# kakaobrain/hqtransformer

Measured on AMD Instinct MI355X. Metric: images/sec (256x256 class-cond sampling), higher is better.
Workload: dtype bf16

## Files before the change

hqtransformer_amd/_lib.py:

```python
from __future__ import annotations

import ctypes as C
import os
import subprocess
from typing import List, Optional

HERE = os.path.dirname(os.path.abspath(__file__))
LIB_PATH = os.path.join(HERE, 'libhqt.so')
CSRC = os.path.join(HERE, 'csrc')
SOURCES = ['engine.hip', 'kernels.hip', 'attention.hip', 'fast_kernels.hip', 'persist.hip', 'tile_gemm.hip', 'exact_gemm.hip', 'mfma_gemm.hip', 'split_conv.hip', 'split_stream_conv.hip']
ABI_VERSION = 9

PRECISION_EXACT, PRECISION_FAST, PRECISION_SPLIT = 0, 1, 2
PRECISIONS = {'exact': PRECISION_EXACT, 'fast': PRECISION_FAST, 'split': PRECISION_SPLIT}
POLICY_LATENCY, POLICY_THROUGHPUT = 0, 1
SWITCH_PERSIST, SWITCH_SINGLE_KEY, SWITCH_PERSIST_FAULT, SWITCH_SPLIT_KSLICES = 0, 1, 2, 3
LAYOUT_FAST, LAYOUT_EXACT, LAYOUT_SPLIT, LAYOUT_ALL = 1, 2, 4, 7
RESAMPLE_PIXELSHUFFLE, RESAMPLE_NEAREST, RESAMPLE_CONV2 = 0, 1, 2


class HqtLibraryError(RuntimeError):
    pass


class HqtError(RuntimeError):
    def __init__(self, code: int, msg: str):
        super().__init__(f'libhqt error {code}: {msg}')
        self.code = code


class hqt_config(C.Structure):
    _fields_ = [
        ('abi_version', C.c_int32),
        ('has_stage2', C.c_int32),
        ('embed_dim', C.c_int32), ('n_layers', C.c_int32), ('n_heads', C.c_int32), ('n_layers_depth', C.c_int32),
        ('vocab_top', C.c_int32), ('vocab_bot', C.c_int32), ('vocab_txt', C.c_int32),
        ('ctx_len_img', C.c_int32), ('ctx_len_txt', C.c_int32), ('n_classes', C.c_int32),
        ('cond_type', C.c_int32), ('embedding_type', C.c_int32), ('gelu_approx', C.c_int32),
        ('has_stage1', C.c_int32),
        ('s1_ch', C.c_int32), ('s1_n_mult', C.c_int32), ('s1_ch_mult', C.c_int32 * 8),
        ('s1_num_res_blocks', C.c_int32),
        ('s1_n_attn_res', C.c_int32), ('s1_attn_res', C.c_int32 * 4),
        ('s1_resolution', C.c_int32), ('s1_z_channels', C.c_int32), ('s1_embed_dim', C.c_int32),
        ('s1_n_embed', C.c_int32), ('s1_out_ch', C.c_int32),
        ('s1_use_init_downsample', C.c_int32), ('s1_use_mid_block', C.c_int32), ('s1_use_attn', C.c_int32),
        ('max_batch', C.c_int32), ('max_steps', C.c_int32),
        ('code_levels', C.c_int32),
        ('depth_decoding', C.c_int32),
        ('ar_layouts', C.c_int32),
        ('s1_resample', C.c_int32),
    ]


class hqt_sample_opts(C.Structure):
    _fields_ = [
        ('precision', C.c_int32), ('n_steps', C.c_int32),
        ('top_k_top', C.c_int32), ('top_k_bot', C.c_int32),
        ('top_p_top', C.c_float), ('top_p_bot', C.c_float),
        ('temperature_top', C.c_float), ('temperature_bot', C.c_float),
        ('seed', C.c_uint64), ('sample_offset', C.c_int64),
        ('use_graph', C.c_int32),
        ('row_seeds', C.c_void_p), ('row_offsets', C.c_void_p),
    ]


class hqt_sample_opts_l3(C.Structure):
    _fields_ = [
        ('precision', C.c_int32), ('n_steps', C.c_int32),
        ('top_k', C.c_int32 * 3), ('top_p', C.c_float * 3), ('temperature', C.c_float * 3),
        ('seed', C.c_uint64), ('sample_offset', C.c_int64),
        ('use_graph', C.c_int32),
        ('row_seeds', C.c_void_p), ('row_offsets', C.c_void_p),
    ]


class hqt_row_sampler(C.Structure):
    _fields_ = [('temperature', C.c_float * 3), ('top_k', C.c_int32 * 3), ('top_p', C.c_float * 3)]


class hqt_guide_pair(C.Structure):
    _fields_ = [('pos_row', C.c_int32), ('neg_row', C.c_int32), ('scale', C.c_float * 3)]


class hqt_encode_out(C.Structure):
    _fields_ = [
        ('codes', C.c_void_p * 3), ('quant', C.c_void_p * 3), ('resid', C.c_void_p * 3),
        ('recon', C.c_void_p), ('diff', C.c_void_p),
    ]


_VP, _I64P, _F32P = C.c_void_p, C.c_void_p, C.c_void_p
SYMBOLS = {
    'hqt_abi_version': (C.c_int, []),
    'hqt_last_error': (C.c_char_p, []),
    'hqt_create': (C.c_int, [C.POINTER(hqt_config), C.c_int, C.POINTER(_VP)]),
    'hqt_set_weight': (C.c_int, [_VP, C.c_char_p, _VP, C.c_int, C.POINTER(C.c_int64), C.c_int]),
    'hqt_finalize_weights': (C.c_int, [_VP]),
    'hqt_clone': (C.c_int, [_VP, C.POINTER(_VP)]),
    'hqt_set_policy': (C.c_int, [_VP, C.c_int]),
    'hqt_set_switch': (C.c_int, [_VP, C.c_int, C.c_int]),
    'hqt_set_row_samplers': (C.c_int, [_VP, C.c_int, C.POINTER(hqt_row_sampler)]),
    'hqt_set_logprob_out': (C.c_int, [_VP, _F32P]),
    'hqt_set_guidance': (C.c_int, [_VP, C.c_int, C.POINTER(hqt_guide_pair)]),
    'hqt_set_keep_mask': (C.c_int, [_VP, C.c_int, C.c_int, _VP, C.POINTER(C.c_void_p)]),
    'hqt_set_prompt_groups': (C.c_int, [_VP, C.c_int, C.c_int, _VP]),
    'hqt_sample': (C.c_int, [_VP, C.c_int, _I64P, C.POINTER(hqt_sample_opts), _F32P, _I64P, _I64P, _F32P, _I64P, _I64P, _VP]),
    'hqt_set_max_prefix': (C.c_int, [_VP, C.c_int]),
    'hqt_sample_prefix': (C.c_int, [_VP, C.c_int, _I64P, C.POINTER(hqt_sample_opts), _F32P, C.c_int, _I64P, _I64P, _I64P, _I64P, _F32P, _I64P, _I64P, _VP]),
    'hqt_set_score_chunk': (C.c_int, [_VP, C.c_int]),
    'hqt_score': (C.c_int, [_VP, C.c_int, _I64P, C.POINTER(C.c_void_p), C.c_int, C.c_int, _F32P, C.POINTER(C.c_void_p), _VP]),
    'hqt_decode': (C.c_int, [_VP, C.c_int, _I64P, _I64P, _F32P, C.c_int, C.c_int, _VP]),
    'hqt_decode_seq': (C.c_int, [_VP, C.c_int, _I64P, _I64P, _F32P, C.c_int, C.c_int, _VP]),
    'hqt_sample_l3': (C.c_int, [_VP, C.c_int, _I64P, C.POINTER(hqt_sample_opts_l3), _F32P, _I64P, _I64P, _I64P, _F32P, _I64P, _I64P, _I64P, _VP]),
    'hqt_sample_prefix_l3': (C.c_int, [_VP, C.c_int, _I64P, C.POINTER(hqt_sample_opts_l3), _F32P, C.c_int, _I64P, _I64P, _I64P, _I64P, _I64P, _I64P, _F32P, _I64P, _I64P, _I64P, _VP]),
    'hqt_decode_l3': (C.c_int, [_VP, C.c_int, _I64P, _I64P, _I64P, _F32P, C.c_int, C.c_int, _VP]),
    'hqt_decode_seq_l3': (C.c_int, [_VP, C.c_int, _I64P, _I64P, _I64P, _F32P, C.c_int, C.c_int, _VP]),
    'hqt_encode': (C.c_int, [_VP, C.c_int, _F32P, C.c_int, C.POINTER(hqt_encode_out), _VP]),
    'hqt_has_encoder': (C.c_int, [_VP]),
    'hqt_range_check': (C.c_int, [_VP, _VP]),
    'hqt_param_count': (C.c_int64, [_VP, C.c_int]),
    'hqt_workspace_bytes': (C.c_int64, [_VP]),
    'hqt_timing_enable': (C.c_int, [_VP, C.c_int]),
    'hqt_timing_reset': (C.c_int, [_VP]),
    'hqt_timing_get': (C.c_int, [_VP, C.c_int, C.c_char_p, C.c_int, C.POINTER(C.c_int64), C.POINTER(C.c_double)]),
    'hqt_timing_slots': (C.c_int, [_VP]),
    'hqt_destroy': (C.c_int, [_VP]),
}

_lib: Optional[C.CDLL] = None


def build(force: bool = False, verbose: bool = False) -> str:
    import hashlib
    from concurrent.futures import ThreadPoolExecutor
    hdrs = sorted([os.path.join(CSRC, f) for f in os.listdir(CSRC) if f.endswith('.h')] + [os.path.join(os.path.dirname(HERE), 'include', 'hqt.h')])
    hipcc = os.environ.get('HIPCC', '/opt/rocm/bin/hipcc')
    flags = ['-O3', '--offload-arch=gfx950', '-std=c++17', '-fPIC', '-Wno-unused-value', '-Wno-unused-result']
    objdir = os.path.join(CSRC, 'build')
    os.makedirs(objdir, exist_ok=True)
    ver = subprocess.run([hipcc, '--version'], stdout=subprocess.PIPE, stderr=subprocess.STDOUT, text=True).stdout
    common = hashlib.sha256()
    for f in hdrs:
        with open(f, 'rb') as fp:
            common.update(os.path.basename(f).encode() + b'\0' + fp.read())
    common.update(' '.join(flags).encode() + ver.encode())

    def read(path):
        try:
            with open(path) as fp:
                return fp.read().strip()
        except OSError:
            return ''

    def stamp_of(name):
        hh = common.copy()
        with open(os.path.join(CSRC, name), 'rb') as fp:
            hh.update(name.encode() + b'\0' + fp.read())
        return hh.hexdigest()

    def compile_one(name):
        src, obj = os.path.join(CSRC, name), os.path.join(objdir, name.replace('.hip', '.o'))
        stamp, want = obj[:-2] + '.stamp', stamp_of(name)
        if not force and os.path.exists(obj) and read(stamp) == want:
            return obj, want
        if os.path.exists(stamp):
            os.remove(stamp)
        cmd = [hipcc] + flags + ['-c', src, '-o', obj]
        if verbose:
            print(' '.join(cmd), flush=True)
# ... 106 lines not shown
```

hqtransformer_amd/csrc/engine.hip:

```cpp
#include "../../include/hqt.h"
#include "kernels.h"
#include "fast_kernels.h"
#include "split_kernels.h"
#include "persist.h"

#include <algorithm>
#include <cmath>
#include <cstdarg>
#include <cstdio>
#include <cstring>
#include <map>
#include <memory>
#include <mutex>
#include <string>
#include <vector>

static thread_local std::string g_err;
static int fail(int code, const char* fmt, ...) {
    char buf[1024];
    va_list ap;
    va_start(ap, fmt);
    vsnprintf(buf, sizeof(buf), fmt, ap);
    va_end(ap);
    g_err = buf;
// ... 21 lines not shown
    }
    ~DeviceGuard() { if (prev >= 0) hipSetDevice(prev); }
};
#define ON_DEVICE(h_)                                                                          \
    DeviceGuard dg_((h_)->device);                                                             \
    if (!dg_.ok) return fail(HQT_ERR_HIP, "hipSetDevice(%d) failed", (h_)->device)

struct Tensor {
    float* d = nullptr;
    std::vector<int64_t> shape;
    size_t n = 0;
};

struct Lin {
    const float* w32 = nullptr;
    const float* b32 = nullptr;
    bf16_t* w16 = nullptr;
    half_t* w16h = nullptr;
    half_t* w16l = nullptr;
    float* w32t = nullptr;
    half_t* wfrag16 = nullptr;
    half_t* wup16 = nullptr;
    bf16_t* wpk = nullptr;
    bf16_t* wpk_ln = nullptr;
    float* colsum = nullptr;
    float* bias_ln = nullptr;
    int N = 0, K = 0;
};

struct BlockW {
    bool body = false;
    const float *ln1_g, *ln1_b, *ln2_g, *ln2_b;
    Lin qkv, proj, fc1, fc2;
};

struct DecLayer {
    int kind;
    std::string name;
    int cin, cout, res;
    Lin conv1, conv2, nin, q, k, v, proj;
    const float *n1_g = nullptr, *n1_b = nullptr, *n2_g = nullptr, *n2_b = nullptr;
};

struct PersistProg {
    std::vector<PersistPhase> phases;
    char* stream = nullptr;
    unsigned long long* d_cu_off = nullptr;
    PersistPhase* d_phases = nullptr;
    bool ok = false;
};

struct TimingSlot {
    std::string name;
    std::vector<std::pair<hipEvent_t, hipEvent_t>> ev;
    size_t used = 0;
    int64_t launches = 0;
    double total_ms = 0.0;
};

struct hqt_handle {
    hqt_config cfg;
    int device = 0;
    bool finalized = false;
    std::map<std::string, Tensor> w;
    std::vector<void*> owned;
    size_t workspace_bytes = 0;
    int64_t params[3] = {0, 0, 0};
    std::vector<BlockW> body, depth;
    Lin head_top, head_bot;
    int Tmax = 0;
    int max_prefix = 0;
    static constexpr int BODY_BUFS = 10;
    size_t body_bytes[BODY_BUFS] = {};
    int depth_rows = 0;
    int score_chunk = 0;
    int depth_cap() const { return std::max(cfg.max_batch, score_chunk); }
    static constexpr int DEPTH_BUFS = 4;
    size_t depth_bytes[DEPTH_BUFS] = {};
    float *x = nullptr, *xd = nullptr, *logits = nullptr;
    void *hbuf = nullptr, *qbuf = nullptr, *abuf = nullptr, *mbuf = nullptr;
    void *kcache = nullptr, *vcache = nullptr, *dk = nullptr, *dv = nullptr;
    bf16_t *xpk = nullptr, *xdpk = nullptr;
    float *parts = nullptr, *partsd = nullptr;
    int nparts = 0, npartsd = 0;
    float* fold_tmp = nullptr;
    bool tile_gemm = true;
    float* splitk = nullptr;
    size_t splitk_elems = 0;
    struct { const float* slabs; int S; int rows; const float* bias; } pend = {nullptr, 0, 0, nullptr};
    StepState* state = nullptr;
    RowKey* rows = nullptr;
    static constexpr int ROWS_RING = 4;
    RowKey* rows_pinned[ROWS_RING] = {nullptr, nullptr, nullptr, nullptr};
    hipEvent_t rows_ev[ROWS_RING] = {nullptr, nullptr, nullptr, nullptr};
    bool rows_busy[ROWS_RING] = {false, false, false, false};
    int rows_next = 0;
    RowSampler* row_set = nullptr;
    std::vector<hqt_row_sampler> row_set_staged;
    float* logprob_staged = nullptr;
    GuidePair* guide = nullptr;
    std::vector<hqt_guide_pair> guide_staged;
    size_t guide_room() const { return (size_t)std::max(1, cfg.max_batch / 2); }
    std::vector<uint8_t> keep_staged;
    int keep_B = 0, keep_n = 0;
    const int64_t* keep_codes[3] = {nullptr, nullptr, nullptr};
    unsigned char* keep_mask = nullptr;
    std::vector<int32_t> groups_staged;
    int groups_G = 0;
    int* group_of_row = nullptr;
    void *pg_k = nullptr, *pg_v = nullptr;
    float* pg_x = nullptr;
    int pg_cap = 0;
    size_t pg_bytes = 0;
    void clear_staged() { row_set_staged.clear(); logprob_staged = nullptr; guide_staged.clear(); keep_staged.clear(); groups_staged.clear(); }
    int64_t *cond_buf = nullptr, *codes_top = nullptr, *codes_bot = nullptr;
    int64_t* codes_l2 = nullptr;
    Lin head_l2;
    std::vector<DecLayer> dec;
    std::vector<DecLayer> enc;
    bool has_encoder = false;
    Lin post_quant, quant_conv;
    float* cb_norm[3] = {nullptr, nullptr, nullptr};
    float *vq_h = nullptr, *vq_recon = nullptr, *vq_zz = nullptr, *vq_err = nullptr;
    void* vq_z = nullptr;
    unsigned long long* vq_best = nullptr;
    float* up_table = nullptr;
    Lin up_lin, down_lin;
    float *vq_t = nullptr, *vq_q = nullptr;
    void* act[4] = {nullptr, nullptr, nullptr, nullptr};
    double* gn_partial = nullptr;
    float* gn_tiles = nullptr;
    void* zero_page = nullptr;
    int* range_flag = nullptr;
    size_t act_elems = 0;
    int dec_chunk = 0;
    void *aq = nullptr, *ak = nullptr, *av = nullptr, *ao = nullptr, *as = nullptr, *quant = nullptr;
    float* gn = nullptr;
    hipGraphExec_t graph_exec = nullptr;
    std::vector<uint64_t> graph_key;
    hqt_handle* parent = nullptr;
    int n_clones = 0;
    int policy = 0;
    PersistProg pbody, pfull;
    float* lnf_shift = nullptr;
    int ncu = 0;
    unsigned* persist_counters = nullptr;
    unsigned* persist_err = nullptr;
    float* persist_slabs = nullptr;
    bool persist_used = false;
    bool persist_enabled = true;
    bool persist_tripped = false;
    bool single_key = true;
    bool split_kslices = true;
    bool capture_persist = false;
    bool graph_has_persist = false;
    int layouts = 0;
    bool timing = false;
    std::vector<TimingSlot> slots;
    hipEvent_t chain_ev = nullptr;
    bool chain_valid = false;
    std::vector<hipEvent_t> all_events;
};

static int dev_alloc(hqt_handle* h, void** p, size_t bytes, bool workspace) {
    HIPCHK(hipMalloc(p, bytes ? bytes : 16));
    const bool poison = getenv("HQT_POISON_WORKSPACE") != nullptr;
    if (poison && workspace && bytes) HIPCHK(hipMemset(*p, 0xFF, bytes));
    h->owned.push_back(*p);
    if (workspace) h->workspace_bytes += bytes;
    return HQT_OK;
}

static int slot_id(hqt_handle* h, const char* name) {
    for (size_t i = 0; i < h->slots.size(); ++i)
        if (h->slots[i].name == name) return (int)i;
    h->slots.push_back(TimingSlot());
    h->slots.back().name = name;
    return (int)h->slots.size() - 1;
}
struct Timed {
    hqt_handle* h; int slot; hipStream_t st; bool on;
    Timed(hqt_handle* h_, const char* name, hipStream_t st_) : h(h_), slot(-1), st(st_), on(h_->timing) {
        if (!on) return;
        slot = slot_id(h, name);
        if (!h->chain_valid) {
            hipEventCreate(&h->chain_ev);
            hipEventRecord(h->chain_ev, st);
            h->chain_valid = true;
        }
    }
    void next(const char* name) {
        if (!on) return;
        hipEvent_t e;
        hipEventCreate(&e);
        hipEventRecord(e, st);
        h->slots[slot].ev.push_back({h->chain_ev, e});
        h->slots[slot].used++;
        h->all_events.push_back(h->chain_ev);
        h->chain_ev = e;
        slot = slot_id(h, name);
    }
    ~Timed() {
        if (!on) return;
        hipEvent_t e;
        hipEventCreate(&e);
        hipEventRecord(e, st);
        h->slots[slot].ev.push_back({h->chain_ev, e});
        h->slots[slot].used++;
        h->all_events.push_back(h->chain_ev);
        h->chain_ev = e;
    }
};
static void count_variant(hqt_handle* h, const char* fmt, ...) {
    if (!h->timing) return;
    char buf[96];
    va_list ap;
    va_start(ap, fmt);
    vsnprintf(buf, sizeof buf, fmt, ap);
    va_end(ap);
    h->slots[slot_id(h, buf)].launches++;
}
static void timing_collect(hqt_handle* h) {
    if (h->chain_valid) hipEventSynchronize(h->chain_ev);
    for (auto& s : h->slots) {
        for (auto& pr : s.ev) {
            float ms = 0.f;
            if (hipEventElapsedTime(&ms, pr.first, pr.second) == hipSuccess) { s.total_ms += ms; s.launches++; }
        }
        s.ev.clear();
        s.used = 0;
    }
    for (hipEvent_t e : h->all_events) hipEventDestroy(e);
    h->all_events.clear();
    if (h->chain_valid) { hipEventDestroy(h->chain_ev); h->chain_valid = false; }
}

static void build_decoder_plan(hqt_handle* h) {
    const hqt_config& c = h->cfg;
    const int n = c.s1_n_mult;
    int block_in = c.s1_ch * c.s1_ch_mult[n - 1];
    int res = c.s1_resolution >> (c.s1_use_init_downsample ? n : n - 1);
    auto is_attn_res = [&](int r) {
        for (int i = 0; i < c.s1_n_attn_res; ++i) if (c.s1_attn_res[i] == r) return true;
        return false;
    };
    auto add = [&](int kind, const std::string& name, int cin, int cout, int r) {
        DecLayer l; l.kind = kind; l.name = name; l.cin = cin; l.cout = cout; l.res = r;
        h->dec.push_back(l);
    };
    add(0, "decoder.conv_in", c.s1_z_channels, block_in, res);
    if (c.s1_use_mid_block) {
        add(1, "decoder.mid.block_1", block_in, block_in, res);
        if (c.s1_use_attn) add(2, "decoder.mid.attn_1", block_in, block_in, res);
        add(1, "decoder.mid.block_2", block_in, block_in, res);
    }
    for (int lvl = n - 1; lvl >= 0; --lvl) {
        const int block_out = c.s1_ch * c.s1_ch_mult[lvl];
        for (int b = 0; b <= c.s1_num_res_blocks; ++b) {
            add(1, "decoder.up." + std::to_string(lvl) + ".block." + std::to_string(b), block_in, block_out, res);
            block_in = block_out;
            if (is_attn_res(res) && c.s1_use_attn)
                add(2, "decoder.up." + std::to_string(lvl) + ".attn." + std::to_string(b), block_in, block_in, res);
        }
        if (lvl != 0 || c.s1_use_init_downsample) {
            add(3, "decoder.up." + std::to_string(lvl) + ".upsample.conv", block_in, block_in, res);
            res *= 2;
        }
    }
    add(4, "decoder", block_in, c.s1_out_ch, res);
}

static void build_encoder_plan(hqt_handle* h) {
    const hqt_config& c = h->cfg;
    const int n = c.s1_n_mult;
    auto is_attn_res = [&](int r) {
        for (int i = 0; i < c.s1_n_attn_res; ++i) if (c.s1_attn_res[i] == r) return true;
        return false;
    };
    auto add = [&](int kind, const std::string& name, int cin, int cout, int r) {
        DecLayer l; l.kind = kind; l.name = name; l.cin = cin; l.cout = cout; l.res = r;
        h->enc.push_back(l);
    };
    add(6, "encoder.conv_in", 3, c.s1_ch, c.s1_resolution);
    int label = c.s1_resolution;
    int res = c.s1_use_init_downsample ? c.s1_resolution / 2 : c.s1_resolution;
    int block_in = c.s1_ch;
    for (int lvl = 0; lvl < n; ++lvl) {
        const int block_out = c.s1_ch * c.s1_ch_mult[lvl];
        for (int b = 0; b < c.s1_num_res_blocks; ++b) {
            add(1, "encoder.down." + std::to_string(lvl) + ".block." + std::to_string(b), block_in, block_out, res);
            block_in = block_out;
            if (is_attn_res(label) && c.s1_use_attn)
                add(2, "encoder.down." + std::to_string(lvl) + ".attn." + std::to_string(b), block_in, block_in, res);
        }
        if (lvl != n - 1) {
            add(5, "encoder.down." + std::to_string(lvl) + ".downsample.conv", block_in, block_in, res);
            res /= 2; label /= 2;
        }
    }
    if (c.s1_use_mid_block) {
        add(1, "encoder.mid.block_1", block_in, block_in, res);
        if (c.s1_use_attn) add(2, "encoder.mid.attn_1", block_in, block_in, res);
        add(1, "encoder.mid.block_2", block_in, block_in, res);
    }
    add(7, "encoder", block_in, c.s1_z_channels, res);
}

extern "C" int hqt_abi_version(void) { return HQT_ABI_VERSION; }
extern "C" const char* hqt_last_error(void) { return g_err.c_str(); }

static int alloc_workspace(hqt_handle* hp);

extern "C" int hqt_create(const hqt_config* cfg, int device, hqt_handle** out) {
    if (!cfg || !out) return fail(HQT_ERR_INVALID, "null argument");
    if (cfg->abi_version != HQT_ABI_VERSION) return fail(HQT_ERR_INVALID, "abi_version %d != %d", cfg->abi_version, HQT_ABI_VERSION);
    if (cfg->max_batch < 1) return fail(HQT_ERR_INVALID, "max_batch must be >= 1");
    DeviceGuard dg(device);
    if (!dg.ok) return fail(HQT_ERR_HIP, "hipSetDevice(%d) failed", device);
    std::unique_ptr<hqt_handle> h(new hqt_handle());
    h->tile_gemm = getenv("HQT_NO_TILE_GEMM") == nullptr;
    { const char* e = getenv("HQT_PERSIST"); h->persist_enabled = !(e && atoi(e) == 0); }
    h->single_key = getenv("HQT_NO_SINGLE_KEY") == nullptr;
    h->split_kslices = getenv("HQT_SPLIT_KSLICES_OFF") == nullptr;
    h->cfg = *cfg;
    h->layouts = (cfg->ar_layouts & HQT_LAYOUT_ALL) ? (cfg->ar_layouts & HQT_LAYOUT_ALL) : HQT_LAYOUT_ALL;
    h->device = device;
    const hqt_config& c = h->cfg;
    if (c.has_stage2) {
        if (c.embed_dim % c.n_heads || c.embed_dim % 16) return fail(HQT_ERR_INVALID, "embed_dim must be a multiple of n_heads and 16");
        const int hs = c.embed_dim / c.n_heads;
        if (hs % 8 || hs > 256 || (hs & (hs - 1))) return fail(HQT_ERR_INVALID, "head_dim %d unsupported (power of two in [8, 256])", hs);
        if (c.vocab_top != c.vocab_bot) return fail(HQT_ERR_INVALID, "vocab_top != vocab_bot");
        const bool bidir = c.depth_decoding == HQT_DEPTH_BIDIRECTIONAL;
        if (c.depth_decoding < 0 || c.depth_decoding > HQT_DEPTH_BIDIRECTIONAL || (c.depth_decoding && !bidir && c.code_levels != 3) || (bidir && c.code_levels == 3))
            return fail(HQT_ERR_INVALID, "depth_decoding %d: 0 'parallel-add', 1 'parallel', 2 'parallel-reduce', 3 'top2mid2bot' (three code levels only), "
                        "4 'bidirectional' (two code levels only)", c.depth_decoding);
        if (bidir && c.cond_type == HQT_COND_TEXT)
            return fail(HQT_ERR_INVALID, "depth_decoding 4 'bidirectional' with text conditioning is not built");
        if (c.vocab_top > HQT_MAX_V || c.vocab_top % 4) return fail(HQT_ERR_INVALID, "vocab size %d unsupported", c.vocab_top);
        if (c.cond_type == HQT_COND_CLASS && c.n_classes < 1) return fail(HQT_ERR_INVALID, "n_classes");
        if (c.max_steps < 1 || c.max_steps > c.ctx_len_img) return fail(HQT_ERR_INVALID, "max_steps must be in [1, ctx_len_img]");
    }
    if (c.has_stage1) {
        if (c.s1_n_mult < 1 || c.s1_n_mult > 8) return fail(HQT_ERR_INVALID, "s1_n_mult");
        if (c.s1_ch % 32) return fail(HQT_ERR_INVALID, "GroupNorm(32) needs ch %% 32 == 0");
        if (c.s1_z_channels % 16 || (2 * c.s1_embed_dim) % 16) return fail(HQT_ERR_INVALID, "z_channels and 2*embed_dim must be multiples of 16");
        if (c.s1_resample < 0 || c.s1_resample > HQT_RESAMPLE_CONV2) return fail(HQT_ERR_INVALID, "s1_resample %d: 0 pixelshuffle, 1 nearest, 2 conv2", c.s1_resample);
        if (c.s1_resample && c.code_levels == 3) return fail(HQT_ERR_INVALID, "s1_resample %d with three code levels: the three-level HQ-VAE is built with pixelshuffle only", c.s1_resample);
        if (c.s1_resample == HQT_RESAMPLE_CONV2 && c.s1_embed_dim % 16) return fail(HQT_ERR_INVALID, "s1_resample 2 (conv2) needs embed_dim %% 16 == 0");
        build_decoder_plan(h.get());
        build_encoder_plan(h.get());
    }
    CHK(alloc_workspace(h.get()));
    *out = h.release();
    return HQT_OK;
}

static int alloc_encode_workspace(hqt_handle* h) {
    const hqt_config& c = h->cfg;
    const int r = h->dec.front().res;
    const size_t rows = (size_t)c.max_batch * r * r, elems = rows * c.s1_embed_dim;
    CHK(dev_alloc(h, (void**)&h->vq_h, elems * 4, true));
    CHK(dev_alloc(h, (void**)&h->vq_recon, elems * 4, true));
    CHK(dev_alloc(h, &h->vq_z, elems * 4, true));
    CHK(dev_alloc(h, (void**)&h->vq_zz, rows * 4, true));
    CHK(dev_alloc(h, (void**)&h->vq_best, rows * 8, true));
    CHK(dev_alloc(h, (void**)&h->vq_err, rows * 4 * 3, true));
    if (c.s1_resample) {
        CHK(dev_alloc(h, (void**)&h->vq_t, elems / 4 * 4, true));
        CHK(dev_alloc(h, (void**)&h->vq_q, elems / 4 * 4, true));
    }
    return HQT_OK;
}

static int alloc_body_rows(hqt_handle* h, bool release_old) {
    const hqt_config& c = h->cfg;
    const size_t B = (size_t)c.max_batch, D = c.embed_dim;
    const int Tp = c.cond_type == HQT_COND_TEXT ? c.ctx_len_txt + h->max_prefix : (h->max_prefix > 0 ? h->max_prefix + 1 : 1);
    const int Tdepth = c.code_levels == 3 ? 16 : (c.depth_decoding == HQT_DEPTH_BIDIRECTIONAL ? 5 : 4);
    const size_t rows = (std::max(B * (size_t)std::max(Tp, Tdepth), (size_t)h->depth_cap() * Tdepth) + 31) / 32 * 32;
    size_t rows_pk = 256;
    while (rows_pk < rows && rows_pk < (size_t)PACKED_MAX_ROWS) rows_pk *= 2;
    rows_pk = std::max(rows_pk, rows);
    h->splitk_elems = (size_t)16 * rows * (size_t)std::max<size_t>(4 * D, (size_t)c.vocab_top);
    void** const bufs[hqt_handle::BODY_BUFS] = {(void**)&h->x, &h->hbuf, &h->qbuf, &h->abuf, &h->mbuf, (void**)&h->splitk,
                                                (void**)&h->xpk, (void**)&h->xdpk, (void**)&h->parts, (void**)&h->partsd};
    const size_t bytes[hqt_handle::BODY_BUFS] = {rows * D * 4, rows * D * 4, rows * D * 4, rows * D * 4, rows * 4 * D * 4, h->splitk_elems * 4,
                                                 rows_pk * D * 2, rows_pk * D * 2, (D / 32 + 1) * rows_pk * 2 * 4, (D / 32 + 1) * rows_pk * 2 * 4};
    for (int i = 0; i < hqt_handle::BODY_BUFS; ++i) {
        if (release_old && *bufs[i]) {
            HIPCHK(hipFree(*bufs[i]));
            h->owned.erase(std::remove(h->owned.begin(), h->owned.end(), *bufs[i]), h->owned.end());
            h->workspace_bytes -= h->body_bytes[i];
            *bufs[i] = nullptr;
        }
        CHK(dev_alloc(h, bufs[i], bytes[i], true));
        h->body_bytes[i] = bytes[i];
    }
    return HQT_OK;
}

static int alloc_depth_ws(hqt_handle* h, bool release_old) {
    const hqt_config& c = h->cfg;
    const size_t cap = (size_t)h->depth_cap(), D = c.embed_dim;
    const int Tdepth = c.code_levels == 3 ? 16 : (c.depth_decoding == HQT_DEPTH_BIDIRECTIONAL ? 5 : 4);
    const size_t dkv = (size_t)c.n_layers_depth * cap * h->depth_rows * D * 4;
    void** const bufs[hqt_handle::DEPTH_BUFS] = {(void**)&h->xd, (void**)&h->logits, &h->dk, &h->dv};
    const size_t bytes[hqt_handle::DEPTH_BUFS] = {cap * Tdepth * D * 4, cap * Tdepth * (size_t)c.vocab_top * 4, dkv, dkv};
    for (int i = 0; i < hqt_handle::DEPTH_BUFS; ++i) {
        if (release_old && *bufs[i]) {
            HIPCHK(hipFree(*bufs[i]));
            h->owned.erase(std::remove(h->owned.begin(), h->owned.end(), *bufs[i]), h->owned.end());
            h->workspace_bytes -= h->depth_bytes[i];
            *bufs[i] = nullptr;
        }
        CHK(dev_alloc(h, bufs[i], bytes[i], true));
        h->depth_bytes[i] = bytes[i];
    }
    return HQT_OK;
}

extern "C" int hqt_set_score_chunk(hqt_handle* h, int pairs) {
    if (!h) return fail(HQT_ERR_INVALID, "null handle");
    const hqt_config& c = h->cfg;
    if (!c.has_stage2) return fail(HQT_ERR_INVALID, "hqt_set_score_chunk: the handle was created without stage 2");
    if (h->finalized || h->parent) return fail(HQT_ERR_STATE, "hqt_set_score_chunk comes between hqt_create and hqt_finalize_weights (lanes inherit the value)");
    const int Tdepth = c.code_levels == 3 ? 16 : (c.depth_decoding == HQT_DEPTH_BIDIRECTIONAL ? 5 : 4);
    if (pairs < 0) return fail(HQT_ERR_INVALID, "hqt_set_score_chunk: pairs=%d is negative (0 restores the default, max_batch pairs)", pairs);
    if ((long long)pairs * Tdepth > PACKED_MAX_ROWS)
        return fail(HQT_ERR_INVALID, "hqt_set_score_chunk: pairs * Tdepth = %d * %d exceeds the %d rows of one pass (at most %d pairs for this depth head)", pairs, Tdepth, PACKED_MAX_ROWS, PACKED_MAX_ROWS / Tdepth);
    if (pairs == h->score_chunk) return HQT_OK;
    ON_DEVICE(h);
    const int cap_before = h->depth_cap();
    h->score_chunk = pairs;
    if (h->depth_cap() == cap_before) return HQT_OK;
    CHK(alloc_depth_ws(h, true));
    return alloc_body_rows(h, true);
}

extern "C" int hqt_set_max_prefix(hqt_handle* h, int max_prefix) {
    if (!h) return fail(HQT_ERR_INVALID, "null handle");
    const hqt_config& c = h->cfg;
    if (!c.has_stage2) return fail(HQT_ERR_INVALID, "hqt_set_max_prefix: the handle was created without stage 2");
    if (h->finalized || h->parent) return fail(HQT_ERR_STATE, "hqt_set_max_prefix comes between hqt_create and hqt_finalize_weights (lanes inherit the value)");
    if (max_prefix < 0 || max_prefix > c.max_steps - 1) return fail(HQT_ERR_INVALID, "max_prefix=%d outside [0, max_steps - 1 = %d]", max_prefix, c.max_steps - 1);
    if (max_prefix && c.cond_type == HQT_COND_TEXT) {
        if (c.code_levels == 3) return fail(HQT_ERR_INVALID, "max_prefix with text conditioning and three code levels is not built (two code levels are)");
        if ((long long)c.max_batch * (c.ctx_len_txt + max_prefix) > PACKED_MAX_ROWS)
            return fail(HQT_ERR_INVALID, "max_batch * (ctx_len_txt + max_prefix) = %d * (%d + %d) exceeds the %d rows of one pass", c.max_batch, c.ctx_len_txt, max_prefix, PACKED_MAX_ROWS);
    }
    if (max_prefix == h->max_prefix) return HQT_OK;
    ON_DEVICE(h);
    h->max_prefix = max_prefix;
    return alloc_body_rows(h, true);
}

static int alloc_workspace(hqt_handle* hp) {
    struct { hqt_handle* p; hqt_handle* get() const { return p; } hqt_handle* operator->() const { return p; } } h{hp};
    const hqt_config& c = h->cfg;
    const size_t B = (size_t)c.max_batch;
    CHK(dev_alloc(h.get(), &h->zero_page, 256, true));
    HIPCHK(hipMemset(h->zero_page, 0, 256));
    CHK(dev_alloc(h.get(), (void**)&h->range_flag, 256, true));
    HIPCHK(hipMemset(h->range_flag, 0, 256));
    if (c.has_stage2) {
        const size_t D = c.embed_dim;
        h->Tmax = (c.cond_type == HQT_COND_TEXT ? c.ctx_len_txt : 0) + c.max_steps;
        h->depth_rows = c.code_levels == 3 ? 21 : 5;
        CHK(alloc_body_rows(h.get(), false));
        h->xd = h->logits = nullptr; h->dk = h->dv = nullptr;
        CHK(alloc_depth_ws(h.get(), false));
        const size_t kv = (size_t)c.n_layers * B * h->Tmax * D * 4;
        CHK(dev_alloc(h.get(), &h->kcache, kv, true));
        CHK(dev_alloc(h.get(), &h->vcache, kv, true));
        CHK(dev_alloc(h.get(), (void**)&h->state, sizeof(StepState), true));
        CHK(dev_alloc(h.get(), (void**)&h->rows, B * sizeof(RowKey), true));
// ... 338 lines not shown
        const int64_t D = c.embed_dim;
        const bool l3 = c.code_levels == 3;
        CHK(get_w(h, key2(h, "head_top.weight"), {c.vocab_top, D}, &w));
        CHK(make_lin(h, h->head_top, w, nullptr, c.vocab_top, D, true, true));
        CHK(get_w(h, key2(h, "head_bot.weight"), {c.vocab_bot, D}, &w));
        CHK(make_lin(h, h->head_bot, w, nullptr, c.vocab_bot, D, true, true));
        if (l3) {
            CHK(get_w(h, "stage2.head_levels.2.weight", {c.vocab_top, D}, &w));
            CHK(make_lin(h, h->head_l2, w, nullptr, c.vocab_top, D, true, true));
        }
        const float* t;
        CHK(get_w(h, "stage2.ln_f.weight", {D}, &t)); CHK(get_w(h, "stage2.ln_f.bias", {D}, &t));
        CHK(get_w(h, key2(h, "ln_top.weight"), {D}, &t)); CHK(get_w(h, key2(h, "ln_top.bias"), {D}, &t));
        CHK(get_w(h, key2(h, "ln_bot.weight"), {D}, &t)); CHK(get_w(h, key2(h, "ln_bot.bias"), {D}, &t));
        CHK(get_w(h, "stage2.sos_depth", {1, 1, D}, &t));
        CHK(get_w(h, key2(h, "tok_emb_top.weight"), {c.vocab_top, D}, &t));
        CHK(get_w(h, key2(h, "tok_emb_bot.weight"), {c.vocab_bot, c.embedding_type == HQT_EMB_REDUCE ? D / 4 : D}, &t));
        if (c.embedding_type == HQT_EMB_TRANSFORMER1) CHK(get_w(h, "stage2.pos_emb_emb.weight", {l3 ? 21 : 5, D}, &t));
        CHK(get_w(h, "stage2.pos_emb_top.weight", {c.ctx_len_img, D}, &t));
        const int dmul = (l3 && c.depth_decoding == HQT_DEPTH_PARALLEL_REDUCE) ? 4 : 1;
        const bool causal_head = l3 && c.depth_decoding == HQT_DEPTH_TOP2MID2BOT;
        if (!causal_head) CHK(get_w(h, key2(h, "tok_emb_top_depth.weight"), {c.vocab_top, dmul * D}, &t));
        CHK(get_w(h, key2(h, "pos_emb_depth.weight"), {causal_head ? 21 : (l3 ? 4 : 5), D}, &t));
        if (l3) {
            CHK(get_w(h, "stage2.tok_emb_levels.2.weight", {c.vocab_top, D}, &t));
            if (!causal_head) {
                CHK(get_w(h, "stage2.tok_emb_depth_levels.1.weight", {c.vocab_top, dmul * D}, &t));
                CHK(get_w(h, "stage2.pos_emb_depths.1.weight", {16, D}, &t));
            }
            CHK(get_w(h, "stage2.ln_levels.2.weight", {D}, &t)); CHK(get_w(h, "stage2.ln_levels.2.bias", {D}, &t));
        }
        {
            const float *g1, *b1;
            CHK(get_w(h, key2(h, "ln_top.weight"), {D}, &g1)); CHK(get_w(h, key2(h, "ln_top.bias"), {D}, &b1));
            CHK(fold_ln(h, h->head_top, g1, b1));
            CHK(get_w(h, key2(h, "ln_bot.weight"), {D}, &g1)); CHK(get_w(h, key2(h, "ln_bot.bias"), {D}, &b1));
            CHK(fold_ln(h, h->head_bot, g1, b1));
            if (l3) {
                CHK(get_w(h, "stage2.ln_levels.2.weight", {D}, &g1)); CHK(get_w(h, "stage2.ln_levels.2.bias", {D}, &b1));
                CHK(fold_ln(h, h->head_l2, g1, b1));
            }
            HIPCHK(hipDeviceSynchronize());
        }
        CHK(persist_build(h));
        if (c.cond_type == HQT_COND_CLASS) CHK(get_w(h, "stage2.sos.weight", {c.n_classes, D}, &t));
        else if (c.cond_type == HQT_COND_TEXT) {
            CHK(get_w(h, "stage2.tok_emb_txt.weight", {c.vocab_txt, D}, &t));
            CHK(get_w(h, "stage2.pos_emb_txt.weight", {c.ctx_len_txt, D}, &t));
        } else CHK(get_w(h, "stage2.sos", {1, 1, D}, &t));
    }
    if (c.has_stage1) {
        const int E = c.s1_embed_dim;
        const float* t;
        if (c.code_levels == 3) {
            CHK(get_w(h, "stage1.quantizers.0.embedding", {c.s1_n_embed, 16 * E}, &t));
            CHK(get_w(h, "stage1.quantizers.1.embedding", {c.s1_n_embed, 4 * E}, &t));
            CHK(get_w(h, "stage1.quantizers.2.embedding", {c.s1_n_embed, E}, &t));
            CHK(load_conv(h, "post_quant_conv_b", c.s1_z_channels, E, 1, h->post_quant));
        } else {
            CHK(get_w(h, "stage1.quantize_t.embedding", {c.s1_n_embed, c.s1_resample ? E : 4 * E}, &t));
            if (c.s1_resample == HQT_RESAMPLE_CONV2) {
                const float *uw, *ub;
                CHK(get_w(h, "stage1.upsample_t.weight", {E, E, 2, 2}, &uw));
                CHK(get_w(h, "stage1.upsample_t.bias", {E}, &ub));
                CHK(dev_alloc(h, (void**)&h->up_table, (size_t)c.s1_n_embed * 4 * E * 4, false));
                HIPCHK(launch_fold_upsample_t(t, uw, ub, h->up_table, c.s1_n_embed, E, 0));
                float *wt, *b4;
                CHK(dev_alloc(h, (void**)&wt, (size_t)4 * E * E * 4, false));
                CHK(dev_alloc(h, (void**)&b4, (size_t)4 * E * 4, false));
                HIPCHK(launch_repack_upsample_t(uw, ub, wt, b4, E, 0));
                h->up_lin = Lin();
                h->up_lin.w32 = wt; h->up_lin.b32 = b4; h->up_lin.N = 4 * E; h->up_lin.K = E;
            }
            CHK(get_w(h, "stage1.quantize_b.embedding", {c.s1_n_embed, E}, &t));
            CHK(load_conv(h, "post_quant_conv_b", c.s1_z_channels, 2 * E, 1, h->post_quant));
        }
        for (auto& l : h->dec) {
            if (l.kind == 0 || l.kind == 3) CHK(load_conv(h, l.name, l.cout, l.cin, 3, l.conv1, l.kind == 3));
            else if (l.kind == 1) {
                CHK(get_w(h, "stage1." + l.name + ".norm1.weight", {l.cin}, &l.n1_g));
                CHK(get_w(h, "stage1." + l.name + ".norm1.bias", {l.cin}, &l.n1_b));
                CHK(get_w(h, "stage1." + l.name + ".norm2.weight", {l.cout}, &l.n2_g));
                CHK(get_w(h, "stage1." + l.name + ".norm2.bias", {l.cout}, &l.n2_b));
                CHK(load_conv(h, l.name + ".conv1", l.cout, l.cin, 3, l.conv1));
                CHK(load_conv(h, l.name + ".conv2", l.cout, l.cout, 3, l.conv2));
                if (l.cin != l.cout) CHK(load_conv(h, l.name + ".nin_shortcut", l.cout, l.cin, 1, l.nin));
            } else if (l.kind == 2) {
                CHK(get_w(h, "stage1." + l.name + ".norm.weight", {l.cin}, &l.n1_g));
                CHK(get_w(h, "stage1." + l.name + ".norm.bias", {l.cin}, &l.n1_b));
                CHK(load_conv(h, l.name + ".q", l.cin, l.cin, 1, l.q));
                CHK(load_conv(h, l.name + ".k", l.cin, l.cin, 1, l.k));
                CHK(load_conv(h, l.name + ".v", l.cin, l.cin, 1, l.v));
                CHK(load_conv(h, l.name + ".proj_out", l.cin, l.cin, 1, l.proj));
            } else {
                CHK(get_w(h, "stage1.decoder.norm_out.weight", {l.cin}, &l.n1_g));
                CHK(get_w(h, "stage1.decoder.norm_out.bias", {l.cin}, &l.n1_b));
                CHK(load_conv(h, "decoder.conv_out", l.cout, l.cin, 3, l.conv1));
            }
        }
    }
    if (c.has_stage1 && h->w.count("stage1.encoder.conv_in.weight") && (c.s1_resample != HQT_RESAMPLE_CONV2 || h->w.count("stage1.down_t.weight")))
        CHK(load_encoder(h));
    HIPCHK(stream_gemm_configure());
    HIPCHK(tile_gemm_configure());
    HIPCHK(mfma_gemm_configure());
    HIPCHK(split_kernels_configure());
    HIPCHK(hipDeviceSynchronize());
    h->finalized = true;
    return HQT_OK;
}

struct Mode {
    bool fast = false;
    bool split = false;
    bool split_ar = false;
    int act_dt() const { return fast ? DT_BF16 : DT_F32; }
    size_t act_sz() const { return fast ? 2 : 4; }
};
static int mode_of(int precision, bool stage1, Mode* md) {
    if (precision == HQT_PRECISION_FAST) md->fast = true;
    else if (precision == HQT_PRECISION_SPLIT && stage1) md->split = true;
    else if (precision == HQT_PRECISION_SPLIT) md->split_ar = true;
    else if (precision != HQT_PRECISION_EXACT) return fail(HQT_ERR_INVALID, "unknown precision %d", precision);
    return HQT_OK;
}

static void lin_args(const hqt_handle* h, GemmArgs& g, const Lin& l, bool split_planes) {
    g.N = l.N; g.K = l.K; g.ldb = l.K;
    g.bias = l.b32;
    g.zero_page = h->zero_page;
    g.tune = h->policy;
    if (g.alpha == 0.0f) g.alpha = 1.0f;
    if (g.lda == 0) g.lda = l.K;
    if (split_planes) { g.Bw = l.w16h; g.Bw_lo = l.w16l; g.Bw_frag16 = l.wfrag16; g.Bw_up16 = l.wup16; }
}

struct SlotName {
    char s[64];
    SlotName(const char* tag, int rows) {
        static const bool by_rows = getenv("HQT_TIMING_BY_ROWS") != nullptr;
        snprintf(s, sizeof s, by_rows ? "%s@%d" : "%s", tag, rows);
    }
};

static int ar_linear(hqt_handle* h, const Mode& md, GemmArgs g, const Lin& l, int a_dt, int c_dt, hipStream_t st,
                     const char* tag, bool defer_residual = false, int* resid_nparts = nullptr) {
    lin_args(h, g, l, false);
    g.k_quarters = 1;
    const SlotName slot(tag, g.M);
    Timed t(h, slot.s, st);
    if (md.fast) {
        if (resid_nparts) *resid_nparts = g.N / 32;
        if ((g.ln_parts ? l.wpk_ln : l.wpk) && h->tile_gemm && tile_gemm_ok(g, a_dt, c_dt)) {
            const TilePlan tp = tile_gemm_plan(g);
            if (tp.geom >= 0 && (size_t)tp.S * 32 * g.a_packed_mb * g.N <= h->splitk_elems) {
                if (g.ln_parts) g.bias = l.bias_ln;
                HIPCHK(launch_tile_gemm(g, g.ln_parts ? l.wpk_ln : l.wpk, a_dt, c_dt, tp, h->splitk, st));
                if (tp.S > 1) {
                    count_variant(h, "variant:tile_gemm_%dx%d_splitk%d:%s", tp.bm, tp.bn, tp.S, slot.s);
                    t.next(SlotName("gemm_combine", g.M).s);
                    HIPCHK(launch_resid_combine(g, h->splitk, tp.S, st));
                } else count_variant(h, "variant:tile_gemm_%dx%d%s:%s", tp.bm, tp.bn, g.ln_parts ? "_dln" : "", slot.s);
                if (resid_nparts) *resid_nparts = tp.S > 1 ? 1 : g.N / tp.bn;
                return HQT_OK;
            }
        }
        if (g.ln_parts) {
            if (!l.wpk_ln || !stream_gemm_ok(g, a_dt, c_dt)) return fail(HQT_ERR_STATE, "deferred-LayerNorm GEMM without folded weights (%s)", tag);
            g.bias = l.bias_ln;
            HIPCHK(launch_stream_gemm(g, l.wpk_ln, a_dt, c_dt, 1, nullptr, st));
            count_variant(h, "variant:stream_gemm_dln:%s", tag);
            return HQT_OK;
        }
        if (l.wpk && stream_gemm_ok(g, a_dt, c_dt)) {
            int S = (defer_residual && g.store != STORE_RESID) ? stream_gemm_splitk(g) : 1;
            if ((size_t)S * 32 * g.a_packed_mb * g.N > h->splitk_elems) S = 1;
            HIPCHK(launch_stream_gemm(g, l.wpk, a_dt, c_dt, S, h->splitk, st));
            count_variant(h, "variant:stream_gemm:%s", tag);
            if (S > 1) h->pend = {h->splitk, S, 32 * g.a_packed_mb, l.b32};
            return HQT_OK;
        }
        g.Bw = l.w16;
        if (mfma_gemm_ok(g, a_dt, DT_BF16, c_dt)) {
            HIPCHK(launch_mfma_gemm(g, a_dt, DT_BF16, c_dt, st));
            count_variant(h, "variant:mfma_gemm:%s", tag);
        } else {
            HIPCHK(launch_gemm_generic(g, a_dt, DT_BF16, c_dt, st));
            count_variant(h, "variant:gemm_generic_bf16:%s", tag);
        }
        return HQT_OK;
    }
    if (md.split_ar && l.w16h && l.w16l && !g.a_packed_mb && g.M > 256) {
        GemmArgs sg = g;
        lin_args(h, sg, l, true);
        sg.a_f32 = 1; sg.range_flag = h->range_flag;
        if (split_gemm_ok(sg)) {
            const int S = h->split_kslices ? split_gemm_slices(sg) : 1;
            if (S > 1 && (size_t)S * sg.M * sg.N <= h->splitk_elems) { sg.k_slices = S; sg.k_slabs = h->splitk; }
            HIPCHK(launch_split_gemm(sg, st));
            if (sg.k_slices > 1) count_variant(h, "variant:split_gemm_kslices%d:%s", sg.k_slices, tag);
            else count_variant(h, "variant:split_gemm:%s", tag);
            return HQT_OK;
        }
    }
    g.Bw = l.w32;
    if (exact_mfma_ok(g)) {
        if (l.w32t && g.N % 16 == 0) { g.Bw = l.w32t; g.b_tile16 = 1; }
        HIPCHK(launch_exact_mfma_gemm(g, st));
        count_variant(h, "variant:exact_mfma:%s", tag);
        return HQT_OK;
    }
    HIPCHK(launch_gemm_generic(g, DT_F32, DT_F32, DT_F32, st));
    count_variant(h, "variant:gemm_generic_f32:%s", tag);
    return HQT_OK;
}

struct SamplerSet { float temperature = 1.f; int top_k = 0; float top_p = 0.f; };
struct SampleCtx {
    int B;
    const int64_t* cond;
    int levels;
    int precision, n_steps, use_graph;
    uint64_t seed;
    int64_t sample_offset;
    const uint64_t* row_seeds;
    const int64_t* row_offsets;
    SamplerSet lv[3];
    const hqt_row_sampler* row_set = nullptr;
    bool row_top_p = false;
    const float* noise;
    const int64_t* feed[3] = {nullptr, nullptr, nullptr};
    int64_t* out[3] = {nullptr, nullptr, nullptr};
    int prefix_len = 0;
    const int64_t* prefix[3] = {nullptr, nullptr, nullptr};
    bool with_prefix = false;
    float* logits_out;
    float* logprob_out = nullptr;
    const hqt_guide_pair* guide = nullptr;
    int n_guide = 0;
    const uint8_t* keep = nullptr;
    const int64_t* keep_codes[3] = {nullptr, nullptr, nullptr};
    const int32_t* groups = nullptr;
    int n_groups = 0;
    hipStream_t st;
    Mode md;
};

static std::string key2(const hqt_handle* h, const char* name) {
    std::string n(name);
    if (h->cfg.code_levels == 3) {
        static const char* const tr[][2] = {
            {"tok_emb_top.weight", "tok_emb_levels.0.weight"}, {"tok_emb_bot.weight", "tok_emb_levels.1.weight"},
            {"tok_emb_top_depth.weight", "tok_emb_depth_levels.0.weight"}, {"pos_emb_depth.weight", "pos_emb_depths.0.weight"},
            {"ln_top.weight", "ln_levels.0.weight"}, {"ln_top.bias", "ln_levels.0.bias"},
            {"ln_bot.weight", "ln_levels.1.weight"}, {"ln_bot.bias", "ln_levels.1.bias"},
            {"head_top.weight", "head_levels.0.weight"}, {"head_bot.weight", "head_levels.1.weight"}};
        for (auto& t : tr) if (n == t[0]) { n = t[1]; break; }
    }
    return "stage2." + n;
}
static const float* W(hqt_handle* h, const char* name) { return h->w[key2(h, name)].d; }


struct PackSrc { const float* w; const float* gamma; };

static void persist_block_shapes(hqt_handle* h, const BlockW& bw, bool single_key, int cache_T, int* k4, std::vector<PersistPhase>& out, std::vector<PackSrc>& src) {
    const int D = h->cfg.embed_dim;
    PersistPhase ph{};
    if (single_key) {
        ph.type = PP_KV1; ph.N = 2 * D; ph.K = D; ph.dln = 1; ph.cache_T = cache_T; ph.kv_row = 0;
        out.push_back(ph); src.push_back({bw.qkv.w32 + (size_t)D * D, bw.ln1_g});
    } else {
        ph.type = PP_QKV; ph.N = 3 * D; ph.K = D; ph.dln = 1; ph.cache_T = cache_T;
        out.push_back(ph); src.push_back({bw.qkv.w32, bw.ln1_g});
        ph = PersistPhase{}; ph.type = PP_ATTN; ph.cache_T = cache_T;
        out.push_back(ph); src.push_back({nullptr, nullptr});
    }
    ph = PersistPhase{}; ph.type = PP_RESID; ph.map = PP_MAP_QUAD; ph.N = D; ph.K = D;
    out.push_back(ph); src.push_back({bw.proj.w32, nullptr});
    ph = PersistPhase{}; ph.type = PP_GELU; ph.N = 4 * D; ph.K = D; ph.dln = 1; ph.act = h->cfg.gelu_approx ? ACT_GELU_SIGMOID : ACT_GELU_ERF;
    out.push_back(ph); src.push_back({bw.fc1.w32, bw.ln2_g});
    ph = PersistPhase{}; ph.type = PP_RESID_K4; ph.map = PP_MAP_K4; ph.N = D; ph.K = 4 * D; ph.k4_epoch = ++*k4;
    out.push_back(ph); src.push_back({bw.fc2.w32, nullptr});
}

static int persist_build_one(hqt_handle* h, PersistProg& pr, const std::vector<PackSrc>& src) {
    const hqt_config& c = h->cfg;
    pr.ok = false;
    if (!persist_program_ok(pr.phases, c.embed_dim, 64, c.n_heads, h->ncu)) return HQT_OK;
    std::vector<unsigned long long> cu_off, tile_off;
    const size_t bytes = persist_layout(pr.phases, h->ncu, cu_off, tile_off);
    CHK(dev_alloc(h, (void**)&pr.stream, bytes + 1024, false));
    CHK(dev_alloc(h, (void**)&pr.d_cu_off, cu_off.size() * 8, false));
    HIPCHK(hipMemcpy(pr.d_cu_off, cu_off.data(), cu_off.size() * 8, hipMemcpyHostToDevice));
    unsigned long long* d_tile = nullptr;
    HIPCHK(hipMalloc((void**)&d_tile, tile_off.size() * 8));
    hipError_t e = hipMemcpy(d_tile, tile_off.data(), tile_off.size() * 8, hipMemcpyHostToDevice);
    for (size_t p = 0; p < pr.phases.size() && e == hipSuccess; ++p)
        if (src[p].w) e = launch_persist_pack(src[p].w, src[p].gamma, pr.phases[p], h->ncu, pr.stream, d_tile + p * h->ncu, 0);
    if (e == hipSuccess) e = hipDeviceSynchronize();
    hipFree(d_tile);
    HIPCHK(e);
    pr.ok = true;
    return HQT_OK;
}

static int persist_build(hqt_handle* h) {
// ... 767 lines not shown
                    HIPCHK(launch_score_depth_embed(feed[0], p0, np, W(h, "tok_emb_top_depth.weight"), W(h, "pos_emb_depth.weight"), h->xd, D, xpk, pk, h->partsd,
                                                    c.st, V, dmul * D));
                } else {
                    Timed t(h, "embed", c.st);
                    HIPCHK(launch_score_depth_embed_l2(feed[0], feed[1], p0, np, cf.depth_decoding == HQT_DEPTH_PARALLEL_ADD ? W(h, "tok_emb_top_depth.weight") : nullptr,
                                                       W(h, "tok_emb_depth_levels.1.weight"), W(h, "pos_emb_depths.1.weight"), h->xd, D, xpk, pk, h->partsd,
                                                       c.st, V, dmul * D));
                }
                h->npartsd = 1;
                CHK(run_depth(h, cc, dln, s.Tq, s.tbase));
            }
            float* lg = (logits_out && logits_out[s.lv]) ? logits_out[s.lv] + (size_t)p0 * s.Tq * V : h->logits;
            CHK(run_head(h, cc, *heads[s.lv], s.lv, M, dln, normed[s.lv], lg));
            {
                Timed t(h, "score_logprob", c.st);
                HIPCHK(launch_score_logprob(lg, feed[s.lv] + (size_t)p0 * s.Tq, logprobs + (size_t)p0 * draws, np, V, s.Tq, s.tbase, draws, c.st));
            }
        }
    }
    return HQT_OK;
}

struct PersistOrder {
    static std::mutex& mu() { static std::mutex m; return m; }
    static hipEvent_t& ev(int device) { static std::map<int, hipEvent_t> evs; return evs[device]; }
    std::unique_lock<std::mutex> lock;
    hipStream_t st;
    int device;
    bool active;
    PersistOrder(int device_, hipStream_t st_, bool active_) : st(st_), device(device_), active(active_) {
        if (!active) return;
        lock = std::unique_lock<std::mutex>(mu());
        hipEvent_t& e = ev(device);
        if (!e) { if (hipEventCreateWithFlags(&e, hipEventDisableTiming) != hipSuccess) { e = nullptr; return; } }
        else hipStreamWaitEvent(st, e, 0);
    }
    ~PersistOrder() {
        if (!active) return;
        hipEvent_t e = ev(device);
        if (e) hipEventRecord(e, st);
    }
};

static int sample_run(hqt_handle* h, const SampleCtx& c) {
    const hqt_config& cf = h->cfg;
    const int B = c.B;
    bool top_p = false;
    for (int i = 0; i < c.levels; ++i) top_p = top_p || c.lv[i].top_p > 0.f;
    HIPCHK(sampler_configure(cf.vocab_top, top_p || c.row_top_p));
    CHK(persist_bind(h));
    HIPCHK(launch_set_step(h->state, 0, 0, c.st));
    if ((c.row_seeds || c.row_offsets) && (!c.row_seeds || !c.row_offsets)) return fail(HQT_ERR_INVALID, "row_seeds and row_offsets come together");
    if (c.row_seeds || c.row_set || c.guide || c.keep || c.groups) {
        const int slot = h->rows_next;
        h->rows_next = (slot + 1) % hqt_handle::ROWS_RING;
        if (!h->rows_pinned[slot]) {
            HIPCHK(hipHostMalloc((void**)&h->rows_pinned[slot], (size_t)h->cfg.max_batch * (sizeof(RowKey) + sizeof(RowSampler)) + h->guide_room() * sizeof(GuidePair) + (size_t)h->cfg.max_batch * sizeof(int32_t) + (size_t)h->cfg.max_batch * h->cfg.max_steps, hipHostMallocDefault));
            HIPCHK(hipEventCreateWithFlags(&h->rows_ev[slot], hipEventDisableTiming));
        }
        if (h->rows_busy[slot]) HIPCHK(hipEventSynchronize(h->rows_ev[slot]));
        RowKey* rk = h->rows_pinned[slot];
        if (c.row_seeds || c.guide) {
            for (int b = 0; b < B; ++b) {
                rk[b].seed = c.row_seeds ? c.row_seeds[b] : c.seed;
                rk[b].global_row = c.row_offsets ? c.row_offsets[b] : c.sample_offset + b;
            }
            for (int i = 0; i < c.n_guide; ++i) rk[c.guide[i].neg_row] = rk[c.guide[i].pos_row];
            HIPCHK(hipMemcpyAsync(h->rows, rk, (size_t)B * sizeof(RowKey), hipMemcpyHostToDevice, c.st));
        }
        if (c.row_set) {
            RowSampler* rs = reinterpret_cast<RowSampler*>(rk + h->cfg.max_batch);
            memcpy(rs, c.row_set, (size_t)B * sizeof(RowSampler));
            HIPCHK(hipMemcpyAsync(h->row_set, rs, (size_t)B * sizeof(RowSampler), hipMemcpyHostToDevice, c.st));
        }
        if (c.guide) {
            GuidePair* gp = reinterpret_cast<GuidePair*>(reinterpret_cast<RowSampler*>(rk + h->cfg.max_batch) + h->cfg.max_batch);
            memcpy(gp, c.guide, (size_t)c.n_guide * sizeof(GuidePair));
            HIPCHK(hipMemcpyAsync(h->guide, gp, (size_t)c.n_guide * sizeof(GuidePair), hipMemcpyHostToDevice, c.st));
        }
        if (c.keep) {
            unsigned char* km = reinterpret_cast<unsigned char*>(reinterpret_cast<int32_t*>(reinterpret_cast<GuidePair*>(reinterpret_cast<RowSampler*>(rk + h->cfg.max_batch) + h->cfg.max_batch) + h->guide_room()) + h->cfg.max_batch);
            memcpy(km, c.keep, (size_t)B * c.n_steps);
            HIPCHK(hipMemcpyAsync(h->keep_mask, km, (size_t)B * c.n_steps, hipMemcpyHostToDevice, c.st));
        }
        if (c.groups) {
            int32_t* gr = reinterpret_cast<int32_t*>(reinterpret_cast<GuidePair*>(reinterpret_cast<RowSampler*>(rk + h->cfg.max_batch) + h->cfg.max_batch) + h->guide_room());
            memcpy(gr, c.groups, (size_t)B * sizeof(int32_t));
            HIPCHK(hipMemcpyAsync(h->group_of_row, gr, (size_t)B * sizeof(int32_t), hipMemcpyHostToDevice, c.st));
        }
        HIPCHK(hipEventRecord(h->rows_ev[slot], c.st));
        h->rows_busy[slot] = true;
    }
    if (c.keep) {
        static const int width[3] = {1, 4, 16};
        for (int i = 0; i < c.levels; ++i)
            HIPCHK(launch_copy_kept(c.keep_codes[i], c.out[i], h->keep_mask, B, c.n_steps, width[i], cf.vocab_top, c.st));
    }
    if (!c.row_seeds && !c.guide) HIPCHK(launch_set_rows(h->rows, B, c.seed, c.sample_offset, c.st));
    int first = 0;
    const int64_t* const own[3] = {h->codes_top, h->codes_bot, h->codes_l2};
    if (cf.cond_type == HQT_COND_TEXT && c.groups) {
        const int T = cf.ctx_len_txt;
        const int G = c.n_groups, D = cf.embed_dim;
        SampleCtx cg = c;
        cg.B = G;
        HIPCHK(launch_embed_text(c.cond, W(h, "tok_emb_txt.weight"), W(h, "pos_emb_txt.weight"), h->x, G, T, D, c.st, cf.vocab_txt, T));
        const KvStage stage{h->pg_k, h->pg_v};
        bool pfull = false;
        CHK(run_body(h, cg, T, 0, false, false, &pfull, &stage));
        if (h->pend.slabs) CHK(run_ln(h, c.st, h->x, W(h, "ln_f.weight"), W(h, "ln_f.bias"), nullptr, h->hbuf, G * T, D, 1, 0, DT_F32, 0));
        {
            Timed t(h, "prompt_fanout", c.st);
            const FanoutArgs fa{h->pg_k, h->pg_v, h->kcache, h->vcache, h->x, h->pg_x, h->group_of_row, cf.n_layers, B, G, T, D,
                                D * (int)c.md.act_sz(), cf.max_batch, h->Tmax};
            HIPCHK(launch_prompt_fanout(fa, c.st));
        }
        float* const x_body = h->x;
        h->x = h->pg_x;
        const int rc = run_depth_head(h, c, 1, false);
        h->x = x_body;
        CHK(rc);
        HIPCHK(launch_advance_step(h->state, T, c.st));
        first = 1;
    } else if (cf.cond_type == HQT_COND_TEXT) {
        const int T = cf.ctx_len_txt, P = c.prefix_len;
        if (P) HIPCHK(launch_set_step(h->state, P, 0, c.st));
        HIPCHK(launch_embed_text(c.cond, W(h, "tok_emb_txt.weight"), W(h, "pos_emb_txt.weight"), h->x, B, T, cf.embed_dim, c.st, cf.vocab_txt, T + P));
        if (P) {
            Timed t(h, "embed_prefix", c.st);
            HIPCHK(launch_embed_prefix(embed_args(h, c, own), P, T + P, T, 1, c.st));
        }
        CHK(run_position(h, c, T + P, 0, false));
        HIPCHK(launch_advance_step(h->state, T + P, c.st));
        first = P + 1;
    } else if (c.prefix_len) {
        const int P = c.prefix_len;
        HIPCHK(launch_set_step(h->state, P, 0, c.st));
        {
            Timed t(h, "embed_prefix", c.st);
            HIPCHK(launch_embed_prefix(embed_args(h, c, own), P + 1, P + 1, 0, 0, c.st));
        }
        CHK(run_position(h, c, P + 1, 0, false));
        HIPCHK(launch_advance_step(h->state, P + 1, c.st));
        first = P + 1;
    }
    const int remaining = c.n_steps - first;
    if (remaining <= 0) return HQT_OK;
    if (c.use_graph && !h->timing) {
        static const int gmax = getenv("HQT_GRAPH_POSITIONS") ? std::max(1, atoi(getenv("HQT_GRAPH_POSITIONS"))) : 16;
        int G = 1;
        for (int d = std::min(gmax, remaining); d >= 1; --d) if (remaining % d == 0) { G = d; break; }
        std::vector<uint64_t> key = {(uint64_t)G, (uint64_t)B, (uint64_t)(c.cond != nullptr), (uint64_t)c.noise, (uint64_t)c.logits_out, (uint64_t)c.logprob_out,
                                     (uint64_t)c.precision, (uint64_t)c.n_steps, (uint64_t)c.levels, (uint64_t)h->policy,
                                     (uint64_t)((h->persist_enabled && !h->persist_tripped ? 1 : 0) + (h->single_key ? 0 : 4) + (h->split_kslices ? 0 : 8))};
        for (const int64_t* f : c.feed) key.push_back((uint64_t)f);
        for (const SamplerSet& l : c.lv) {
            uint32_t f[2];
            memcpy(f, &l.top_p, 4); memcpy(f + 1, &l.temperature, 4);
            key.push_back((uint64_t)l.top_k); key.push_back(f[0]); key.push_back(f[1]);
        }
        key.push_back((uint64_t)((c.row_set ? 1 : 0) + (c.row_top_p ? 2 : 0)));
        key.push_back((uint64_t)c.n_guide);
        key.push_back(c.keep ? (uint64_t)c.prefix_len + 1 : 0);
        if (!h->graph_exec || key != h->graph_key) {
            if (h->graph_exec) {
                HIPCHK(hipStreamSynchronize(c.st));
                hipGraphExecDestroy(h->graph_exec);
                h->graph_exec = nullptr;
            }
            hipStream_t cs;
            HIPCHK(hipStreamCreateWithFlags(&cs, hipStreamNonBlocking));
            SampleCtx cc = c;
            cc.st = cs;
            h->capture_persist = false;
            HIPCHK(hipStreamBeginCapture(cs, hipStreamCaptureModeThreadLocal));
            int rc = HQT_OK;
            for (int gi = 0; gi < G && rc == HQT_OK; ++gi) rc = run_decode_step(h, cc);
            hipGraph_t graph = nullptr;
            hipError_t e = hipStreamEndCapture(cs, &graph);
            hipStreamDestroy(cs);
            if (rc != HQT_OK) { if (graph) hipGraphDestroy(graph); return rc; }
            HIPCHK(e);
            HIPCHK(hipGraphInstantiate(&h->graph_exec, graph, nullptr, nullptr, 0));
            hipGraphDestroy(graph);
            h->graph_key = key;
            h->graph_has_persist = h->capture_persist;
            h->persist_used = false;
        }
        PersistOrder order(h->device, c.st, h->graph_has_persist);
        if (h->graph_has_persist) h->persist_used = true;
        for (int s = 0; s < remaining / G; ++s) HIPCHK(hipGraphLaunch(h->graph_exec, c.st));
        return HQT_OK;
    }
    const bool may_persist = c.md.fast && c.B <= 64 && (persist_on(h, c, h->pfull) || persist_on(h, c, h->pbody));
    PersistOrder order(h->device, c.st, may_persist);
    for (int s = 0; s < remaining; ++s) CHK(run_decode_step(h, c));
    return HQT_OK;
}

static const float* W1(hqt_handle* h, const std::string& name) { return h->w["stage1." + name].d; }

static GemmArgs conv_args(const void* in, int nimg, int res_out, int cin, int taps, int upsample, void* out, int cout) {
    GemmArgs g{};
    g.A = in; g.conv_taps = taps; g.H = res_out; g.W = res_out; g.Cin = cin; g.upsample = upsample;
    g.M = nimg * res_out * res_out; g.batch = 1;
    g.C = out; g.ldc = cout; g.store = STORE_ROWS;
    return g;
}
static void with_gn(GemmArgs& g, const float* stats, const float* gamma, const float* beta, int swish) {
    g.gn_stats = stats; g.gn_gamma = gamma; g.gn_beta = beta; g.gn_groups = 32; g.gn_swish = swish;
}

struct S1Ctx {
    hqt_handle* h;
    int n;
    Mode md;
    hipStream_t st;
    int adt;
    void *cur, *t1, *t2, *tn;
    float *gn1, *gn2;
    bool cur_planes = false;
    struct { const void* tensor; int tiles; bool dbl; } gn_ready = {nullptr, 0, false};
};

enum S1Operand { S1_TENSOR, S1_PLANES, S1_SPLIT_IN_KERNEL };

static bool split_shape_ok(const hqt_handle* h, const GemmArgs& g, const Lin& l) {
    if (!l.w16h) return false;
    GemmArgs t = g;
    lin_args(h, t, l, true);
    return t.conv_taps == 9 ? split_conv3_ok(t) : split_gemm_ok(t);
}
static int s1_split_pack(S1Ctx& c, GemmArgs* g, const float* stats, const float* gamma, const float* beta, int swish) {
    hqt_handle* h = c.h;
    const int hw_in = g->conv_taps ? ((g->H << g->conv_stride2) >> g->upsample) * ((g->W << g->conv_stride2) >> g->upsample) : 0;
    const int C = g->conv_taps ? g->Cin : g->lda;
    const int rows = g->conv_taps ? c.n : 1, per = g->conv_taps ? hw_in : g->M;
    Timed t(h, "split_pack", c.st);
    HIPCHK(launch_split_pack(reinterpret_cast<const float*>(g->A), reinterpret_cast<half_t*>(c.tn), stats, gamma, beta, rows, per, C, 32, swish, h->range_flag, c.st));
    g->A = c.tn;
    if (!g->conv_taps) g->lda = 2 * C;
    return HQT_OK;
}

static int s1_split_stats(S1Ctx& c, const void* src, int C, int hw, float* stats) {
    Timed t(c.h, "gn_stats", c.st);
    if (c.gn_ready.tensor == src && c.gn_ready.dbl) {
        count_variant(c.h, "variant:gn_stats_tiles:gn");
        HIPCHK(launch_gn_finalize_tiles_d(reinterpret_cast<const double*>(c.h->gn_tiles), stats, c.n, c.gn_ready.tiles, hw, C, 32, 1e-6f, c.st));
    } else {
        count_variant(c.h, "variant:gn_stats_pass:gn");
        HIPCHK(launch_gn_stats_fast(src, stats, c.h->gn_partial, c.n, hw, C, 32, 1e-6f, c.st, DT_F32));
    }
    return HQT_OK;
}

static int s1_norm(S1Ctx& c, const void* src, int C, int hw, float* stats, const float* gamma, const float* beta, int swish, GemmArgs* g,
                   const Lin& l, S1Operand* a) {
    hqt_handle* h = c.h;
    hipStream_t st = c.st;
    *a = S1_TENSOR;
    if (c.md.fast) {
        {
            Timed t(h, "gn_stats", st);
            if (c.gn_ready.tensor == src && !c.gn_ready.dbl) {
                count_variant(h, "variant:gn_stats_tiles:gn");
                HIPCHK(launch_gn_finalize_tiles(h->gn_tiles, stats, c.n, c.gn_ready.tiles, hw, C, 32, 1e-6f, st));
            } else {
                count_variant(h, "variant:gn_stats_pass:gn");
                HIPCHK(launch_gn_stats_fast(src, stats, h->gn_partial, c.n, hw, C, 32, 1e-6f, st));
            }
        }
        { Timed t(h, "gn_apply", st); HIPCHK(launch_gn_apply(src, c.tn, stats, gamma, beta, c.n, hw, C, 32, swish, st)); }
        g->A = c.tn;
    } else if (c.md.split && split_shape_ok(h, *g, l)) {
        CHK(s1_split_stats(c, src, C, hw, stats));
        CHK(s1_split_pack(c, g, stats, gamma, beta, swish));
        *a = S1_PLANES;
    } else {
        { Timed t(h, "gn_stats", st); HIPCHK(launch_gn_stats(src, c.adt, stats, c.n, hw, C, 32, 1e-6f, st)); }
        count_variant(h, "variant:gn_stats_two_pass:gn");
        with_gn(*g, stats, gamma, beta, swish);
    }
    return HQT_OK;
}
static int s1_plain(S1Ctx& c, GemmArgs* g, const Lin& l, S1Operand* a) {
    *a = S1_TENSOR;
    if (!c.md.split) return HQT_OK;
    if (g->conv_taps == 1) {
        GemmArgs t = *g;
        t.a_f32 = 1;
        if (split_shape_ok(c.h, t, l)) {
            g->a_f32 = 1; g->range_flag = c.h->range_flag; *a = S1_SPLIT_IN_KERNEL;
            return HQT_OK;
        }
    }
    if (!split_shape_ok(c.h, *g, l)) return HQT_OK;
    *a = S1_PLANES;
    return s1_split_pack(c, g, nullptr, nullptr, nullptr, 0);
}

static int s1_conv(S1Ctx& c, GemmArgs g, S1Operand a, const Lin& l, int c_dt, const char* tag) {
    hqt_handle* h = c.h;
    lin_args(h, g, l, a != S1_TENSOR);
    Timed t(h, SlotName(tag, g.M).s, c.st);
    if (c.gn_ready.tensor == g.C) c.gn_ready.tensor = nullptr;
    if (a != S1_TENSOR) {
// ... 212 lines not shown
                          int precision, void* stream) {
    return decode_impl(h, B, code_t, nullptr, code_b, 0, out, clamp01, precision, stream, 2);
}
extern "C" int hqt_decode_seq(hqt_handle* h, int B, const int64_t* codes_top, const int64_t* codes_bot, float* out,
                              int clamp01, int precision, void* stream) {
    return decode_impl(h, B, codes_top, nullptr, codes_bot, 1, out, clamp01, precision, stream, 2);
}
extern "C" int hqt_decode_l3(hqt_handle* h, int B, const int64_t* code_t, const int64_t* code_m, const int64_t* code_b, float* out,
                             int clamp01, int precision, void* stream) {
    return decode_impl(h, B, code_t, code_m, code_b, 0, out, clamp01, precision, stream, 3);
}
extern "C" int hqt_decode_seq_l3(hqt_handle* h, int B, const int64_t* codes0, const int64_t* codes1, const int64_t* codes2, float* out,
                                 int clamp01, int precision, void* stream) {
    return decode_impl(h, B, codes0, codes1, codes2, 1, out, clamp01, precision, stream, 3);
}

static int encode_chunk(hqt_handle* h, int n, const float* pixels, float* h_rows, const Mode& md, hipStream_t st) {
    const hqt_config& cf = h->cfg;
    const int adt = md.act_dt();
    S1Ctx c{h, n, md, st, adt, h->act[0], h->act[1], h->act[2], h->act[3], h->gn, h->gn + (size_t)h->dec_chunk * 64};
    for (auto& l : h->enc) {
        if (l.kind == 6) {
            const int cp = conv_in_cpad(cf), down = cf.s1_use_init_downsample ? 1 : 0;
            { Timed t(h, "image_layout", st); HIPCHK(launch_image_to_nhwc(pixels, c.t2, adt, n, l.res, cp, st)); }
            GemmArgs g = conv_args(c.t2, n, l.res >> down, cp, down ? 16 : 9, 0, c.t1, l.cout);
            g.conv_stride2 = down;
            CHK(s1_conv(c, g, S1_TENSOR, l.conv1, adt, "conv_in"));
            std::swap(c.cur, c.t1);
        } else if (l.kind == 7) {
            const int hw = l.res * l.res;
            GemmArgs g = conv_args(c.cur, n, l.res, l.cin, 9, 0, c.t1, l.cout);
            S1Operand a;
            CHK(s1_norm(c, c.cur, l.cin, hw, c.gn1, l.n1_g, l.n1_b, 1, &g, l.conv1, &a));
            CHK(s1_conv(c, g, a, l.conv1, adt, "conv3x3"));
            GemmArgs q = conv_args(c.t1, n, l.res, l.cout, 1, 0, h_rows, cf.s1_embed_dim);
            CHK(s1_plain(c, &q, h->quant_conv, &a));
            CHK(s1_conv(c, q, a, h->quant_conv, DT_F32, "conv1x1"));
        } else {
            CHK(s1_layer(c, l));
        }
    }
    return HQT_OK;
}

static int encode_top_resampled(hqt_handle* h, int B, const hqt_encode_out* out, hipStream_t st) {
    const hqt_config& cf = h->cfg;
    const int r = h->dec.front().res, E = cf.s1_embed_dim, rq = r / 2, M = B * rq * rq;
    const bool conv2 = cf.s1_resample == HQT_RESAMPLE_CONV2;
    auto linear = [&](const float* A, const Lin& l, float* C, const char* slot) -> int {
        Timed t(h, slot, st);
        GemmArgs g{};
        g.A = A; g.lda = l.K; g.M = M; g.N = l.N; g.K = l.K; g.batch = 1; g.Bw = l.w32; g.ldb = l.K; g.bias = l.b32; g.alpha = 1.0f;
        g.C = C; g.ldc = l.N; g.store = STORE_ROWS; g.zero_page = h->zero_page;
        HIPCHK(launch_gemm_generic(g, DT_F32, DT_F32, DT_F32, st));
        return HQT_OK;
    };
    if (conv2) {
        VqArgs u{};
        u.h = h->vq_h; u.recon = nullptr; u.B = B; u.r = r; u.E = E; u.k = 1; u.z = h->vq_z; u.z_dtype = DT_F32; u.zz = h->vq_zz;
        { Timed t(h, "vq_rows", st); HIPCHK(launch_vq_rows(u, st)); }
        CHK(linear((const float*)h->vq_z, h->down_lin, h->vq_t, "vq_down_t"));
    } else {
        Timed t(h, "vq_rows", st);
        HIPCHK(launch_vq_avgpool_rows(h->vq_h, h->vq_t, B, r, E, st));
    }
    HIPCHK(launch_row_sumsq(h->vq_t, DT_F32, h->vq_zz, M, E, st));
    if (out->resid[0]) HIPCHK(launch_nhwc_to_nchw_f32(h->vq_t, out->resid[0], B, rq * rq, E, st));
    HIPCHK(hipMemsetAsync(h->vq_best, 0xff, (size_t)M * 8, st));
    const float* emb = W1(h, "quantize_t.embedding");
    {
        Timed t(h, "vq_distance", st);
        GemmArgs g{};
        g.A = h->vq_t; g.lda = E; g.M = M; g.N = cf.s1_n_embed; g.K = E; g.batch = 1; g.ldb = E; g.alpha = 1.0f;
        g.store = STORE_ARGMIN; g.am_rownorm = h->vq_zz; g.am_best = h->vq_best; g.zero_page = h->zero_page;
        g.Bw = emb; g.am_colnorm = h->cb_norm[0];
        HIPCHK(launch_gemm_generic(g, DT_F32, DT_F32, DT_F32, st));
    }
    VqTopArgs a{h->vq_t, h->vq_best, emb, B, r, E, out->codes[0], out->quant[0], conv2 ? h->vq_q : nullptr, conv2 ? nullptr : h->vq_recon, h->vq_err};
    { Timed t(h, "vq_finish", st); HIPCHK(launch_vq_finish_top(a, st)); }
    if (conv2) {
        CHK(linear(h->vq_q, h->up_lin, (float*)h->vq_z, "vq_upsample_t"));
        Timed t(h, "vq_finish", st);
        HIPCHK(launch_vq_scatter_up((const float*)h->vq_z, h->vq_recon, B, r, E, st));
    }
    if (out->diff) HIPCHK(launch_vq_diff(h->vq_err, M, 0.25f / ((float)M * (float)E), out->diff, st));
    return HQT_OK;
}

extern "C" int hqt_has_encoder(const hqt_handle* h) { return h ? (h->has_encoder ? 1 : 0) : -1; }

extern "C" int hqt_encode(hqt_handle* h, int B, const float* pixels, int precision, const hqt_encode_out* out, void* stream) {
    if (!h || !pixels || !out) return fail(HQT_ERR_INVALID, "null argument");
    if (!h->finalized) return fail(HQT_ERR_STATE, "hqt_finalize_weights has not run");
    if (!h->cfg.has_stage1) return fail(HQT_ERR_STATE, "handle was created without stage 1");
    if (!h->has_encoder) return fail(HQT_ERR_STATE, "the encoder tensors (stage1.encoder.*, stage1.quant_conv_b.*%s) were not set before hqt_finalize_weights",
                                     h->cfg.s1_resample == HQT_RESAMPLE_CONV2 ? ", stage1.down_t.*" : "");
    if (B < 1 || B > h->cfg.max_batch) return fail(HQT_ERR_INVALID, "B must be in [1, max_batch = %d]", h->cfg.max_batch);
    const hqt_config& cf = h->cfg;
    const int L = cf.code_levels == 3 ? 3 : 2;
    for (int l = 0; l < L; ++l) if (!out->codes[l]) return fail(HQT_ERR_INVALID, "codes[%d] is NULL", l);
    ON_DEVICE(h);
    hipStream_t st = (hipStream_t)stream;
    Mode md;
    CHK(mode_of(precision, true, &md));
    const int r = h->dec.front().res, E = cf.s1_embed_dim, R = cf.s1_resolution;
    for (int b0 = 0; b0 < B; b0 += h->dec_chunk) {
        const int n = std::min(h->dec_chunk, B - b0);
        CHK(encode_chunk(h, n, pixels + (size_t)b0 * 3 * R * R, h->vq_h + (size_t)b0 * r * r * E, md, st));
    }
    const size_t elems = (size_t)B * r * r * E;
    for (int l = 0; l < L; ++l) {
        if (l == 0 && cf.s1_resample) { CHK(encode_top_resampled(h, B, out, st)); continue; }
        const int k = L - 1 - l, rq = r >> k, dim = E << (2 * k), M = B * rq * rq;
        const std::string name = L == 3 ? "quantizers." + std::to_string(l) + ".embedding" : (l == 0 ? "quantize_t.embedding" : "quantize_b.embedding");
        VqArgs a{};
        a.h = h->vq_h; a.recon = l == 0 ? nullptr : h->vq_recon;
        a.B = B; a.r = r; a.E = E; a.k = k;
        a.z = h->vq_z; a.z_dtype = DT_F32; a.zz = h->vq_zz; a.resid_nchw = out->resid[l];
        a.best = h->vq_best; a.emb = W1(h, name); a.codes = out->codes[l]; a.quant_nchw = out->quant[l];
        a.err_rows = h->vq_err + (size_t)l * cf.max_batch * r * r;
        { Timed t(h, "vq_rows", st); HIPCHK(launch_vq_rows(a, st)); }
        HIPCHK(hipMemsetAsync(h->vq_best, 0xff, (size_t)M * 8, st));
        {
            Timed t(h, "vq_distance", st);
            GemmArgs g{};
            g.A = h->vq_z; g.lda = dim; g.M = M; g.N = cf.s1_n_embed; g.K = dim; g.batch = 1; g.ldb = dim; g.alpha = 1.0f;
            g.store = STORE_ARGMIN; g.am_rownorm = h->vq_zz; g.am_best = h->vq_best; g.zero_page = h->zero_page;
            g.Bw = a.emb; g.am_colnorm = h->cb_norm[l];
            HIPCHK(launch_gemm_generic(g, DT_F32, DT_F32, DT_F32, st));
        }
        if (l == 0) {
            HIPCHK(hipMemsetAsync(h->vq_recon, 0, elems * 4, st));
            a.recon = h->vq_recon;
        }
        { Timed t(h, "vq_finish", st); HIPCHK(launch_vq_finish(a, st)); }
        if (out->diff) HIPCHK(launch_vq_diff(a.err_rows, M, 0.25f / ((float)M * (float)dim), out->diff + l, st));
    }
    if (out->recon) HIPCHK(launch_nhwc_to_nchw_f32(h->vq_recon, out->recon, B, r * r, E, st));
    return HQT_OK;
}

extern "C" int hqt_set_policy(hqt_handle* h, int policy) {
    if (!h) return fail(HQT_ERR_INVALID, "null handle");
    if (policy != HQT_POLICY_LATENCY && policy != HQT_POLICY_THROUGHPUT) return fail(HQT_ERR_INVALID, "unknown policy %d", policy);
    h->policy = policy;
    return HQT_OK;
}

extern "C" int hqt_set_switch(hqt_handle* h, int which, int on) {
    if (!h) return fail(HQT_ERR_INVALID, "null handle");
    if (which == HQT_SWITCH_PERSIST) { h->persist_enabled = on != 0; if (on) h->persist_tripped = false; }
    else if (which == HQT_SWITCH_SINGLE_KEY) h->single_key = on != 0;
    else if (which == HQT_SWITCH_SPLIT_KSLICES) h->split_kslices = on != 0;
    else if (which == HQT_SWITCH_PERSIST_FAULT) {
        if (!h->persist_err) return fail(HQT_ERR_STATE, "no persistent chain on this handle (a lane, or a handle without stage 2)");
        ON_DEVICE(h);
        const unsigned v = (unsigned)on;
        HIPCHK(hipDeviceSynchronize());
        HIPCHK(hipMemcpy(h->persist_err + 1, &v, sizeof v, hipMemcpyHostToDevice));
    }
    else return fail(HQT_ERR_INVALID, "unknown switch %d", which);
    return HQT_OK;
}

extern "C" int hqt_range_check(hqt_handle* h, void* stream) {
    if (!h) return fail(HQT_ERR_INVALID, "null");
    ON_DEVICE(h);
    int flag = 0;
    HIPCHK(hipStreamSynchronize((hipStream_t)stream));
    if (h->persist_used && h->persist_err) {
        unsigned pe = 0;
        HIPCHK(hipMemcpy(&pe, h->persist_err, sizeof pe, hipMemcpyDeviceToHost));
        h->persist_used = false;
        if (pe) {
            HIPCHK(hipMemset(h->persist_err, 0, sizeof pe));
            h->persist_tripped = true;
            return fail(HQT_ERR_STATE, "a persistent AR launch on this handle gave up at the grid barrier in front of phase %u (its workgroups were not all resident within 1 s: the GPU is shared with a process that keeps compute units busy): "
                                       "the codes of that call are invalid; repeat it -- this handle now takes the launch chain (hqt_set_switch(h, HQT_SWITCH_PERSIST, 1) re-arms the persistent launch)", pe - 1);
        }
    }
    HIPCHK(hipMemcpy(&flag, h->range_flag, sizeof flag, hipMemcpyDeviceToHost));
    if (!flag) return HQT_OK;
    HIPCHK(hipMemset(h->range_flag, 0, sizeof flag));
    return fail(HQT_ERR_RANGE, "a SPLIT-precision call on this handle met an activation outside the fp16 range (NaN or |x| >= 65504): its output is "
                               "invalid; repeat the call with HQT_PRECISION_EXACT");
}

extern "C" int64_t hqt_param_count(const hqt_handle* h, int stage) { return (h && (stage == 1 || stage == 2)) ? h->params[stage] : -1; }
extern "C" int64_t hqt_workspace_bytes(const hqt_handle* h) { return h ? (int64_t)h->workspace_bytes : -1; }
extern "C" int hqt_timing_enable(hqt_handle* h, int on) { if (!h) return fail(HQT_ERR_INVALID, "null"); timing_collect(h); h->timing = on != 0; return HQT_OK; }
extern "C" int hqt_timing_reset(hqt_handle* h) {
    if (!h) return fail(HQT_ERR_INVALID, "null");
    timing_collect(h);
    for (auto& s : h->slots) { s.launches = 0; s.total_ms = 0.0; }
    return HQT_OK;
}
extern "C" int hqt_timing_slots(const hqt_handle* h) { return h ? (int)h->slots.size() : -1; }
extern "C" int hqt_timing_get(hqt_handle* h, int slot, char* name, int name_len, int64_t* launches, double* total_ms) {
    if (!h || slot < 0 || slot >= (int)h->slots.size()) return fail(HQT_ERR_INVALID, "bad slot");
    timing_collect(h);
    const TimingSlot& s = h->slots[slot];
    if (name && name_len > 0) { strncpy(name, s.name.c_str(), name_len - 1); name[name_len - 1] = 0; }
    if (launches) *launches = s.launches;
    if (total_ms) *total_ms = s.total_ms;
    return HQT_OK;
}
```

hqtransformer_amd/csrc/fast_kernels.h:

```cpp
#pragma once
#include "common.h"
#include "kernels.h"

hipError_t launch_f32_to_bf16(const float* src, bf16_t* dst, size_t n, hipStream_t st);
hipError_t launch_repack_conv(const float* src, float* dst, int O, int I, int taps, hipStream_t st, int Ipad = 0);

bool stream_gemm_supported(int N, int K);
hipError_t launch_pack_stream_weights(const float* w32, bf16_t* packed, int N, int K, hipStream_t st);
hipError_t launch_fold_layernorm(const float* w32, const float* gamma, const float* beta, const float* bias, float* wfold_tmp,
                                 bf16_t* packed, float* colsum, float* bias_out, int N, int K, hipStream_t st);
bool stream_gemm_ok(const GemmArgs& g, int a_dt, int c_dt);
hipError_t stream_gemm_configure();
int stream_gemm_splitk(const GemmArgs& g);
hipError_t launch_stream_gemm(const GemmArgs& g, const bf16_t* wpk, int a_dt, int c_dt, int S, float* slabs, hipStream_t st);

struct TilePlan { int geom; int bm, bn; int S; };
constexpr int TILE_CTR_MAX = 4096;
bool tile_gemm_ok(const GemmArgs& g, int a_dt, int c_dt);
TilePlan tile_gemm_plan(const GemmArgs& g);
hipError_t launch_tile_gemm(const GemmArgs& g, const bf16_t* wpk, int a_dt, int c_dt, const TilePlan& p, float* slabs, hipStream_t st);
hipError_t launch_resid_combine(const GemmArgs& g, const float* slabs, int S, hipStream_t st);
hipError_t tile_gemm_configure();

bool mfma_gemm_ok(const GemmArgs& g, int a_dt, int b_dt, int c_dt);
hipError_t launch_mfma_gemm(const GemmArgs& g, int a_dt, int b_dt, int c_dt, hipStream_t st);
bool conv_halo_ok(const GemmArgs& g, int c_dt);
bool conv_halo_stats_ok(int N, int groups);
int conv_halo_tiles_per_image(const GemmArgs& g);
hipError_t mfma_gemm_configure();
```

hqtransformer_amd/csrc/tile_gemm.hip:

```cpp
#include "fast_kernels.h"
#include "gemm_generic.h"
#include <algorithm>
#include <type_traits>

typedef __attribute__((ext_vector_type(8))) __bf16 bf16x8;
typedef __attribute__((ext_vector_type(16))) float f32x16;
typedef __attribute__((ext_vector_type(4))) float f32x4;

enum { TS_QKV = 0, TS_PACKED = 1, TS_RESID = 2, TS_ROWS = 3, TS_SLAB = 4,
       TS_FUSED = 5 };
typedef __attribute__((ext_vector_type(4))) unsigned u32x4;
#ifndef HQT_TILE_STAGGER
#define HQT_TILE_STAGGER 1
#endif

template <int WGM_, int WGN_, int MBW_, int NT_, int KU_, int NSTAGE_, int NLOAD_ = 0>
struct TileGeom {
    static constexpr int WGM = WGM_, WGN = WGN_, MBW = MBW_, NT = NT_, KU = KU_, NSTAGE = NSTAGE_, NLOAD = NLOAD_;
    static constexpr int NC = WGM * WGN;
    static constexpr int NW = NC + NLOAD;
    static constexpr int NDMA = NLOAD ? NLOAD : NC;
    static constexpr int BM = 32 * MBW * WGM, BN = 32 * NT * WGN;
    static constexpr int ACH = BM / 32, WCH = BN / 32;
    static constexpr int CPS = ACH + WCH;
    static constexpr int CH_STAGE = KU * CPS;
    static constexpr int CPW = CH_STAGE / NDMA;
    static constexpr int STAGE_BYTES = CH_STAGE * 1024;
    static constexpr int RING_BYTES = NSTAGE * STAGE_BYTES;
    static constexpr int GR = NC * 64 / BM;
    static constexpr int AUX_BYTES = BM * 8 + BN * 8 + GR * BM * 8;
    static constexpr int LDS_BYTES = RING_BYTES + AUX_BYTES;
    static constexpr int WG_PER_CU = NW == 4 ? (160 * 1024 / LDS_BYTES < 4 ? 160 * 1024 / LDS_BYTES : 4) : (LDS_BYTES <= 80 * 1024 ? 2 : 1);
    static_assert(CH_STAGE % NDMA == 0, "every issuing wave issues the same number of DMA pieces per stage");
    static_assert(NC * 64 % BM == 0 && GR >= 1, "statistics prologue: whole thread groups per row");
    static_assert(WGN * BM * 8 <= RING_BYTES, "residual epilogue: per-wave partial statistics fit the dead ring");
};

__device__ __forceinline__ float gelu_erf_fast(float v) {
    const float x = fabsf(v) * 0.70710678118654752440f;
    const float t = __builtin_amdgcn_rcpf(fmaf(0.3275911f, x, 1.0f));
    const float poly = t * fmaf(t, fmaf(t, fmaf(t, fmaf(t, 1.061405429f, -1.453152027f), 1.421413741f), -0.284496736f), 0.254829592f);
    const float e = 1.0f - poly * __expf(-x * x);
    return 0.5f * v + 0.5f * fabsf(v) * e;
}
template <int ACT> __device__ __forceinline__ float tile_act(float v) {
    if (ACT == ACT_GELU_ERF) return gelu_erf_fast(v);
    if (ACT == ACT_GELU_SIGMOID) return v / (1.0f + __expf(-1.702f * v));
    return v;
}

template <int N> __device__ __forceinline__ void wait_vmcnt() {
    static_assert(N >= 0 && N < 64, "vmcnt immediate");
    asm volatile("s_waitcnt vmcnt(%0)" ::"n"(N) : "memory");
}

__device__ __forceinline__ void tile_of(int b, int total, int S, int TM, int TN, int& z, int& tm, int& tn) {
    int t;
    if (S > 1 && (8 % S) == 0) {
        const int xcd = b & 7, G = 8 / S, xg = xcd / S;
        z = xcd - xg * S;
        const int q = total / G, r = total - q * G;
        t = (xg < r ? xg * (q + 1) : r * (q + 1) + (xg - r) * q) + (b >> 3);
    } else {
        z = b / total;
        const int id = b - z * total;
        const int q = total >> 3, r = total & 7, xcd = id & 7;
        t = (xcd < r ? xcd * (q + 1) : r * (q + 1) + (xcd - r) * q) + (id >> 3);
    }
    const int nb = TM <= 12 ? 1 : (TM + 7) >> 3;
    const int GM = (TM + nb - 1) / nb;
    const int per_group = GM * TN;
    const int group = t / per_group, in_group = t - group * per_group;
    const int first = group * GM, rows = min(TM - first, GM);
    tn = in_group / rows;
    tm = first + in_group - tn * rows;
}

template <class G, int STORE, bool DLN, typename TC, int ACT = ACT_NONE>
__global__ __launch_bounds__(G::NW * 64, (G::NW / 4) * G::WG_PER_CU) void tile_gemm_kernel(GemmArgs g, const char* __restrict__ wpk,
                                                                                              float* __restrict__ slabs, int TM, int TN) {
#if defined(__HIP_DEVICE_COMPILE__)
    constexpr int WGM = G::WGM, MBW = G::MBW, NT = G::NT, KU = G::KU, NSTAGE = G::NSTAGE, NW = G::NW, NC = G::NC, NLOAD = G::NLOAD, NDMA = G::NDMA;
    constexpr int BM = G::BM, BN = G::BN, ACH = G::ACH, CPS = G::CPS, CPW = G::CPW, STAGE = G::STAGE_BYTES;
    extern __shared__ __attribute__((aligned(1024))) char lds[];
    float* const meanrstd = reinterpret_cast<float*>(lds + G::RING_BYTES);
    float* const colb = meanrstd + 2 * BM;
    float* const scratch = colb + 2 * BN;
#ifdef HQT_TILE_STAMPS
    long long stamp[8];
    stamp[5] = stamp[6] = stamp[7] = 0;
    stamp[0] = wall_clock64(); stamp[1] = clock64();
#endif
    const int wave = __builtin_amdgcn_readfirstlane(threadIdx.x >> 6), lane = threadIdx.x & 63;
    const int wm = wave % WGM, wn = wave / WGM;
    const bool loader = NLOAD > 0 && wave >= NC;
    const int dw = NLOAD > 0 ? max(wave - NC, 0) : wave;
    const int total = TM * TN;
    const int S = gridDim.x / total;
    int z, tile_m, tile_n;
    tile_of(blockIdx.x, total, S, TM, TN, z, tile_m, tile_n);
    const int m0 = tile_m * BM, n0 = tile_n * BN;
    const int MB = g.a_packed_mb, KS = g.K >> 4, NTILES = g.N >> 5;
    const int ks_lo = (int)(((long long)KS * z) / S), ks_hi = (int)(((long long)KS * (z + 1)) / S);
    const int KT = (ks_hi - ks_lo) / KU;

    const auto rsA = __builtin_amdgcn_make_buffer_rsrc(const_cast<void*>(g.A), 0, 0xFFFFFFFF, 0x00020000);
    const auto rsW = __builtin_amdgcn_make_buffer_rsrc(const_cast<char*>(wpk), 0, 0xFFFFFFFF, 0x00020000);
    constexpr int NA = KU * ACH;
    static_assert(NA % NDMA == 0, "pieces 0 .. NA / NDMA - 1 of every issuing wave are A fragments, the rest W fragments");
    unsigned off[CPW], dstoff[CPW];
#pragma unroll
    for (int i = 0; i < CPW; ++i) {
        const int f = i * NDMA + dw;
        if (i < NA / NDMA) {
            const int ku = f / ACH, r = f - ku * ACH;
            off[i] = (unsigned)(((size_t)(ks_lo + ku) * MB + min(tile_m * ACH + r, MB - 1)) * 1024);
            dstoff[i] = (ku * CPS + r) * 1024;
        } else {
            const int fw = f - NA, ku = fw / G::WCH, r = fw - ku * G::WCH;
            off[i] = (unsigned)(((size_t)min(tile_n * G::WCH + r, NTILES - 1) * KS + ks_lo + ku) * 1024);
            dstoff[i] = (ku * CPS + ACH + r) * 1024;
        }
    }
    const unsigned stepA = (unsigned)KU * MB * 1024, stepW = KU * 1024;
    const int lane16 = lane * 16;
    auto issue = [&](int slot) {
#pragma unroll
        for (int i = 0; i < CPW; ++i) {
            char* dst = lds + slot * STAGE + dstoff[i];
            if (i < NA / NDMA) {
                __builtin_amdgcn_raw_ptr_buffer_load_lds(rsA, (__attribute__((address_space(3))) void*)dst, 16, lane16, off[i], 0, 0);
                off[i] += stepA;
            } else {
                __builtin_amdgcn_raw_ptr_buffer_load_lds(rsW, (__attribute__((address_space(3))) void*)dst, 16, lane16, off[i], 0, 0);
                off[i] += stepW;
            }
        }
    };

    f32x16 acc[NT][MBW];
#pragma unroll
    for (int j = 0; j < NT; ++j)
#pragma unroll
        for (int i = 0; i < MBW; ++i)
#pragma unroll
            for (int r = 0; r < 16; ++r) acc[j][i][r] = 0.0f;

    float bias_r = 0.0f, cs_r = 0.0f;
    const int pc = min((int)threadIdx.x, BN - 1);
    if (STORE != TS_SLAB) {
        const float* zsrc = reinterpret_cast<const float*>(g.A);
        const int n = min(n0 + pc, g.N - 1);
        bias_r = *(g.bias ? g.bias + n : zsrc);
        cs_r = *(DLN ? g.ln_colsum + n : zsrc);
    }
    constexpr int NPL = 6;
    float2 pv[NPL];
    const int pr = threadIdx.x % BM, pgi = threadIdx.x / BM;
    if (DLN && !loader) {
        const float2* base = reinterpret_cast<const float2*>(g.ln_parts) + min(m0 + pr, MB * 32 - 1);
#pragma unroll
        for (int i = 0; i < NPL; ++i) pv[i] = base[(size_t)min(pgi + i * G::GR, g.ln_nparts - 1) * (MB * 32)];
    }
    __builtin_amdgcn_sched_barrier(0);
    if (NLOAD == 0 || loader) {
#pragma unroll
        for (int s = 0; s < NSTAGE; ++s) issue(s);
    }
    __builtin_amdgcn_sched_barrier(0);
    if (STORE != TS_SLAB && (int)threadIdx.x < BN) {
        colb[pc] = g.bias ? bias_r : 0.0f;
        colb[BN + pc] = cs_r;
    }
    if (DLN) {
        float sm = 0.0f, sq = 0.0f;
#pragma unroll
        for (int i = 0; i < NPL; ++i)
            if (pgi + i * G::GR < g.ln_nparts) { sm += pv[i].x; sq += pv[i].y; }
        if (g.ln_nparts > NPL * G::GR) {
            const float2* base = reinterpret_cast<const float2*>(g.ln_parts) + min(m0 + pr, MB * 32 - 1);
            for (int p0 = pgi + NPL * G::GR; p0 < g.ln_nparts; p0 += G::GR) { const float2 v = base[(size_t)p0 * (MB * 32)]; sm += v.x; sq += v.y; }
        }
        if (!loader) {
            scratch[2 * threadIdx.x] = sm;
            scratch[2 * threadIdx.x + 1] = sq;
        }
        asm volatile("s_waitcnt lgkmcnt(0)" ::: "memory");
        __builtin_amdgcn_s_barrier();
        __builtin_amdgcn_sched_barrier(0);
        if (threadIdx.x < BM) {
            float a = 0.0f, b = 0.0f;
#pragma unroll
            for (int k = 0; k < G::GR; ++k) { a += scratch[2 * (k * BM + threadIdx.x)]; b += scratch[2 * (k * BM + threadIdx.x) + 1]; }
            const float mean = a / (float)g.K;
            const float var = fmaxf(b / (float)g.K - mean * mean, 0.0f);
            meanrstd[2 * threadIdx.x] = mean;
            meanrstd[2 * threadIdx.x + 1] = 1.0f / sqrtf(var + g.ln_eps);
        }
    }
    const int qkv_row_dev = (STORE == TS_QKV && g.row_offset_dev) ? *g.row_offset_dev : 0;

    bf16x8 af[2][MBW], wf[2][NT];
    auto read_frags = [&](auto set_tag, int slot, int ku) {
        constexpr int SET = decltype(set_tag)::value;
        const char* st = lds + slot * STAGE + ku * (CPS * 1024) + lane * 16;
#pragma unroll
        for (int j = 0; j < NT; ++j) wf[SET][j] = *reinterpret_cast<const bf16x8*>(st + (ACH + wn * NT + j) * 1024);
#pragma unroll
        for (int i = 0; i < MBW; ++i) af[SET][i] = *reinterpret_cast<const bf16x8*>(st + (wm * MBW + i) * 1024);
    };
    auto multiply = [&](auto set_tag) {
        constexpr int SET = decltype(set_tag)::value;
#pragma unroll
        for (int j = 0; j < NT; ++j)
#pragma unroll
            for (int i = 0; i < MBW; ++i) acc[j][i] = __builtin_amdgcn_mfma_f32_32x32x16_bf16(wf[SET][j], af[SET][i], acc[j][i], 0, 0, 0);
    };
    auto wait_stage = [&](int younger) {
        constexpr int MAXY = (63 / CPW) < (NSTAGE - 1) ? (63 / CPW) : (NSTAGE - 1);
        if (MAXY >= 5 && younger >= 5) wait_vmcnt<MAXY >= 5 ? CPW * 5 : 0>();
        else if (MAXY >= 4 && younger >= 4) wait_vmcnt<MAXY >= 4 ? CPW * 4 : 0>();
        else if (MAXY >= 3 && younger >= 3) wait_vmcnt<MAXY >= 3 ? CPW * 3 : 0>();
        else if (MAXY >= 2 && younger >= 2) wait_vmcnt<MAXY >= 2 ? CPW * 2 : 0>();
        else if (MAXY >= 1 && younger >= 1) wait_vmcnt<CPW>();
        else wait_vmcnt<0>();
    };
    const bool early = NW < 8 || wave < NW / 2 || HQT_TILE_STAGGER == 0;
    if (NLOAD > 0 && loader) {
        wait_stage(NSTAGE - 1);
        __builtin_amdgcn_s_barrier();
        int slot = 0;
        for (int kt = 0; kt < KT - 1; ++kt) {
            wait_stage(min(NSTAGE - 2, KT - 2 - kt));
            __builtin_amdgcn_s_barrier();
            if (kt + NSTAGE < KT) issue(slot);
            slot = slot + 1 == NSTAGE ? 0 : slot + 1;
        }
        return;
    }
    if (NLOAD == 0) wait_stage(NSTAGE - 1);
    __builtin_amdgcn_s_barrier();
    __builtin_amdgcn_sched_barrier(0);
#ifdef HQT_TILE_STAMPS
    stamp[2] = clock64();
#endif
    __builtin_amdgcn_s_waitcnt(0xC07F);
    read_frags(std::integral_constant<int, 0>{}, 0, 0);
    int rd = 0;
    auto stage = [&](auto par_tag, auto last_tag, int kt) {
        constexpr int P = decltype(par_tag)::value;
        constexpr bool LAST = decltype(last_tag)::value;
#pragma unroll
        for (int ku = 0; ku < KU; ++ku) {
            const bool cur1 = ((P + ku) & 1) != 0;
            if (ku < KU - 1) {
                if (cur1) { read_frags(std::integral_constant<int, 0>{}, rd, ku + 1); __builtin_amdgcn_sched_barrier(0); multiply(std::integral_constant<int, 1>{}); }
                else { read_frags(std::integral_constant<int, 1>{}, rd, ku + 1); __builtin_amdgcn_sched_barrier(0); multiply(std::integral_constant<int, 0>{}); }
                __builtin_amdgcn_sched_barrier(0);
            } else {
                const int nxt = rd + 1 == NSTAGE ? 0 : rd + 1;
                if (!LAST) {
                    if (NLOAD == 0) wait_stage(min(NSTAGE - 2, KT - 2 - kt));
                    asm volatile("s_waitcnt lgkmcnt(0)" ::: "memory");
                    __builtin_amdgcn_s_barrier();
                    __builtin_amdgcn_sched_barrier(0);
                    if (NLOAD == 0 && early && kt + NSTAGE < KT) issue(rd);
                    if (cur1) read_frags(std::integral_constant<int, 0>{}, nxt, 0);
                    else read_frags(std::integral_constant<int, 1>{}, nxt, 0);
                    __builtin_amdgcn_sched_barrier(0);
                }
                if (cur1) multiply(std::integral_constant<int, 1>{});
                else multiply(std::integral_constant<int, 0>{});
                __builtin_amdgcn_sched_barrier(0);
                if (NLOAD == 0 && !LAST && !early && kt + NSTAGE < KT) issue(rd);
                __builtin_amdgcn_sched_barrier(0);
                rd = nxt;
            }
        }
    };
    constexpr std::integral_constant<int, 0> P0{};
    constexpr std::integral_constant<int, 1> P1{};
    constexpr std::false_type MORE{};
    constexpr std::true_type FINAL{};
    if (KU % 2 == 0) {
        for (int kt = 0; kt < KT - 1; ++kt) stage(P0, MORE, kt);
        stage(P0, FINAL, KT - 1);
    } else {
        int kt = 0;
        for (; kt + 2 < KT; kt += 2) { stage(P0, MORE, kt); stage(P1, MORE, kt + 1); }
        if (kt + 2 == KT) { stage(P0, MORE, kt); stage(P1, FINAL, kt + 1); }
        else stage(P0, FINAL, kt);
    }

#ifdef HQT_TILE_STAMPS
    __builtin_amdgcn_sched_barrier(0);
    asm volatile("s_nop 15\n\ts_nop 15" ::: "memory");
    stamp[3] = clock64();
    __builtin_amdgcn_sched_barrier(0);
#endif
    const int c = lane & 31, h = lane >> 5;
    const int Mc = g.c_packed_mb * 32;
    constexpr int WCOLS = 32 * NT, PITCH = WCOLS + 4;
    float* const stg = reinterpret_cast<float*>(lds) + wave * (32 * PITCH);
    static_assert(NC * 32 * PITCH * 4 <= G::RING_BYTES, "staging patches fit the ring");
    float mean[MBW], rstd[MBW];
#pragma unroll
    for (int i = 0; i < MBW; ++i) {
        mean[i] = DLN ? meanrstd[2 * ((wm * MBW + i) * 32 + c)] : 0.0f;
        rstd[i] = DLN ? meanrstd[2 * ((wm * MBW + i) * 32 + c) + 1] : 1.0f;
    }
    const int qkv_part_local = STORE == TS_QKV ? n0 / max(g.qkv_D, 1) : 0;
    const int qkv_part = qkv_part_local + g.qkv_first;
    bf16_t* const qkv_base = reinterpret_cast<bf16_t*>(qkv_part == 0 ? g.C : (qkv_part == 1 ? g.C2 : g.C3));
    bf16_t* const qkv_vcopy = (STORE == TS_QKV && qkv_part == 2) ? g.qkv_v_pk : nullptr;
    const auto rs_qkv = __builtin_amdgcn_make_buffer_rsrc(qkv_base, 0, 0xFFFFFFFF, 0x00020000);
    float* const slab_out = STORE == TS_SLAB ? slabs + (size_t)z * (MB * 32) * g.N : nullptr;
    const auto rs_slab = __builtin_amdgcn_make_buffer_rsrc(STORE == TS_FUSED ? slabs : nullptr, 0, 0xFFFFFFFF, 0x00020000);
    const unsigned slab_stride = (unsigned)((size_t)(MB * 32) * g.N * 4);
    float rs[MBW], rq[MBW];
#pragma unroll
    for (int i = 0; i < MBW; ++i) rs[i] = rq[i] = 0.0f;
    const int wcol0 = n0 + wn * WCOLS;
    if (STORE != TS_PACKED) __syncthreads();
    static_assert(STORE != TS_FUSED || (!DLN && G::NLOAD >= 0), "TS_FUSED: plain residual producers");
#ifdef HQT_TILE_STAMPS
    __builtin_amdgcn_sched_barrier(0);
    stamp[5] = clock64();
    __builtin_amdgcn_sched_barrier(0);
#endif
    auto run_epilogue = [&](auto mode_c, auto from_slabs_c) {
    constexpr int MODE = decltype(mode_c)::value;
    constexpr bool FROM_SLABS = decltype(from_slabs_c)::value;
#pragma unroll
    for (int i = 0; i < MBW; ++i) {
        const int mrow0 = m0 + (wm * MBW + i) * 32;
#pragma unroll
        for (int j = 0; j < NT; ++j)
#pragma unroll
            for (int q4 = 0; q4 < 4; ++q4) {
                if (FROM_SLABS) continue;
                const int cl = j * 32 + 8 * q4 + 4 * h;
                float v[4];
                if (MODE == TS_SLAB) {
#pragma unroll
                    for (int e = 0; e < 4; ++e) v[e] = acc[j][i][4 * q4 + e];
                } else {
                    const f32x4 b4 = *reinterpret_cast<const f32x4*>(colb + wn * WCOLS + cl);
                    const f32x4 cs4 = *reinterpret_cast<const f32x4*>(colb + BN + wn * WCOLS + cl);
#pragma unroll
                    for (int e = 0; e < 4; ++e) {
                        float t = acc[j][i][4 * q4 + e];
                        if (DLN) t = rstd[i] * (t - mean[i] * cs4[e]);
                        v[e] = t * g.alpha + b4[e];
                    }
                }
                if (MODE == TS_PACKED) {
#pragma unroll
                    for (int e = 0; e < 4; ++e) v[e] = tile_act<ACT>(v[e]);
                    if (mrow0 + c < g.M) st4<bf16_t>(reinterpret_cast<bf16_t*>(g.C) + packed_off(mrow0 + c, wcol0 + cl, g.c_packed_mb), v);
                    continue;
                }
                if (MODE == TS_ROWS) {
#pragma unroll
                    for (int e = 0; e < 4; ++e) v[e] = tile_act<ACT>(v[e]);
                }
                if (qkv_vcopy && mrow0 + c < g.M) st4<bf16_t>(qkv_vcopy + packed_off(mrow0 + c, wcol0 + cl - qkv_part_local * g.qkv_D, g.c_packed_mb), v);
                *reinterpret_cast<f32x4*>(stg + c * PITCH + cl) = f32x4{v[0], v[1], v[2], v[3]};
            }
        if (MODE == TS_PACKED) continue;
        __builtin_amdgcn_fence(__ATOMIC_ACQ_REL, "wavefront");
        __builtin_amdgcn_wave_barrier();
        if (MODE == TS_SLAB || MODE == TS_RESID || (MODE == TS_ROWS && sizeof(TC) == 4)) {
            constexpr int LPR = WCOLS / 4, RPP = 64 / LPR, NP = 32 / RPP;
            const int cg = (lane % LPR) * 4, r0 = lane / LPR;
            float* const out = MODE == TS_SLAB ? slab_out : reinterpret_cast<float*>(g.C);
            const int ldo = MODE == TS_SLAB ? g.N : g.ldc;
            f32x4 x0[NP];
            if (MODE == TS_RESID) {
#pragma unroll
                for (int p = 0; p < NP; ++p) {
                    const int m = min(mrow0 + p * RPP + r0, g.M - 1);
                    x0[p] = *reinterpret_cast<const f32x4*>(out + (size_t)m * ldo + wcol0 + cg);
                }
            }
            if (FROM_SLABS) {
                const f32x4 b4 = *reinterpret_cast<const f32x4*>(colb + wn * WCOLS + cg);
                constexpr int HP = NP / 2;
#pragma unroll
                for (int hp = 0; hp < 2; ++hp) {
                    u32x4 pz[8][HP];
#pragma unroll
                    for (int p = 0; p < HP; ++p) {
                        const int m = min(mrow0 + (hp * HP + p) * RPP + r0, g.M - 1);
                        const unsigned boff = (unsigned)(((size_t)m * g.N + wcol0 + cg) * 4);
#pragma unroll
                        for (int zz = 0; zz < 8; ++zz)
                            if (zz < S) pz[zz][p] = __builtin_amdgcn_raw_buffer_load_b128(rs_slab, boff + (unsigned)zz * slab_stride, 0, 16);
                    }
#pragma unroll
                    for (int p = 0; p < HP; ++p) {
                        const int r = (hp * HP + p) * RPP + r0, m = mrow0 + r;
                        f32x4 sum = __builtin_bit_cast(f32x4, pz[0][p]);
#pragma unroll
                        for (int zz = 1; zz < 8; ++zz)
                            if (zz < S) sum += __builtin_bit_cast(f32x4, pz[zz][p]);
                        f32x4 v = x0[hp * HP + p];
                        v += sum + b4;
                        *reinterpret_cast<f32x4*>(stg + r * PITCH + cg) = v;
                        if (m < g.M) *reinterpret_cast<f32x4*>(out + (size_t)m * ldo + wcol0 + cg) = v;
                    }
                }
            } else {
#pragma unroll
            for (int p = 0; p < NP; ++p) {
                const int r = p * RPP + r0, m = mrow0 + r;
                f32x4 v = *reinterpret_cast<const f32x4*>(stg + r * PITCH + cg);
                if (MODE == TS_RESID) {
                    v += x0[p];
                    *reinterpret_cast<f32x4*>(stg + r * PITCH + cg) = v;
                }
                if (MODE == TS_SLAB && STORE == TS_FUSED) {
                    if (m < g.M) __builtin_amdgcn_raw_buffer_store_b128(__builtin_bit_cast(u32x4, v), rs_slab, (unsigned)(((size_t)m * g.N + wcol0 + cg) * 4) + (unsigned)z * slab_stride, 0, 16);
                } else if (m < g.M) *reinterpret_cast<f32x4*>(out + (size_t)m * ldo + wcol0 + cg) = v;
            }
            }
        } else {
            constexpr int LPR = WCOLS / 8, RPP = 64 / LPR, NP = 32 / RPP;
            const int cg = (lane % LPR) * 8, r0 = lane / LPR;
#pragma unroll
            for (int p = 0; p < NP; ++p) {
                const int r = p * RPP + r0, m = mrow0 + r;
                const f32x4 a = *reinterpret_cast<const f32x4*>(stg + r * PITCH + cg), b = *reinterpret_cast<const f32x4*>(stg + r * PITCH + cg + 4);
                uint4 pk;
                pk.x = (unsigned)f32_to_bf16(a[0]) | ((unsigned)f32_to_bf16(a[1]) << 16);
                pk.y = (unsigned)f32_to_bf16(a[2]) | ((unsigned)f32_to_bf16(a[3]) << 16);
                pk.z = (unsigned)f32_to_bf16(b[0]) | ((unsigned)f32_to_bf16(b[1]) << 16);
                pk.w = (unsigned)f32_to_bf16(b[2]) | ((unsigned)f32_to_bf16(b[3]) << 16);
                if (m >= g.M) continue;
                if (MODE == TS_QKV) {
                    long long row = m;
                    if (qkv_part > 0) row = (long long)(m / g.rows_per_group) * g.group_stride + m % g.rows_per_group + g.row_offset + qkv_row_dev;
                    const long long eoff = row * g.ldc + (wcol0 + cg - qkv_part_local * g.qkv_D);
                    if (eoff < (1ll << 30)) __builtin_amdgcn_raw_buffer_store_b128(__builtin_bit_cast(u32x4, pk), rs_qkv, (unsigned)(eoff * 2), 0, 16);
                    else *reinterpret_cast<uint4*>(qkv_base + eoff) = pk;
                } else {
                    *reinterpret_cast<uint4*>(reinterpret_cast<bf16_t*>(g.C) + (long long)m * g.ldc + wcol0 + cg) = pk;
                }
            }
        }
        __builtin_amdgcn_fence(__ATOMIC_ACQ_REL, "wavefront");
        __builtin_amdgcn_wave_barrier();
        if (MODE == TS_RESID) {
#pragma unroll
            for (int j = 0; j < NT; ++j)
#pragma unroll
                for (int q4 = 0; q4 < 4; ++q4) {
                    const int cl = j * 32 + 8 * q4 + 4 * h;
                    const f32x4 x4 = *reinterpret_cast<const f32x4*>(stg + c * PITCH + cl);
                    if (mrow0 + c < g.M) {
                        bf16_t hb[4];
#pragma unroll
                        for (int e = 0; e < 4; ++e) {
                            hb[e] = f32_to_bf16(x4[e]);
                            const float r = bf16_to_f32(hb[e]);
                            rs[i] += r; rq[i] += r * r;
                        }
                        uint2 pk;
                        pk.x = (unsigned)hb[0] | ((unsigned)hb[1] << 16);
                        pk.y = (unsigned)hb[2] | ((unsigned)hb[3] << 16);
                        *reinterpret_cast<uint2*>(g.resid_pk + packed_off(mrow0 + c, wcol0 + cl, g.c_packed_mb)) = pk;
                    }
                }
            __builtin_amdgcn_fence(__ATOMIC_ACQ_REL, "wavefront");
            __builtin_amdgcn_wave_barrier();
        }
    }
    };
    if (STORE != TS_FUSED) run_epilogue(std::integral_constant<int, STORE>{}, std::false_type{});
    else {
        run_epilogue(std::integral_constant<int, TS_SLAB>{}, std::false_type{});
        asm volatile("s_waitcnt vmcnt(0)" ::: "memory");
        __syncthreads();
        unsigned* const ctr = g.tile_ctr + (tile_m * TN + tile_n);
        if (threadIdx.x == 0) {
            const unsigned t = __hip_atomic_fetch_add(ctr, 1u, __ATOMIC_RELAXED, __HIP_MEMORY_SCOPE_AGENT);
            if (t + 1u == (unsigned)S) __hip_atomic_store(ctr, 0u, __ATOMIC_RELAXED, __HIP_MEMORY_SCOPE_AGENT);
            reinterpret_cast<volatile unsigned*>(scratch)[0] = t;
        }
        __syncthreads();
        const unsigned ticket = reinterpret_cast<volatile unsigned*>(scratch)[0];
        if (ticket + 1u != (unsigned)S) return;
        __syncthreads();
        run_epilogue(std::integral_constant<int, TS_RESID>{}, std::true_type{});
    }
#ifdef HQT_TILE_STAMPS
    __builtin_amdgcn_sched_barrier(0);
    stamp[6] = clock64();
    __builtin_amdgcn_sched_barrier(0);
#endif
    if (STORE == TS_RESID || STORE == TS_FUSED) {
        float* red = reinterpret_cast<float*>(lds) + NC * 32 * PITCH;
        static_assert((NC * 32 * PITCH + G::WGN * BM * 2) * 4 <= G::RING_BYTES, "statistics scratch fits behind the staging patches");
#pragma unroll
        for (int i = 0; i < MBW; ++i) {
            const float a = rs[i] + __shfl_xor(rs[i], 32, 64), b = rq[i] + __shfl_xor(rq[i], 32, 64);
            if (h == 0) {
                red[2 * (wn * BM + (wm * MBW + i) * 32 + c)] = a;
                red[2 * (wn * BM + (wm * MBW + i) * 32 + c) + 1] = b;
            }
        }
        __syncthreads();
        for (int r = threadIdx.x; r < BM; r += NC * 64) {
            float a = 0.0f, b = 0.0f;
#pragma unroll
            for (int w = 0; w < G::WGN; ++w) { a += red[2 * (w * BM + r)]; b += red[2 * (w * BM + r) + 1]; }
            if (m0 + r < Mc) {
                float* pp = g.resid_parts + ((size_t)tile_n * Mc + m0 + r) * 2;
                pp[0] = a; pp[1] = b;
            }
        }
    }
#ifdef HQT_TILE_STAMPS
    if (g.am_best && threadIdx.x == 0) {
        asm volatile("s_waitcnt vmcnt(0)" ::: "memory");
        long long* dbg = reinterpret_cast<long long*>(g.am_best) + (size_t)blockIdx.x * 8;
        dbg[0] = stamp[0]; dbg[1] = stamp[2] - stamp[1]; dbg[2] = stamp[3] - stamp[1]; dbg[3] = clock64() - stamp[1]; dbg[4] = wall_clock64();
        dbg[5] = stamp[5] - stamp[1]; dbg[6] = stamp[6] - stamp[1];
    }
#endif
#endif
}

template <int S, int NT>
__global__ __launch_bounds__(NT) void resid_combine_kernel(float* __restrict__ x, const float* __restrict__ slabs, const float* __restrict__ bias,
                                                           bf16_t* __restrict__ xpk, float* __restrict__ parts, int M, int N, int slab_rows, int pk_mb) {
    __shared__ float red[2 * (NT / 64)];
    const int m = blockIdx.x;
    float rs = 0.0f, rq = 0.0f;
    for (int n4 = threadIdx.x * 4; n4 < N; n4 += NT * 4) {
        f32x4 p[S];
#pragma unroll
        for (int zz = 0; zz < S; ++zz) p[zz] = __builtin_nontemporal_load(reinterpret_cast<const f32x4*>(slabs + ((size_t)zz * slab_rows + m) * N + n4));
        f32x4 v = *reinterpret_cast<const f32x4*>(x + (size_t)m * N + n4);
        const f32x4 b = bias ? *reinterpret_cast<const f32x4*>(bias + n4) : f32x4{0.f, 0.f, 0.f, 0.f};
        f32x4 sum = p[0];
#pragma unroll
        for (int zz = 1; zz < S; ++zz) sum += p[zz];
        v += sum + b;
        *reinterpret_cast<f32x4*>(x + (size_t)m * N + n4) = v;
        bf16_t hb[4];
#pragma unroll
        for (int e = 0; e < 4; ++e) {
            hb[e] = f32_to_bf16(v[e]);
            const float r = bf16_to_f32(hb[e]);
            rs += r; rq += r * r;
        }
        uint2 pk;
        pk.x = (unsigned)hb[0] | ((unsigned)hb[1] << 16);
        pk.y = (unsigned)hb[2] | ((unsigned)hb[3] << 16);
        *reinterpret_cast<uint2*>(xpk + packed_off(m, n4, pk_mb)) = pk;
    }
#pragma unroll
    for (int off = 32; off > 0; off >>= 1) { rs += __shfl_xor(rs, off, 64); rq += __shfl_xor(rq, off, 64); }
    constexpr int NWV = NT / 64;
    if ((threadIdx.x & 63) == 0) { red[threadIdx.x >> 6] = rs; red[NWV + (threadIdx.x >> 6)] = rq; }
    __syncthreads();
    if (threadIdx.x == 0) {
        float a = 0.0f, b = 0.0f;
#pragma unroll
        for (int w = 0; w < NWV; ++w) { a += red[w]; b += red[NWV + w]; }
        parts[2 * m] = a;
        parts[2 * m + 1] = b;
    }
}

typedef TileGeom<2, 2, 2, 2, 2, 3> Tile128;
typedef TileGeom<2, 2, 1, 2, 2, 3> Tile64;
typedef TileGeom<2, 4, 1, 1, 4, 3> Tile64W8;
typedef TileGeom<2, 2, 2, 2, 2, 4, 4> Tile128PC;
typedef TileGeom<2, 2, 1, 1, 4, 3> Tile64x64;

template <class G, int STORE, bool DLN, typename TC, int ACT = ACT_NONE>
static hipError_t launch_tile_t(const GemmArgs& g, const bf16_t* wpk, int S, float* slabs, hipStream_t st) {
    const int TM = (g.M + G::BM - 1) / G::BM, TN = (g.N + G::BN - 1) / G::BN;
    tile_gemm_kernel<G, STORE, DLN, TC, ACT><<<TM * TN * S, G::NW * 64, G::LDS_BYTES, st>>>(g, reinterpret_cast<const char*>(wpk), slabs, TM, TN);
    return hipGetLastError();
}
template <class G, bool DLN>
static hipError_t launch_tile_packed(const GemmArgs& g, const bf16_t* wpk, hipStream_t st) {
    switch (g.act) {
    case ACT_NONE: return launch_tile_t<G, TS_PACKED, DLN, bf16_t, ACT_NONE>(g, wpk, 1, nullptr, st);
    case ACT_GELU_ERF: return launch_tile_t<G, TS_PACKED, DLN, bf16_t, ACT_GELU_ERF>(g, wpk, 1, nullptr, st);
    case ACT_GELU_SIGMOID: return launch_tile_t<G, TS_PACKED, DLN, bf16_t, ACT_GELU_SIGMOID>(g, wpk, 1, nullptr, st);
    }
    return hipErrorInvalidValue;
}

template <class G>
static hipError_t launch_tile_g(const GemmArgs& g, const bf16_t* wpk, int c_dt, int S, float* slabs, hipStream_t st) {
    const bool dln = g.ln_parts != nullptr;
    if (S > 1) return launch_tile_t<G, TS_SLAB, false, float>(g, wpk, S, slabs, st);
    switch (g.store) {
    case STORE_QKV: return dln ? launch_tile_t<G, TS_QKV, true, bf16_t>(g, wpk, 1, nullptr, st) : launch_tile_t<G, TS_QKV, false, bf16_t>(g, wpk, 1, nullptr, st);
    case STORE_PACKED: return dln ? launch_tile_packed<G, true>(g, wpk, st) : launch_tile_packed<G, false>(g, wpk, st);
    case STORE_RESID: return launch_tile_t<G, TS_RESID, false, float>(g, wpk, 1, nullptr, st);
    case STORE_ROWS:
        if (c_dt == DT_F32) return dln ? launch_tile_t<G, TS_ROWS, true, float>(g, wpk, 1, nullptr, st) : launch_tile_t<G, TS_ROWS, false, float>(g, wpk, 1, nullptr, st);
        return dln ? launch_tile_t<G, TS_ROWS, true, bf16_t>(g, wpk, 1, nullptr, st) : launch_tile_t<G, TS_ROWS, false, bf16_t>(g, wpk, 1, nullptr, st);
    }
    return hipErrorInvalidValue;
}

bool tile_gemm_ok(const GemmArgs& g, int a_dt, int c_dt) {
    if (!(g.a_packed_mb >= 16 && a_dt == DT_BF16 && !g.conv_taps && g.batch <= 1 && g.M >= 512)) return false;
    if (g.N % 128 != 0 || g.K % 32 != 0 || g.K < 256 || g.ldc % 8 != 0 || g.resid) return false;
    if (g.act != ACT_NONE && g.store != STORE_PACKED) return false;
    if (g.store == STORE_QKV) return c_dt == DT_BF16 && g.qkv_D % 128 == 0 && g.rows_per_group > 0;
    if (g.store == STORE_PACKED) return c_dt == DT_BF16 && g.c_packed_mb > 0;
    if (g.store == STORE_RESID) return c_dt == DT_F32 && g.c_packed_mb > 0 && !g.ln_parts && g.resid_pk && g.resid_parts && g.N == g.ldc && (g.K >= 3072 || g.M >= 640);
    if (g.store == STORE_ROWS) return g.rows_per_group == 0 && g.act == ACT_NONE;
    return false;
}

TilePlan tile_gemm_plan(const GemmArgs& g) {
    constexpr int max_s = 8;
    TilePlan p{0, Tile128::BM, Tile128::BN, 1};
    const int KS = g.K / 16, tiles = ((g.M + p.bm - 1) / p.bm) * (g.N / p.bn);
    if (g.store == STORE_RESID && g.K < 3072 && ((g.M + 63) / 64) * (g.N / 64) <= 256 && KS % Tile64x64::KU == 0 && KS / Tile64x64::KU >= 2 * Tile64x64::NSTAGE)
        return TilePlan{3, 64, 64, 1};
    if (g.store != STORE_RESID && tiles >= 160 && tiles <= 256 && KS % Tile128PC::KU == 0 && KS / Tile128PC::KU >= 2 * Tile128PC::NSTAGE)
        return TilePlan{4, Tile128PC::BM, Tile128PC::BN, 1};
    if (g.store != STORE_RESID && tiles < 256 && KS / Tile64::KU >= Tile64::NSTAGE) {
        const int t64 = ((g.M + Tile64::BM - 1) / Tile64::BM) * (g.N / Tile64::BN);
        if (t64 <= 512 && KS % Tile64W8::KU == 0 && KS / Tile64W8::KU >= 2 * Tile64W8::NSTAGE) return TilePlan{2, Tile64::BM, Tile64::BN, 1};
        return TilePlan{1, Tile64::BM, Tile64::BN, 1};
    }
    if (g.store == STORE_RESID && g.K < 3072 && tiles < 256 && KS % Tile64W8::KU == 0 && KS / Tile64W8::KU >= 2 * Tile64W8::NSTAGE)
        return TilePlan{2, Tile64::BM, Tile64::BN, 1};
    if (g.store == STORE_RESID && g.K >= 3072 && tiles >= 160 && tiles <= 256 && KS % Tile128PC::KU == 0 && KS / Tile128PC::KU >= 2 * Tile128PC::NSTAGE)
        return TilePlan{4, Tile128PC::BM, Tile128PC::BN, 1};
    if (g.store == STORE_RESID && g.K >= 3072 && tiles < 256) {
        const int t64 = ((g.M + Tile64::BM - 1) / Tile64::BM) * (g.N / Tile64::BN);
        if (((t64 >= 176 && t64 <= 208) || (t64 >= 448 && t64 <= 512)) && KS % Tile64W8::KU == 0 && KS / Tile64W8::KU >= 2 * Tile64W8::NSTAGE)
            return TilePlan{2, Tile64::BM, Tile64::BN, 1};
        if ((tiles * 4 <= 256 || tiles % 64 == 0) && KS % (Tile128::KU * 4) == 0 && KS / 4 / Tile128::KU >= 2 * Tile128::NSTAGE) {
            p.S = 4;
            if (tiles * 4 <= 256 && KS / 4 / Tile128PC::KU >= 2 * Tile128PC::NSTAGE) p.geom = 4;
            return p;
        }
        for (int S : {8, 6, 4, 3, 2})
            if (S <= max_s && tiles * S <= 576 && KS % (Tile128::KU * S) == 0 && KS / S / Tile128::KU >= 2 * Tile128::NSTAGE) { p.S = S; break; }
    }
    return p;
}

hipError_t launch_tile_gemm(const GemmArgs& g, const bf16_t* wpk, int a_dt, int c_dt, const TilePlan& p, float* slabs, hipStream_t st) {
    (void)a_dt;
    const GemmArgs& gg = g;
    if (p.geom == 0) return launch_tile_g<Tile128>(gg, wpk, c_dt, p.S, slabs, st);
    if (p.geom == 1) return launch_tile_g<Tile64>(gg, wpk, c_dt, p.S, slabs, st);
    if (p.geom == 2) return launch_tile_g<Tile64W8>(gg, wpk, c_dt, p.S, slabs, st);
    if (p.geom == 3) return launch_tile_g<Tile64x64>(gg, wpk, c_dt, p.S, slabs, st);
    if (p.geom == 4) return launch_tile_g<Tile128PC>(gg, wpk, c_dt, p.S, slabs, st);
    return hipErrorInvalidValue;
}

hipError_t launch_resid_combine(const GemmArgs& g, const float* slabs, int S, hipStream_t st) {
    float* x = reinterpret_cast<float*>(g.C);
    const int rows = g.a_packed_mb * 32;
    switch (S) {
#define COMBINE(S_) case S_:                                                                                                                          \
        if (g.N == 1536) resid_combine_kernel<S_, 384><<<g.M, 384, 0, st>>>(x, slabs, g.bias, g.resid_pk, g.resid_parts, g.M, g.N, rows, g.c_packed_mb);     \
        else resid_combine_kernel<S_, 256><<<g.M, 256, 0, st>>>(x, slabs, g.bias, g.resid_pk, g.resid_parts, g.M, g.N, rows, g.c_packed_mb);                 \
        break;
    COMBINE(2) COMBINE(3) COMBINE(4) COMBINE(6) COMBINE(8)
#undef COMBINE
    default: return hipErrorInvalidValue;
    }
    return hipGetLastError();
}

template <class G, int STORE, bool DLN, typename TC, int ACT = ACT_NONE>
static hipError_t configure_one() {
    void (*kernel)(GemmArgs, const char*, float*, int, int) = tile_gemm_kernel<G, STORE, DLN, TC, ACT>;
    return hipFuncSetAttribute(reinterpret_cast<const void*>(kernel), hipFuncAttributeMaxDynamicSharedMemorySize, G::LDS_BYTES);
}
template <class G>
static hipError_t configure_g() {
    hipError_t e;
#define CFG(STORE, DLN, TC)                      \
    e = configure_one<G, STORE, DLN, TC>();      \
    if (e != hipSuccess) return e;
    CFG(TS_QKV, true, bf16_t) CFG(TS_QKV, false, bf16_t) CFG(TS_PACKED, true, bf16_t) CFG(TS_PACKED, false, bf16_t)
    CFG(TS_RESID, false, float) CFG(TS_ROWS, true, float) CFG(TS_ROWS, false, float) CFG(TS_ROWS, true, bf16_t) CFG(TS_ROWS, false, bf16_t)
    CFG(TS_SLAB, false, float)
#undef CFG
    for (hipError_t e2 : {configure_one<G, TS_PACKED, true, bf16_t, ACT_GELU_ERF>(), configure_one<G, TS_PACKED, false, bf16_t, ACT_GELU_ERF>(),
                          configure_one<G, TS_PACKED, true, bf16_t, ACT_GELU_SIGMOID>(), configure_one<G, TS_PACKED, false, bf16_t, ACT_GELU_SIGMOID>()})
        if (e2 != hipSuccess) return e2;
    return hipSuccess;
}
hipError_t tile_gemm_configure() {
    hipError_t e = configure_g<Tile128>();
    if (e == hipSuccess) e = configure_g<Tile64>();
    if (e == hipSuccess) e = configure_g<Tile64W8>();
    if (e == hipSuccess) e = configure_g<Tile64x64>();
    if (e == hipSuccess) e = configure_g<Tile128PC>();
    return e;
}
```

hqtransformer_amd/engine.py:

```python
from __future__ import annotations

import ctypes as C
import weakref
from typing import Dict, List, Optional, Sequence, Tuple

import numpy as np
import torch

from . import _lib
from ._lib import PRECISION_EXACT, PRECISION_FAST, hqt_config, hqt_encode_out, hqt_guide_pair, hqt_row_sampler, hqt_sample_opts, hqt_sample_opts_l3
from .spec import DEPTH_DECODINGS, STAGE1_RESAMPLES, Stage1Spec, Stage2Spec


def _ptr(t: Optional[torch.Tensor]) -> Optional[int]:
    return None if t is None else t.data_ptr()


def make_config(s2: Optional[Stage2Spec], s1: Optional[Stage1Spec], max_batch: int, max_steps: int, ar_layouts: int = 0) -> hqt_config:
    c = hqt_config()
    c.abi_version = _lib.ABI_VERSION
    c.max_batch = int(max_batch)
    c.max_steps = int(max_steps)
    c.ar_layouts = int(ar_layouts)
    if s2 is not None:
# ... 109 lines not shown
                             'run on request only: pass text_prefix=True')
        if s2.depth_decoding == 'bidirectional':
            raise ValueError("a code prefix with text conditioning is built for the two-level 'parallel' depth head; the 'bidirectional' head "
                             "with text conditioning is not built at all (the reference's own step does not pick the last text token)")
        if s2.levels == 3:
            raise ValueError("a code prefix with text conditioning is built for two code levels (the 'parallel' depth head); three code levels "
                             'with text conditioning are not')
    L = s2.levels
    if not isinstance(prefix, (list, tuple)) or len(prefix) != L:
        raise ValueError(f'prefix: expected the {L} code levels as one list, coarse to fine')
    levels = [torch.as_tensor(p) for p in prefix]
    if levels[0].dim() != 2 or int(levels[0].shape[0]) != int(batch):
        raise ValueError(f'prefix[0]: expected shape ({int(batch)}, P), got {tuple(levels[0].shape)}')
    P = int(levels[0].shape[1])
    if P < 1 or P >= int(n_steps):
        raise ValueError(f'prefix of P={P} positions: P must lie in [1, n_steps - 1 = {int(n_steps) - 1}] (at least one position is left to draw)')
    if max_prefix is not None and P > int(max_prefix):
        raise ValueError(f'prefix of P={P} positions exceeds max_prefix={int(max_prefix)} of this engine')
    for l, t in enumerate(levels):
        want = (int(batch), P) + ((4 ** l,) if l else ())
        if tuple(t.shape) != want:
            raise ValueError(f'prefix[{l}]: expected shape {want}, got {tuple(t.shape)}')
        if t.dtype.is_floating_point or t.dtype == torch.bool:
            raise ValueError(f'prefix[{l}]: expected integer codes, got {t.dtype}')
        if not t.is_cuda:
            lo, hi = int(t.min()), int(t.max())
            if lo < 0 or hi >= s2.vocab_top:
                raise IndexError(f'prefix[{l}]: index out of range (values span [{lo}, {hi}], table has {s2.vocab_top} rows)')
    return levels


def keep_leading_run(mask, max_prefix: int, text_l3: bool = False) -> int:
    m = np.asarray(torch.as_tensor(mask).cpu() if isinstance(mask, torch.Tensor) else mask).astype(bool)
    if m.ndim != 2 or m.shape[0] < 1 or m.shape[1] < 1:
        raise ValueError(f'keep mask: expected shape (B, n), got {m.shape}')
    if text_l3:
        return 0
    run = np.where(m.all(axis=1), m.shape[1], np.argmin(m, axis=1))
    return int(max(0, min(int(run.min()), int(max_prefix), m.shape[1] - 1)))


def check_keep(s2: Stage2Spec, batch: int, n_steps: int, keep) -> Optional[tuple]:
    if keep is None:
        return None
    if not isinstance(keep, (list, tuple)) or len(keep) != 2:
        raise ValueError('keep: expected (mask [B, n], codes: the code levels as one list)')
    mask, codes = keep
    m = torch.as_tensor(mask).cpu()
    if tuple(m.shape) != (int(batch), int(n_steps)):
        raise ValueError(f'keep mask: expected shape {(int(batch), int(n_steps))}, got {tuple(m.shape)}')
    if m.dtype.is_floating_point:
        raise ValueError(f'keep mask: expected bool (or 0 / 1 integers), got {m.dtype}')
    m = np.ascontiguousarray((m != 0).numpy().astype(np.uint8))
    L = s2.levels
    if not isinstance(codes, (list, tuple)) or len(codes) != L:
        raise ValueError(f'kept codes: expected the {L} code levels as one list, coarse to fine')
    levels = [torch.as_tensor(c) for c in codes]
    for l, t in enumerate(levels):
        want = (int(batch), int(n_steps)) + ((4 ** l,) if l else ())
        if tuple(t.shape) != want:
            raise ValueError(f'kept codes[{l}]: expected shape {want}, got {tuple(t.shape)}')
        if t.dtype.is_floating_point or t.dtype == torch.bool:
            raise ValueError(f'kept codes[{l}]: expected integer codes, got {t.dtype}')
        if not t.is_cuda and m.any():
            sel = t[torch.from_numpy(m.astype(bool))]
            lo, hi = int(sel.min()), int(sel.max())
            if lo < 0 or hi >= s2.vocab_top:
                raise IndexError(f'kept codes[{l}]: index out of range (values span [{lo}, {hi}], table has {s2.vocab_top} rows)')
    return m, levels


def check_score_codes(s2: Stage2Spec, codes, what: str = 'one-pass scoring') -> int:
    if s2.depth_decoding == 'top2mid2bot':
        raise ValueError(f"{what}: the 'top2mid2bot' depth head runs 21 causal sub-steps per position and is scored stepwise only: use one_pass=False")
    if s2.cond == 2 and s2.levels == 3:
        raise ValueError(f'{what}: text conditioning with three code levels is not built (two code levels are): use one_pass=False')
    L = s2.levels
    if not isinstance(codes, (list, tuple)) or len(codes) != L:
        raise ValueError(f'codes: expected the {L} code levels as one list, coarse to fine')
    levels = [torch.as_tensor(c) for c in codes]
    if levels[0].dim() != 2 or int(levels[0].shape[1]) < 1:
        raise ValueError(f'codes[0]: expected shape (B, n), got {tuple(levels[0].shape)}')
    B, n = (int(v) for v in levels[0].shape)
    if n > s2.ctx_len_img:
        raise ValueError(f'codes of n={n} positions: the model has ctx_len_img={s2.ctx_len_img}')
    for l, t in enumerate(levels):
        want = (B, n) + ((4 ** l,) if l else ())
        if tuple(t.shape) != want:
            raise ValueError(f'codes[{l}]: expected shape {want}, got {tuple(t.shape)}')
        if t.dtype.is_floating_point or t.dtype == torch.bool:
            raise ValueError(f'codes[{l}]: expected integer codes, got {t.dtype}')
        if not t.is_cuda:
            lo, hi = int(t.min()), int(t.max())
            if lo < 0 or hi >= s2.vocab_top:
                raise IndexError(f'codes[{l}]: index out of range (values span [{lo}, {hi}], table has {s2.vocab_top} rows)')
    return n


class Engine:

    def __init__(self, s2: Optional[Stage2Spec], s1: Optional[Stage1Spec], device: torch.device, max_batch: int,
                 max_steps: Optional[int] = None, ar_layouts: int = 0, max_prefix: int = 0, score_chunk: int = 0):
        self.lib = _lib.load()
        self.s2, self.s1 = s2, s1
        self.device = torch.device(device)
        if self.device.type != 'cuda':
            raise _lib.HqtLibraryError(f'libhqt runs on an MI355X only; got device {self.device} (no CPU fallback)')
        self.max_batch = int(max_batch)
        self.max_steps = int(max_steps if max_steps is not None else (s2.ctx_len_img if s2 else 1))
        self.max_prefix = int(max_prefix)
        self.cfg = make_config(s2, s1, self.max_batch, self.max_steps, ar_layouts)
        h = C.c_void_p()
        _lib.check(self.lib.hqt_create(C.byref(self.cfg), self.device.index or 0, C.byref(h)))
        self.h = h
        self.finalized = False
        if self.max_prefix:
            with torch.cuda.device(self.device):
                _lib.check(self.lib.hqt_set_max_prefix(self.h, self.max_prefix))
        self.score_chunk = int(score_chunk)
        if self.score_chunk:
            with torch.cuda.device(self.device):
                _lib.check(self.lib.hqt_set_score_chunk(self.h, self.score_chunk))
        self.policy = _lib.POLICY_LATENCY

    def clone(self) -> 'Engine':
        if not self.finalized:
            raise _lib.HqtError(-1, 'clone() needs a finalized engine')
        e = Engine.__new__(Engine)
        e.lib, e.s2, e.s1, e.device = self.lib, self.s2, self.s1, self.device
        e.max_batch, e.max_steps, e.max_prefix, e.cfg = self.max_batch, self.max_steps, self.max_prefix, self.cfg
        e.score_chunk = self.score_chunk
        h = C.c_void_p()
        _lib.check(self.lib.hqt_clone(self.h, C.byref(h)))
        e.h, e.finalized = h, True
        e.policy = _lib.POLICY_LATENCY
        e._parent = self
        self._clones = getattr(self, '_clones', [])
        self._clones.append(e)
        return e

    def set_policy(self, policy: int) -> None:
        _lib.check(self.lib.hqt_set_policy(self.h, int(policy)))
        self.policy = int(policy)

    def set_persist(self, on: bool) -> None:
        _lib.check(self.lib.hqt_set_switch(self.h, _lib.SWITCH_PERSIST, int(bool(on))))

    def set_persist_fault(self, cu_plus_one: int) -> None:
        with torch.cuda.device(self.device):
            _lib.check(self.lib.hqt_set_switch(self.h, _lib.SWITCH_PERSIST_FAULT, int(cu_plus_one)))

    def set_split_kslices(self, on: bool) -> None:
        _lib.check(self.lib.hqt_set_switch(self.h, _lib.SWITCH_SPLIT_KSLICES, int(bool(on))))

    def set_single_key(self, on: bool) -> None:
        _lib.check(self.lib.hqt_set_switch(self.h, _lib.SWITCH_SINGLE_KEY, int(bool(on))))

    def _note_split(self, precision: int, stream: int, ar_rows: int = 0) -> None:
        if int(precision) == _lib.PRECISION_SPLIT or (int(precision) == _lib.PRECISION_FAST and 0 < ar_rows <= 64):
            self._split_streams = getattr(self, '_split_streams', set()) | {int(stream or 0)}

    def range_check(self) -> None:
        streams, self._split_streams = getattr(self, '_split_streams', set()), set()
        err = None
        with torch.cuda.device(self.device):
            for st in sorted(streams):
                try:
                    _lib.check(self.lib.hqt_range_check(self.h, C.c_void_p(st)))
                except _lib.HqtError as e:
                    err = e
        if err is not None:
            raise err

    def close(self) -> None:
        for c in getattr(self, '_clones', []):
            c.close()
        self._clones = []
        if getattr(self, 'h', None) is not None and self.h.value:
            self.lib.hqt_destroy(self.h)
            self.h = C.c_void_p()

    def __del__(self):
        try:
            self.close()
        except Exception:
            pass

    def set_weight(self, name: str, t) -> None:
        if isinstance(t, np.ndarray):
            t = torch.from_numpy(np.ascontiguousarray(t, dtype=np.float32))
        t = t.detach().to(dtype=torch.float32).contiguous()
        shape = (C.c_int64 * t.dim())(*t.shape)
        _lib.check(self.lib.hqt_set_weight(self.h, name.encode(), C.c_void_p(t.data_ptr()), 0, shape, t.dim()))

    def load(self, stage2: Optional[Dict[str, object]] = None, stage1: Optional[Dict[str, object]] = None) -> None:
        for prefix, sd in (('stage2.', stage2), ('stage1.', stage1)):
            for k, v in (sd or {}).items():
                self.set_weight(prefix + k, v)

    def finalize(self) -> None:
        _lib.check(self.lib.hqt_finalize_weights(self.h))
        self.finalized = True

    @staticmethod
    def _ident(t: torch.Tensor) -> tuple:
        return (t.data_ptr(), tuple(t.shape), tuple(t.stride()), t.dtype)

    def _trust(self, *tensors, bound: int) -> None:
        for t in tensors:
            if t is not None:
                _TRUSTED[self._ident(t)] = (t._version, weakref.ref(t.untyped_storage()), int(bound))
                if len(_TRUSTED) > 256:
                    _TRUSTED.pop(next(iter(_TRUSTED)))

    def _check_index(self, t: Optional[torch.Tensor], n: int, what: str) -> None:
        if t is None or t.numel() == 0:
            return
        seen = _TRUSTED.get(self._ident(t)) if t.is_cuda else None
        if seen is not None and seen[0] == t._version and seen[1]() is t.untyped_storage() and seen[2] <= n:
            return
        lo, hi = (int(v) for v in torch.stack([t.min(), t.max()]).tolist())
        if lo < 0 or hi >= n:
            raise IndexError(f'{what}: index out of range (values span [{lo}, {hi}], table has {n} rows)')
        if t.is_cuda:
            self._trust(t, bound=hi + 1)

    @staticmethod
    def _check_out(t: torch.Tensor, shape, dtype, dev, what: str) -> torch.Tensor:
        if not isinstance(t, torch.Tensor) or tuple(t.shape) != tuple(shape) or t.dtype != dtype or t.device != dev or not t.is_contiguous():
            raise ValueError(f'{what}: expected a contiguous {dtype} tensor of shape {tuple(shape)} on {dev}, got '
                             f'{getattr(t, "dtype", type(t))} {tuple(getattr(t, "shape", ()))} on {getattr(t, "device", "?")}')
        return t

    @staticmethod
    def _row_keys(o, B: int, row_seeds, row_offsets):
        if row_seeds is None and row_offsets is None:
            return None
        if row_seeds is None or row_offsets is None or len(row_seeds) != B or len(row_offsets) != B:
            raise ValueError(f'row_seeds and row_offsets come together, {B} entries each')
        rs = (C.c_uint64 * B)(*[int(v) & (2 ** 64 - 1) for v in row_seeds])
        ro = (C.c_int64 * B)(*[int(v) for v in row_offsets])
        o.row_seeds, o.row_offsets = C.cast(rs, C.c_void_p), C.cast(ro, C.c_void_p)
        return rs, ro

    def _prep(self, t, shape, dtype, what: str, table: int = 0) -> Optional[torch.Tensor]:
        if t is None:
            return None
        t = torch.as_tensor(t)
        if tuple(t.shape) != tuple(shape):
            raise ValueError(f'{what}: expected shape {tuple(shape)}, got {tuple(t.shape)}')
        if table:
            self._check_index(t, table, what)
        return t.to(device=self.device, dtype=dtype).contiguous()

    def _prep_cond(self, cond, B: int) -> Optional[torch.Tensor]:
        if self.s2.cond == 1:
            return self._prep(cond, (B,), torch.int64, 'cond (class ids)', self.s2.n_classes)
        if self.s2.cond == 2:
            return self._prep(cond, (B, self.s2.ctx_len_txt), torch.int64, 'cond (text token ids)', self.s2.vocab_txt)
        return None

    def _sample_levels(self, levels: int, batch: int, cond, n_steps: int, *, precision, top_k, top_p, temperature, noise, seed, sample_offset,
                       force: Sequence[Optional[torch.Tensor]], out: Optional[Sequence[torch.Tensor]], return_logits, use_graph,
                       row_seeds, row_offsets, row_samplers=None, prefix=None,
                       return_logprobs=False, guidance=None, keep=None,
                       prompt_groups=None) -> Tuple[List[torch.Tensor], Optional[torch.Tensor], Optional[torch.Tensor]]:
        dev = self.device
        B, V, L = int(batch), self.s2.vocab_top, int(levels)
        groups = None if prompt_groups is None else check_prompt_groups(self.s2, B, cond, prompt_groups, self.max_batch, prefix, keep)
        prefix = check_prefix(self.s2, B, n_steps, prefix, self.max_prefix, text_prefix=True)
        P = 0 if prefix is None else int(prefix[0].shape[1])
        keep = check_keep(self.s2, B, n_steps, keep)
        if keep is not None:
            if prefix is not None:
                raise ValueError('keep and prefix: a prefix is a leading run of the keep mask -- put it there')
            for f, what in zip(force, _FORCE_NAMES[L]):
                if f is not None:
                    raise ValueError(f'{what} together with keep is not built: put the forced codes into the kept codes')
            P = keep_leading_run(keep[0], self.max_prefix, text_l3=self.s2.cond == 2 and L == 3)
        draws = (4 ** L - 1) // 3
        shapes = [(B, n_steps) + ((4 ** l,) if l else ()) for l in range(L)]
        o = hqt_sample_opts() if L == 2 else hqt_sample_opts_l3()
        o.precision, o.n_steps = int(precision), int(n_steps)
        for i in range(L):
            k, p, t = int(top_k[i]) if top_k[i] else 0, float(top_p[i]) if top_p[i] else 0.0, float(temperature[i])
            if L == 2:
                for field, v in (('top_k', k), ('top_p', p), ('temperature', t)):
                    setattr(o, f'{field}_{("top", "bot")[i]}', v)
            else:
                o.top_k[i], o.top_p[i], o.temperature[i] = k, p, t
        o.seed, o.sample_offset, o.use_graph = int(seed) & (2 ** 64 - 1), int(sample_offset), int(bool(use_graph))
        rows = self._row_keys(o, B, row_seeds, row_offsets)
        table = None if row_samplers is None else row_sampler_table(L, row_samplers)
        pairs = guide_pair_table(L, guidance) if guidance is not None and len(guidance) else None
        if pairs is not None:
            check_guided_rows(B, len(pairs), self.max_batch)
        cond = self._prep_cond(cond, B if groups is None else groups[1])
        noise = self._prep(noise, (n_steps, draws, B, V), torch.float32, 'noise')
        force = [self._prep(f, shp, torch.int64, what, V) for f, shp, what in zip(force, shapes, _FORCE_NAMES[L])]
        if keep is not None:
            sel = torch.from_numpy(keep[0].astype(bool))

            def kept(t, shp, what):
                if t.is_cuda and sel.any():
                    try:
                        self._check_index(t, V, what)
# ... 202 lines not shown
```

include/hqt.h:

```cpp
#ifndef HQT_H
#define HQT_H

#include <stdint.h>

#ifdef __cplusplus
extern "C" {
#endif

#define HQT_ABI_VERSION 9

typedef enum {
    HQT_OK = 0,
    HQT_ERR_INVALID = -1,
    HQT_ERR_HIP = -2,
    HQT_ERR_STATE = -3,
    HQT_ERR_UNKNOWN_WEIGHT = -4,
    HQT_ERR_SHAPE = -5,
    HQT_ERR_MISSING_WEIGHT = -6,
    HQT_ERR_RANGE = -7
} hqt_status;

enum { HQT_COND_NONE = 0, HQT_COND_CLASS = 1, HQT_COND_TEXT = 2 };
enum { HQT_EMB_TRANSFORMER1 = 0, HQT_EMB_REDUCE = 1 };
enum { HQT_PRECISION_EXACT = 0, HQT_PRECISION_FAST = 1, HQT_PRECISION_SPLIT = 2 };
enum { HQT_DTYPE_F32 = 0 };

typedef struct hqt_handle hqt_handle;

typedef struct {
    int32_t abi_version;
    int32_t has_stage2;
    int32_t embed_dim, n_layers, n_heads, n_layers_depth;
    int32_t vocab_top, vocab_bot, vocab_txt;
    int32_t ctx_len_img, ctx_len_txt, n_classes;
    int32_t cond_type;
    int32_t embedding_type;
    int32_t gelu_approx;
    int32_t has_stage1;
    int32_t s1_ch, s1_n_mult, s1_ch_mult[8];
    int32_t s1_num_res_blocks;
    int32_t s1_n_attn_res, s1_attn_res[4];
    int32_t s1_resolution, s1_z_channels, s1_embed_dim, s1_n_embed, s1_out_ch;
    int32_t s1_use_init_downsample, s1_use_mid_block, s1_use_attn;
    int32_t max_batch;
    int32_t max_steps;
    int32_t code_levels;
    int32_t depth_decoding;
    int32_t ar_layouts;
    int32_t s1_resample;
} hqt_config;
#define HQT_RESAMPLE_PIXELSHUFFLE 0
#define HQT_RESAMPLE_NEAREST 1
#define HQT_RESAMPLE_CONV2 2
#define HQT_LAYOUT_FAST 1
#define HQT_LAYOUT_EXACT 2
#define HQT_LAYOUT_SPLIT 4
#define HQT_LAYOUT_ALL 7
#define HQT_DEPTH_PARALLEL_ADD 0
#define HQT_DEPTH_PARALLEL 1
#define HQT_DEPTH_PARALLEL_REDUCE 2
#define HQT_DEPTH_TOP2MID2BOT 3
#define HQT_DEPTH_BIDIRECTIONAL 4

typedef struct {
    int32_t precision;
    int32_t n_steps;
    int32_t top_k_top, top_k_bot;
    float top_p_top, top_p_bot;
    float temperature_top, temperature_bot;
    uint64_t seed;
    int64_t sample_offset;
    int32_t use_graph;
    const uint64_t* row_seeds;
    const int64_t* row_offsets;
} hqt_sample_opts;

int hqt_create(const hqt_config* cfg, int device, hqt_handle** out);

int hqt_set_weight(hqt_handle* h, const char* name, const void* data, int dtype, const int64_t* shape, int ndim);

int hqt_finalize_weights(hqt_handle* h);

int hqt_clone(hqt_handle* src, hqt_handle** out);

enum { HQT_POLICY_LATENCY = 0, HQT_POLICY_THROUGHPUT = 1 };
int hqt_set_policy(hqt_handle* h, int policy);

enum { HQT_SWITCH_PERSIST = 0, HQT_SWITCH_SINGLE_KEY = 1, HQT_SWITCH_PERSIST_FAULT = 2, HQT_SWITCH_SPLIT_KSLICES = 3 };
int hqt_set_switch(hqt_handle* h, int which, int on);

typedef struct { float temperature[3]; int32_t top_k[3]; float top_p[3]; } hqt_row_sampler;
int hqt_set_row_samplers(hqt_handle* h, int n, const hqt_row_sampler* rows);

int hqt_set_logprob_out(hqt_handle* h, float* logprobs);

typedef struct { int32_t pos_row, neg_row; float scale[3]; } hqt_guide_pair;
int hqt_set_guidance(hqt_handle* h, int n_pairs, const hqt_guide_pair* pairs);

int hqt_set_keep_mask(hqt_handle* h, int B, int n_steps, const uint8_t* keep, const int64_t* const* codes);

int hqt_set_prompt_groups(hqt_handle* h, int B, int n_groups, const int32_t* group_of_row);

int hqt_sample(hqt_handle* h, int B, const int64_t* cond, const hqt_sample_opts* opts, const float* noise,
               const int64_t* force_top, const int64_t* force_bot, float* logits_out,
               int64_t* out_top, int64_t* out_bot, void* stream);

typedef struct {
    int32_t precision, n_steps;
    int32_t top_k[3];
    float top_p[3];
    float temperature[3];
    uint64_t seed;
    int64_t sample_offset;
    int32_t use_graph;
    const uint64_t* row_seeds;
    const int64_t* row_offsets;
} hqt_sample_opts_l3;
int hqt_sample_l3(hqt_handle* h, int B, const int64_t* cond, const hqt_sample_opts_l3* opts, const float* noise,
                  const int64_t* force0, const int64_t* force1, const int64_t* force2, float* logits_out,
                  int64_t* out0, int64_t* out1, int64_t* out2, void* stream);
int hqt_set_max_prefix(hqt_handle* h, int max_prefix);

int hqt_sample_prefix(hqt_handle* h, int B, const int64_t* cond, const hqt_sample_opts* opts, const float* noise,
                      int prefix_len, const int64_t* prefix_top, const int64_t* prefix_bot,
                      const int64_t* force_top, const int64_t* force_bot, float* logits_out,
                      int64_t* out_top, int64_t* out_bot, void* stream);
int hqt_sample_prefix_l3(hqt_handle* h, int B, const int64_t* cond, const hqt_sample_opts_l3* opts, const float* noise,
                         int prefix_len, const int64_t* prefix0, const int64_t* prefix1, const int64_t* prefix2,
                         const int64_t* force0, const int64_t* force1, const int64_t* force2, float* logits_out,
                         int64_t* out0, int64_t* out1, int64_t* out2, void* stream);
int hqt_set_score_chunk(hqt_handle* h, int pairs);
int hqt_score(hqt_handle* h, int B, const int64_t* cond, const int64_t* const* codes, int n, int precision, float* logprobs,
              float* const* logits_out, void* stream);
int hqt_decode_l3(hqt_handle* h, int B, const int64_t* code_t, const int64_t* code_m, const int64_t* code_b, float* out_pixels,
                  int clamp01, int precision, void* stream);
int hqt_decode_seq_l3(hqt_handle* h, int B, const int64_t* codes0, const int64_t* codes1, const int64_t* codes2, float* out_pixels,
                      int clamp01, int precision, void* stream);

typedef struct {
    int64_t* codes[3];
    float* quant[3];
    float* resid[3];
    float* recon;
    float* diff;
} hqt_encode_out;
int hqt_encode(hqt_handle* h, int B, const float* pixels, int precision, const hqt_encode_out* out, void* stream);
int hqt_has_encoder(const hqt_handle* h);

int hqt_decode(hqt_handle* h, int B, const int64_t* code_t, const int64_t* code_b, float* out_pixels,
               int clamp01, int precision, void* stream);
int hqt_decode_seq(hqt_handle* h, int B, const int64_t* codes_top, const int64_t* codes_bot, float* out_pixels,
                   int clamp01, int precision, void* stream);

int hqt_range_check(hqt_handle* h, void* stream);

int hqt_abi_version(void);
int64_t hqt_param_count(const hqt_handle* h, int stage);
int64_t hqt_workspace_bytes(const hqt_handle* h);
int hqt_timing_enable(hqt_handle* h, int on);
int hqt_timing_reset(hqt_handle* h);
int hqt_timing_get(hqt_handle* h, int slot, char* name, int name_len, int64_t* launches, double* total_ms);
int hqt_timing_slots(const hqt_handle* h);

int hqt_destroy(hqt_handle* h);
const char* hqt_last_error(void);

#ifdef __cplusplus
}
#endif
#endif
```

Measured before the change: 1714.

## Add 16x16x32 bf16 MFMA path to tile GEMM for large unsplit tiles

Adds a templated variant of the tile GEMM kernel that uses 16x16x32 bf16 MFMA instructions with f32x4 accumulators in place of the 32x32 fragments. It comes with a new LDS fragment read schedule and a remapped epilogue covering row/column quads, LayerNorm statistics and residual reductions. A planner heuristic turns it on by default for the 128-tile geometry without split-K, and for residual stores only when K is at least 3072. An env var and a runtime switch control it, and the switch value is folded into the graph key. The aim is higher MFMA throughput or better register use on MI355X, at the cost of twice the kernel instantiations and a more complex software pipeline.

```diff
diff --git a/hqtransformer_amd/_lib.py b/hqtransformer_amd/_lib.py
--- a/hqtransformer_amd/_lib.py
+++ b/hqtransformer_amd/_lib.py
@@ -14,7 +14,7 @@
 PRECISION_EXACT, PRECISION_FAST, PRECISION_SPLIT = 0, 1, 2
 PRECISIONS = {'exact': PRECISION_EXACT, 'fast': PRECISION_FAST, 'split': PRECISION_SPLIT}
 POLICY_LATENCY, POLICY_THROUGHPUT = 0, 1
-SWITCH_PERSIST, SWITCH_SINGLE_KEY, SWITCH_PERSIST_FAULT, SWITCH_SPLIT_KSLICES = 0, 1, 2, 3
+SWITCH_PERSIST, SWITCH_SINGLE_KEY, SWITCH_PERSIST_FAULT, SWITCH_SPLIT_KSLICES, SWITCH_TILE_MFMA16 = 0, 1, 2, 3, 4
 LAYOUT_FAST, LAYOUT_EXACT, LAYOUT_SPLIT, LAYOUT_ALL = 1, 2, 4, 7
 RESAMPLE_PIXELSHUFFLE, RESAMPLE_NEAREST, RESAMPLE_CONV2 = 0, 1, 2
 
diff --git a/hqtransformer_amd/csrc/engine.hip b/hqtransformer_amd/csrc/engine.hip
--- a/hqtransformer_amd/csrc/engine.hip
+++ b/hqtransformer_amd/csrc/engine.hip
@@ -197,6 +197,7 @@
     bool persist_tripped = false;
     bool single_key = true;
     bool split_kslices = true;
+    int tile_mfma16 = 1;
     bool capture_persist = false;
     bool graph_has_persist = false;
     int layouts = 0;
@@ -367,6 +368,7 @@
     { const char* e = getenv("HQT_PERSIST"); h->persist_enabled = !(e && atoi(e) == 0); }
     h->single_key = getenv("HQT_NO_SINGLE_KEY") == nullptr;
     h->split_kslices = getenv("HQT_SPLIT_KSLICES_OFF") == nullptr;
+    { const char* e = getenv("HQT_TILE_MFMA16"); h->tile_mfma16 = e ? std::min(std::max(atoi(e), 0), 2) : 1; }
     h->cfg = *cfg;
     h->layouts = (cfg->ar_layouts & HQT_LAYOUT_ALL) ? (cfg->ar_layouts & HQT_LAYOUT_ALL) : HQT_LAYOUT_ALL;
     h->device = device;
@@ -1011,7 +1013,7 @@
     if (md.fast) {
         if (resid_nparts) *resid_nparts = g.N / 32;
         if ((g.ln_parts ? l.wpk_ln : l.wpk) && h->tile_gemm && tile_gemm_ok(g, a_dt, c_dt)) {
-            const TilePlan tp = tile_gemm_plan(g);
+            const TilePlan tp = tile_gemm_plan(g, h->tile_mfma16);
             if (tp.geom >= 0 && (size_t)tp.S * 32 * g.a_packed_mb * g.N <= h->splitk_elems) {
                 if (g.ln_parts) g.bias = l.bias_ln;
                 HIPCHK(launch_tile_gemm(g, g.ln_parts ? l.wpk_ln : l.wpk, a_dt, c_dt, tp, h->splitk, st));
@@ -2085,7 +2087,7 @@
         for (int d = std::min(gmax, remaining); d >= 1; --d) if (remaining % d == 0) { G = d; break; }
         std::vector<uint64_t> key = {(uint64_t)G, (uint64_t)B, (uint64_t)(c.cond != nullptr), (uint64_t)c.noise, (uint64_t)c.logits_out, (uint64_t)c.logprob_out,
                                      (uint64_t)c.precision, (uint64_t)c.n_steps, (uint64_t)c.levels, (uint64_t)h->policy,
-                                     (uint64_t)((h->persist_enabled && !h->persist_tripped ? 1 : 0) + (h->single_key ? 0 : 4) + (h->split_kslices ? 0 : 8))};
+                                     (uint64_t)((h->persist_enabled && !h->persist_tripped ? 1 : 0) + (h->single_key ? 0 : 4) + (h->split_kslices ? 0 : 8) + 16 * h->tile_mfma16)};
         for (const int64_t* f : c.feed) key.push_back((uint64_t)f);
         for (const SamplerSet& l : c.lv) {
             uint32_t f[2];
@@ -2604,6 +2606,7 @@
     if (which == HQT_SWITCH_PERSIST) { h->persist_enabled = on != 0; if (on) h->persist_tripped = false; }
     else if (which == HQT_SWITCH_SINGLE_KEY) h->single_key = on != 0;
     else if (which == HQT_SWITCH_SPLIT_KSLICES) h->split_kslices = on != 0;
+    else if (which == HQT_SWITCH_TILE_MFMA16) h->tile_mfma16 = std::min(std::max(on, 0), 2);
     else if (which == HQT_SWITCH_PERSIST_FAULT) {
         if (!h->persist_err) return fail(HQT_ERR_STATE, "no persistent chain on this handle (a lane, or a handle without stage 2)");
         ON_DEVICE(h);
diff --git a/hqtransformer_amd/csrc/fast_kernels.h b/hqtransformer_amd/csrc/fast_kernels.h
--- a/hqtransformer_amd/csrc/fast_kernels.h
+++ b/hqtransformer_amd/csrc/fast_kernels.h
@@ -14,10 +14,10 @@
 int stream_gemm_splitk(const GemmArgs& g);
 hipError_t launch_stream_gemm(const GemmArgs& g, const bf16_t* wpk, int a_dt, int c_dt, int S, float* slabs, hipStream_t st);
 
-struct TilePlan { int geom; int bm, bn; int S; };
+struct TilePlan { int geom; int bm, bn; int S; int m16; };
 constexpr int TILE_CTR_MAX = 4096;
 bool tile_gemm_ok(const GemmArgs& g, int a_dt, int c_dt);
-TilePlan tile_gemm_plan(const GemmArgs& g);
+TilePlan tile_gemm_plan(const GemmArgs& g, int mfma16 = 0);
 hipError_t launch_tile_gemm(const GemmArgs& g, const bf16_t* wpk, int a_dt, int c_dt, const TilePlan& p, float* slabs, hipStream_t st);
 hipError_t launch_resid_combine(const GemmArgs& g, const float* slabs, int S, hipStream_t st);
 hipError_t tile_gemm_configure();
diff --git a/hqtransformer_amd/csrc/tile_gemm.hip b/hqtransformer_amd/csrc/tile_gemm.hip
--- a/hqtransformer_amd/csrc/tile_gemm.hip
+++ b/hqtransformer_amd/csrc/tile_gemm.hip
@@ -76,7 +76,7 @@
     tm = first + in_group - tn * rows;
 }
 
-template <class G, int STORE, bool DLN, typename TC, int ACT = ACT_NONE>
+template <class G, int STORE, bool DLN, typename TC, int ACT = ACT_NONE, bool M16 = false>
 __global__ __launch_bounds__(G::NW * 64, (G::NW / 4) * G::WG_PER_CU) void tile_gemm_kernel(GemmArgs g, const char* __restrict__ wpk,
                                                                                               float* __restrict__ slabs, int TM, int TN) {
 #if defined(__HIP_DEVICE_COMPILE__)
@@ -138,13 +138,22 @@
         }
     };
 
-    f32x16 acc[NT][MBW];
-#pragma unroll
-    for (int j = 0; j < NT; ++j)
-#pragma unroll
-        for (int i = 0; i < MBW; ++i)
-#pragma unroll
-            for (int r = 0; r < 16; ++r) acc[j][i][r] = 0.0f;
+    constexpr int NWF = 2 * NT, NXF = 2 * MBW;
+    f32x16 acc[M16 ? 1 : NT][M16 ? 1 : MBW];
+    f32x4 acc4[M16 ? NWF : 1][M16 ? NXF : 1];
+    if constexpr (M16) {
+#pragma unroll
+        for (int jw = 0; jw < NWF; ++jw)
+#pragma unroll
+            for (int ix = 0; ix < NXF; ++ix) acc4[jw][ix] = f32x4{0.0f, 0.0f, 0.0f, 0.0f};
+    } else {
+#pragma unroll
+        for (int j = 0; j < NT; ++j)
+#pragma unroll
+            for (int i = 0; i < MBW; ++i)
+#pragma unroll
+                for (int r = 0; r < 16; ++r) acc[j][i][r] = 0.0f;
+    }
 
     float bias_r = 0.0f, cs_r = 0.0f;
     const int pc = min((int)threadIdx.x, BN - 1);
@@ -242,10 +251,10 @@
     __builtin_amdgcn_s_barrier();
     __builtin_amdgcn_sched_barrier(0);
 #ifdef HQT_TILE_STAMPS
-    stamp[2] = clock64();
+    stamp[2] = clock64(); stamp[4] = wall_clock64();
 #endif
     __builtin_amdgcn_s_waitcnt(0xC07F);
-    read_frags(std::integral_constant<int, 0>{}, 0, 0);
+    if constexpr (!M16) read_frags(std::integral_constant<int, 0>{}, 0, 0);
     int rd = 0;
     auto stage = [&](auto par_tag, auto last_tag, int kt) {
         constexpr int P = decltype(par_tag)::value;
@@ -282,6 +291,7 @@
     constexpr std::integral_constant<int, 1> P1{};
     constexpr std::false_type MORE{};
     constexpr std::true_type FINAL{};
+    if constexpr (!M16) {
     if (KU % 2 == 0) {
         for (int kt = 0; kt < KT - 1; ++kt) stage(P0, MORE, kt);
         stage(P0, FINAL, KT - 1);
@@ -291,11 +301,82 @@
         if (kt + 2 == KT) { stage(P0, MORE, kt); stage(P1, FINAL, kt + 1); }
         else stage(P0, FINAL, kt);
     }
+    } else {
+        static_assert(KU % 2 == 0, "M16: a step is two 16-k fragments");
+        constexpr int KS2 = KU / 2;
+        constexpr int W16DB = NLOAD > 0 ? 0 : 1, WIP = NWF - W16DB;
+        bf16x8 xf[2][NXF], wf16[2][NWF];
+        const char* const fb = lds + ((lane >> 5) * (CPS * 1024) + ((((lane >> 4) & 1) * 32 + (lane & 15)) * 16));
+        auto step_base = [&](int slot, int s) { return fb + slot * STAGE + s * (2 * CPS * 1024); };
+        auto read_w = [&](auto set_tag, int jw, const char* st) {
+            constexpr int SET = decltype(set_tag)::value;
+            wf16[SET][jw] = *reinterpret_cast<const bf16x8*>(st + (ACH + wn * NT + (jw >> 1)) * 1024 + (jw & 1) * 256);
+        };
+        auto read_top = [&](auto set_tag, const char* st) {
+            constexpr int SET = decltype(set_tag)::value;
+#pragma unroll
+            for (int ix = 0; ix < NXF; ++ix) xf[SET][ix] = *reinterpret_cast<const bf16x8*>(st + (wm * MBW + (ix >> 1)) * 1024 + (ix & 1) * 256);
+#pragma unroll
+            for (int jw = WIP; jw < NWF; ++jw) read_w(set_tag, jw, st);
+        };
+        auto mul_group = [&](auto set_tag, int jw) {
+            constexpr int SET = decltype(set_tag)::value;
+#pragma unroll
+            for (int ix = 0; ix < NXF; ++ix)
+                acc4[jw][ix] = __builtin_amdgcn_mfma_f32_16x16x32_bf16(wf16[jw < WIP ? 0 : SET][jw], xf[SET][ix], acc4[jw][ix], 0, 0, 0);
+        };
+#pragma unroll
+        for (int jw = 0; jw < WIP; ++jw) read_w(P0, jw, step_base(0, 0));
+        auto stage16 = [&](auto par_tag, int kt) {
+            constexpr int P = decltype(par_tag)::value;
+#pragma unroll
+            for (int s = 0; s < KS2; ++s) {
+                const bool cur1 = ((P + s) & 1) != 0, tail = s == KS2 - 1;
+                const int nxt = rd + 1 == NSTAGE ? 0 : rd + 1;
+                if (tail && kt < KT - 1) {
+                    if (NLOAD == 0) wait_stage(min(NSTAGE - 2, KT - 2 - kt));
+                    asm volatile("s_waitcnt lgkmcnt(0)" ::: "memory");
+                    __builtin_amdgcn_s_barrier();
+                    __builtin_amdgcn_sched_barrier(0);
+                    if (NLOAD == 0 && early && kt + NSTAGE < KT) issue(rd);
+                }
+                const char* const st = tail ? step_base(nxt, 0) : step_base(rd, s + 1);
+                if (cur1) read_top(P0, st);
+                else read_top(P1, st);
+                __builtin_amdgcn_sched_barrier(0);
+#pragma unroll
+                for (int jw = 0; jw < NWF; ++jw) {
+                    if (cur1) mul_group(P1, jw);
+                    else mul_group(P0, jw);
+                    __builtin_amdgcn_sched_barrier(0);
+                    if (jw < WIP) {
+                        read_w(P0, jw, st);
+                        __builtin_amdgcn_sched_barrier(0);
+                    }
+                }
+                if (tail) {
+                    if (NLOAD == 0 && !early && kt + NSTAGE < KT) issue(rd);
+                    __builtin_amdgcn_sched_barrier(0);
+                    rd = nxt;
+                }
+            }
+        };
+        if (KS2 % 2 == 0) {
+            read_top(P0, step_base(0, 0));
+            for (int kt = 0; kt < KT; ++kt) stage16(P0, kt);
+        } else {
+            int kt = 0;
+            if (KT & 1) { read_top(P1, step_base(0, 0)); stage16(P1, 0); kt = 1; }
+            else read_top(P0, step_base(0, 0));
+            for (; kt < KT; kt += 2) { stage16(P0, kt); stage16(P1, kt + 1); }
+        }
+        asm volatile("s_waitcnt lgkmcnt(0)" ::: "memory");
+    }
 
 #ifdef HQT_TILE_STAMPS
     __builtin_amdgcn_sched_barrier(0);
     asm volatile("s_nop 15\n\ts_nop 15" ::: "memory");
-    stamp[3] = clock64();
+    stamp[3] = clock64(); stamp[7] = wall_clock64();
     __builtin_amdgcn_sched_barrier(0);
 #endif
     const int c = lane & 31, h = lane >> 5;
@@ -303,12 +384,19 @@
     constexpr int WCOLS = 32 * NT, PITCH = WCOLS + 4;
     float* const stg = reinterpret_cast<float*>(lds) + wave * (32 * PITCH);
     static_assert(NC * 32 * PITCH * 4 <= G::RING_BYTES, "staging patches fit the ring");
-    float mean[MBW], rstd[MBW];
-#pragma unroll
-    for (int i = 0; i < MBW; ++i) {
-        mean[i] = DLN ? meanrstd[2 * ((wm * MBW + i) * 32 + c)] : 0.0f;
-        rstd[i] = DLN ? meanrstd[2 * ((wm * MBW + i) * 32 + c) + 1] : 1.0f;
-    }
+    constexpr int NQ = 4 * NT, RB = M16 ? 2 : 1;
+    const int c16 = lane & 15, h16 = lane >> 4;
+    auto quad_col = [&](int q) { return M16 ? 16 * (q >> 1) + 4 * h16 : (q >> 2) * 32 + 8 * (q & 3) + 4 * h; };
+    auto quad_row = [&](int q) { return M16 ? 16 * (q & 1) + c16 : c; };
+    float mean[MBW][RB], rstd[MBW][RB];
+#pragma unroll
+    for (int i = 0; i < MBW; ++i)
+#pragma unroll
+        for (int b = 0; b < RB; ++b) {
+            if (M16) continue;
+            mean[i][b] = DLN ? meanrstd[2 * ((wm * MBW + i) * 32 + quad_row(b))] : 0.0f;
+            rstd[i][b] = DLN ? meanrstd[2 * ((wm * MBW + i) * 32 + quad_row(b)) + 1] : 1.0f;
+        }
     const int qkv_part_local = STORE == TS_QKV ? n0 / max(g.qkv_D, 1) : 0;
     const int qkv_part = qkv_part_local + g.qkv_first;
     bf16_t* const qkv_base = reinterpret_cast<bf16_t*>(qkv_part == 0 ? g.C : (qkv_part == 1 ? g.C2 : g.C3));
@@ -317,9 +405,11 @@
     float* const slab_out = STORE == TS_SLAB ? slabs + (size_t)z * (MB * 32) * g.N : nullptr;
     const auto rs_slab = __builtin_amdgcn_make_buffer_rsrc(STORE == TS_FUSED ? slabs : nullptr, 0, 0xFFFFFFFF, 0x00020000);
     const unsigned slab_stride = (unsigned)((size_t)(MB * 32) * g.N * 4);
-    float rs[MBW], rq[MBW];
-#pragma unroll
-    for (int i = 0; i < MBW; ++i) rs[i] = rq[i] = 0.0f;
+    float rs[MBW][RB], rq[MBW][RB];
+#pragma unroll
+    for (int i = 0; i < MBW; ++i)
+#pragma unroll
+        for (int b = 0; b < RB; ++b) rs[i][b] = rq[i][b] = 0.0f;
     const int wcol0 = n0 + wn * WCOLS;
     if (STORE != TS_PACKED) __syncthreads();
     static_assert(STORE != TS_FUSED || (!DLN && G::NLOAD >= 0), "TS_FUSED: plain residual producers");
@@ -334,38 +424,46 @@
 #pragma unroll
     for (int i = 0; i < MBW; ++i) {
         const int mrow0 = m0 + (wm * MBW + i) * 32;
-#pragma unroll
-        for (int j = 0; j < NT; ++j)
-#pragma unroll
-            for (int q4 = 0; q4 < 4; ++q4) {
+        if (M16) {
+#pragma unroll
+            for (int b = 0; b < RB; ++b) {
+                mean[i][b] = DLN ? meanrstd[2 * ((wm * MBW + i) * 32 + quad_row(b))] : 0.0f;
+                rstd[i][b] = DLN ? meanrstd[2 * ((wm * MBW + i) * 32 + quad_row(b)) + 1] : 1.0f;
+            }
+        }
+#pragma unroll
+        for (int q = 0; q < NQ; ++q) {
                 if (FROM_SLABS) continue;
-                const int cl = j * 32 + 8 * q4 + 4 * h;
+                const int cl = quad_col(q), rr = quad_row(q), rb = M16 ? (q & 1) : 0;
+                float av[4];
+#pragma unroll
+                for (int e = 0; e < 4; ++e) av[e] = M16 ? acc4[M16 ? q >> 1 : 0][M16 ? 2 * i + (q & 1) : 0][e] : acc[M16 ? 0 : q >> 2][M16 ? 0 : i][4 * (q & 3) + e];
                 float v[4];
                 if (MODE == TS_SLAB) {
 #pragma unroll
-                    for (int e = 0; e < 4; ++e) v[e] = acc[j][i][4 * q4 + e];
+                    for (int e = 0; e < 4; ++e) v[e] = av[e];
                 } else {
                     const f32x4 b4 = *reinterpret_cast<const f32x4*>(colb + wn * WCOLS + cl);
                     const f32x4 cs4 = *reinterpret_cast<const f32x4*>(colb + BN + wn * WCOLS + cl);
 #pragma unroll
                     for (int e = 0; e < 4; ++e) {
-                        float t = acc[j][i][4 * q4 + e];
-                        if (DLN) t = rstd[i] * (t - mean[i] * cs4[e]);
+                        float t = av[e];
+                        if (DLN) t = rstd[i][rb] * (t - mean[i][rb] * cs4[e]);
                         v[e] = t * g.alpha + b4[e];
                     }
                 }
                 if (MODE == TS_PACKED) {
 #pragma unroll
                     for (int e = 0; e < 4; ++e) v[e] = tile_act<ACT>(v[e]);
-                    if (mrow0 + c < g.M) st4<bf16_t>(reinterpret_cast<bf16_t*>(g.C) + packed_off(mrow0 + c, wcol0 + cl, g.c_packed_mb), v);
+                    if (mrow0 + rr < g.M) st4<bf16_t>(reinterpret_cast<bf16_t*>(g.C) + packed_off(mrow0 + rr, wcol0 + cl, g.c_packed_mb), v);
                     continue;
                 }
                 if (MODE == TS_ROWS) {
 #pragma unroll
                     for (int e = 0; e < 4; ++e) v[e] = tile_act<ACT>(v[e]);
                 }
-                if (qkv_vcopy && mrow0 + c < g.M) st4<bf16_t>(qkv_vcopy + packed_off(mrow0 + c, wcol0 + cl - qkv_part_local * g.qkv_D, g.c_packed_mb), v);
-                *reinterpret_cast<f32x4*>(stg + c * PITCH + cl) = f32x4{v[0], v[1], v[2], v[3]};
+                if (qkv_vcopy && mrow0 + rr < g.M) st4<bf16_t>(qkv_vcopy + packed_off(mrow0 + rr, wcol0 + cl - qkv_part_local * g.qkv_D, g.c_packed_mb), v);
+                *reinterpret_cast<f32x4*>(stg + rr * PITCH + cl) = f32x4{v[0], v[1], v[2], v[3]};
             }
         if (MODE == TS_PACKED) continue;
         __builtin_amdgcn_fence(__ATOMIC_ACQ_REL, "wavefront");
@@ -452,23 +550,21 @@
         __builtin_amdgcn_wave_barrier();
         if (MODE == TS_RESID) {
 #pragma unroll
-            for (int j = 0; j < NT; ++j)
-#pragma unroll
-                for (int q4 = 0; q4 < 4; ++q4) {
-                    const int cl = j * 32 + 8 * q4 + 4 * h;
-                    const f32x4 x4 = *reinterpret_cast<const f32x4*>(stg + c * PITCH + cl);
-                    if (mrow0 + c < g.M) {
+            for (int q = 0; q < NQ; ++q) {
+                    const int cl = quad_col(q), rr = quad_row(q), rb = M16 ? (q & 1) : 0;
+                    const f32x4 x4 = *reinterpret_cast<const f32x4*>(stg + rr * PITCH + cl);
+                    if (mrow0 + rr < g.M) {
                         bf16_t hb[4];
 #pragma unroll
                         for (int e = 0; e < 4; ++e) {
                             hb[e] = f32_to_bf16(x4[e]);
                             const float r = bf16_to_f32(hb[e]);
-                            rs[i] += r; rq[i] += r * r;
+                            rs[i][rb] += r; rq[i][rb] += r * r;
                         }
                         uint2 pk;
                         pk.x = (unsigned)hb[0] | ((unsigned)hb[1] << 16);
                         pk.y = (unsigned)hb[2] | ((unsigned)hb[3] << 16);
-                        *reinterpret_cast<uint2*>(g.resid_pk + packed_off(mrow0 + c, wcol0 + cl, g.c_packed_mb)) = pk;
+                        *reinterpret_cast<uint2*>(g.resid_pk + packed_off(mrow0 + rr, wcol0 + cl, g.c_packed_mb)) = pk;
                     }
                 }
             __builtin_amdgcn_fence(__ATOMIC_ACQ_REL, "wavefront");
@@ -502,13 +598,19 @@
         float* red = reinterpret_cast<float*>(lds) + NC * 32 * PITCH;
         static_assert((NC * 32 * PITCH + G::WGN * BM * 2) * 4 <= G::RING_BYTES, "statistics scratch fits behind the staging patches");
 #pragma unroll
-        for (int i = 0; i < MBW; ++i) {
-            const float a = rs[i] + __shfl_xor(rs[i], 32, 64), b = rq[i] + __shfl_xor(rq[i], 32, 64);
-            if (h == 0) {
-                red[2 * (wn * BM + (wm * MBW + i) * 32 + c)] = a;
-                red[2 * (wn * BM + (wm * MBW + i) * 32 + c) + 1] = b;
-            }
-        }
+        for (int i = 0; i < MBW; ++i)
+#pragma unroll
+            for (int rb = 0; rb < RB; ++rb) {
+                float a = rs[i][rb], b = rq[i][rb];
+                if (M16) {
+                    a += __shfl_xor(a, 16, 64); b += __shfl_xor(b, 16, 64);
+                }
+                a += __shfl_xor(a, 32, 64); b += __shfl_xor(b, 32, 64);
+                if (M16 ? h16 == 0 : h == 0) {
+                    red[2 * (wn * BM + (wm * MBW + i) * 32 + quad_row(rb))] = a;
+                    red[2 * (wn * BM + (wm * MBW + i) * 32 + quad_row(rb)) + 1] = b;
+                }
+            }
         __syncthreads();
         for (int r = threadIdx.x; r < BM; r += NC * 64) {
             float a = 0.0f, b = 0.0f;
@@ -526,6 +628,7 @@
         long long* dbg = reinterpret_cast<long long*>(g.am_best) + (size_t)blockIdx.x * 8;
         dbg[0] = stamp[0]; dbg[1] = stamp[2] - stamp[1]; dbg[2] = stamp[3] - stamp[1]; dbg[3] = clock64() - stamp[1]; dbg[4] = wall_clock64();
         dbg[5] = stamp[5] - stamp[1]; dbg[6] = stamp[6] - stamp[1];
+        dbg[7] = stamp[7] - stamp[4];
     }
 #endif
 #endif
@@ -580,35 +683,40 @@
 typedef TileGeom<2, 2, 2, 2, 2, 4, 4> Tile128PC;
 typedef TileGeom<2, 2, 1, 1, 4, 3> Tile64x64;
 
-template <class G, int STORE, bool DLN, typename TC, int ACT = ACT_NONE>
+template <class G, int STORE, bool DLN, typename TC, int ACT = ACT_NONE, bool M16 = false>
 static hipError_t launch_tile_t(const GemmArgs& g, const bf16_t* wpk, int S, float* slabs, hipStream_t st) {
     const int TM = (g.M + G::BM - 1) / G::BM, TN = (g.N + G::BN - 1) / G::BN;
-    tile_gemm_kernel<G, STORE, DLN, TC, ACT><<<TM * TN * S, G::NW * 64, G::LDS_BYTES, st>>>(g, reinterpret_cast<const char*>(wpk), slabs, TM, TN);
+    tile_gemm_kernel<G, STORE, DLN, TC, ACT, M16><<<TM * TN * S, G::NW * 64, G::LDS_BYTES, st>>>(g, reinterpret_cast<const char*>(wpk), slabs, TM, TN);
     return hipGetLastError();
 }
-template <class G, bool DLN>
+template <class G, bool DLN, bool M16>
 static hipError_t launch_tile_packed(const GemmArgs& g, const bf16_t* wpk, hipStream_t st) {
     switch (g.act) {
-    case ACT_NONE: return launch_tile_t<G, TS_PACKED, DLN, bf16_t, ACT_NONE>(g, wpk, 1, nullptr, st);
-    case ACT_GELU_ERF: return launch_tile_t<G, TS_PACKED, DLN, bf16_t, ACT_GELU_ERF>(g, wpk, 1, nullptr, st);
-    case ACT_GELU_SIGMOID: return launch_tile_t<G, TS_PACKED, DLN, bf16_t, ACT_GELU_SIGMOID>(g, wpk, 1, nullptr, st);
+    case ACT_NONE: return launch_tile_t<G, TS_PACKED, DLN, bf16_t, ACT_NONE, M16>(g, wpk, 1, nullptr, st);
+    case ACT_GELU_ERF: return launch_tile_t<G, TS_PACKED, DLN, bf16_t, ACT_GELU_ERF, M16>(g, wpk, 1, nullptr, st);
+    case ACT_GELU_SIGMOID: return launch_tile_t<G, TS_PACKED, DLN, bf16_t, ACT_GELU_SIGMOID, M16>(g, wpk, 1, nullptr, st);
     }
     return hipErrorInvalidValue;
 }
 
-template <class G>
+template <class G, bool M16>
 static hipError_t launch_tile_g(const GemmArgs& g, const bf16_t* wpk, int c_dt, int S, float* slabs, hipStream_t st) {
     const bool dln = g.ln_parts != nullptr;
-    if (S > 1) return launch_tile_t<G, TS_SLAB, false, float>(g, wpk, S, slabs, st);
+    constexpr int A0 = ACT_NONE;
+    if (S > 1) return launch_tile_t<G, TS_SLAB, false, float, A0, M16>(g, wpk, S, slabs, st);
     switch (g.store) {
-    case STORE_QKV: return dln ? launch_tile_t<G, TS_QKV, true, bf16_t>(g, wpk, 1, nullptr, st) : launch_tile_t<G, TS_QKV, false, bf16_t>(g, wpk, 1, nullptr, st);
-    case STORE_PACKED: return dln ? launch_tile_packed<G, true>(g, wpk, st) : launch_tile_packed<G, false>(g, wpk, st);
-    case STORE_RESID: return launch_tile_t<G, TS_RESID, false, float>(g, wpk, 1, nullptr, st);
+    case STORE_QKV: return dln ? launch_tile_t<G, TS_QKV, true, bf16_t, A0, M16>(g, wpk, 1, nullptr, st) : launch_tile_t<G, TS_QKV, false, bf16_t, A0, M16>(g, wpk, 1, nullptr, st);
+    case STORE_PACKED: return dln ? launch_tile_packed<G, true, M16>(g, wpk, st) : launch_tile_packed<G, false, M16>(g, wpk, st);
+    case STORE_RESID: return launch_tile_t<G, TS_RESID, false, float, A0, M16>(g, wpk, 1, nullptr, st);
     case STORE_ROWS:
-        if (c_dt == DT_F32) return dln ? launch_tile_t<G, TS_ROWS, true, float>(g, wpk, 1, nullptr, st) : launch_tile_t<G, TS_ROWS, false, float>(g, wpk, 1, nullptr, st);
-        return dln ? launch_tile_t<G, TS_ROWS, true, bf16_t>(g, wpk, 1, nullptr, st) : launch_tile_t<G, TS_ROWS, false, bf16_t>(g, wpk, 1, nullptr, st);
+        if (c_dt == DT_F32) return dln ? launch_tile_t<G, TS_ROWS, true, float, A0, M16>(g, wpk, 1, nullptr, st) : launch_tile_t<G, TS_ROWS, false, float, A0, M16>(g, wpk, 1, nullptr, st);
+        return dln ? launch_tile_t<G, TS_ROWS, true, bf16_t, A0, M16>(g, wpk, 1, nullptr, st) : launch_tile_t<G, TS_ROWS, false, bf16_t, A0, M16>(g, wpk, 1, nullptr, st);
     }
     return hipErrorInvalidValue;
+}
+template <class G>
+static hipError_t launch_tile_shape(const GemmArgs& g, const bf16_t* wpk, int c_dt, const TilePlan& p, float* slabs, hipStream_t st) {
+    return p.m16 ? launch_tile_g<G, true>(g, wpk, c_dt, p.S, slabs, st) : launch_tile_g<G, false>(g, wpk, c_dt, p.S, slabs, st);
 }
 
 bool tile_gemm_ok(const GemmArgs& g, int a_dt, int c_dt) {
@@ -622,7 +730,7 @@
     return false;
 }
 
-TilePlan tile_gemm_plan(const GemmArgs& g) {
+static TilePlan tile_geom_plan(const GemmArgs& g) {
     constexpr int max_s = 8;
     TilePlan p{0, Tile128::BM, Tile128::BN, 1};
     const int KS = g.K / 16, tiles = ((g.M + p.bm - 1) / p.bm) * (g.N / p.bn);
@@ -654,14 +762,23 @@
     return p;
 }
 
+static bool tile_mfma16_wins(const TilePlan& p, const GemmArgs& g) {
+    return p.geom == 0 && p.S == 1 && (g.store != STORE_RESID || g.K >= 3072);
+}
+TilePlan tile_gemm_plan(const GemmArgs& g, int mfma16) {
+    TilePlan p = tile_geom_plan(g);
+    p.m16 = mfma16 >= 2 || (mfma16 == 1 && tile_mfma16_wins(p, g)) ? 1 : 0;
+    return p;
+}
+
 hipError_t launch_tile_gemm(const GemmArgs& g, const bf16_t* wpk, int a_dt, int c_dt, const TilePlan& p, float* slabs, hipStream_t st) {
     (void)a_dt;
     const GemmArgs& gg = g;
-    if (p.geom == 0) return launch_tile_g<Tile128>(gg, wpk, c_dt, p.S, slabs, st);
-    if (p.geom == 1) return launch_tile_g<Tile64>(gg, wpk, c_dt, p.S, slabs, st);
-    if (p.geom == 2) return launch_tile_g<Tile64W8>(gg, wpk, c_dt, p.S, slabs, st);
-    if (p.geom == 3) return launch_tile_g<Tile64x64>(gg, wpk, c_dt, p.S, slabs, st);
-    if (p.geom == 4) return launch_tile_g<Tile128PC>(gg, wpk, c_dt, p.S, slabs, st);
+    if (p.geom == 0) return launch_tile_shape<Tile128>(gg, wpk, c_dt, p, slabs, st);
+    if (p.geom == 1) return launch_tile_shape<Tile64>(gg, wpk, c_dt, p, slabs, st);
+    if (p.geom == 2) return launch_tile_shape<Tile64W8>(gg, wpk, c_dt, p, slabs, st);
+    if (p.geom == 3) return launch_tile_shape<Tile64x64>(gg, wpk, c_dt, p, slabs, st);
+    if (p.geom == 4) return launch_tile_shape<Tile128PC>(gg, wpk, c_dt, p, slabs, st);
     return hipErrorInvalidValue;
 }
 
@@ -682,8 +799,11 @@
 
 template <class G, int STORE, bool DLN, typename TC, int ACT = ACT_NONE>
 static hipError_t configure_one() {
-    void (*kernel)(GemmArgs, const char*, float*, int, int) = tile_gemm_kernel<G, STORE, DLN, TC, ACT>;
-    return hipFuncSetAttribute(reinterpret_cast<const void*>(kernel), hipFuncAttributeMaxDynamicSharedMemorySize, G::LDS_BYTES);
+    void (*kernel)(GemmArgs, const char*, float*, int, int) = tile_gemm_kernel<G, STORE, DLN, TC, ACT, false>;
+    void (*kernel16)(GemmArgs, const char*, float*, int, int) = tile_gemm_kernel<G, STORE, DLN, TC, ACT, true>;
+    const hipError_t e = hipFuncSetAttribute(reinterpret_cast<const void*>(kernel), hipFuncAttributeMaxDynamicSharedMemorySize, G::LDS_BYTES);
+    if (e != hipSuccess) return e;
+    return hipFuncSetAttribute(reinterpret_cast<const void*>(kernel16), hipFuncAttributeMaxDynamicSharedMemorySize, G::LDS_BYTES);
 }
 template <class G>
 static hipError_t configure_g() {
diff --git a/hqtransformer_amd/engine.py b/hqtransformer_amd/engine.py
--- a/hqtransformer_amd/engine.py
+++ b/hqtransformer_amd/engine.py
@@ -285,6 +285,9 @@
 
     def set_split_kslices(self, on: bool) -> None:
         _lib.check(self.lib.hqt_set_switch(self.h, _lib.SWITCH_SPLIT_KSLICES, int(bool(on))))
+
+    def set_tile_mfma16(self, on) -> None:
+        _lib.check(self.lib.hqt_set_switch(self.h, _lib.SWITCH_TILE_MFMA16, int(on)))
 
     def set_single_key(self, on: bool) -> None:
         _lib.check(self.lib.hqt_set_switch(self.h, _lib.SWITCH_SINGLE_KEY, int(bool(on))))
diff --git a/include/hqt.h b/include/hqt.h
--- a/include/hqt.h
+++ b/include/hqt.h
@@ -86,7 +86,7 @@
 enum { HQT_POLICY_LATENCY = 0, HQT_POLICY_THROUGHPUT = 1 };
 int hqt_set_policy(hqt_handle* h, int policy);
 
-enum { HQT_SWITCH_PERSIST = 0, HQT_SWITCH_SINGLE_KEY = 1, HQT_SWITCH_PERSIST_FAULT = 2, HQT_SWITCH_SPLIT_KSLICES = 3 };
+enum { HQT_SWITCH_PERSIST = 0, HQT_SWITCH_SINGLE_KEY = 1, HQT_SWITCH_PERSIST_FAULT = 2, HQT_SWITCH_SPLIT_KSLICES = 3, HQT_SWITCH_TILE_MFMA16 = 4 };
 int hqt_set_switch(hqt_handle* h, int which, int on);
 
 typedef struct { float temperature[3]; int32_t top_k[3]; float top_p[3]; } hqt_row_sampler;
```

Result: no change. 1716, median of 6 (+0.1%).
